# Frankie2030/DataMining_RecBLR

Hardware: AMD Instinct MI355X
Metric: sequences/sec fwd+bwd at B=2048 L=200 d=128; 1/2/4/8-GPU scaling (higher is better)
Workload: dtype f32 I/O, f16x3 split GEMM products

## Files before the change

datamining_recblr_amd/_lib.py:

```python
from __future__ import annotations

import ctypes
import os
import re
import threading

_HERE = os.path.dirname(os.path.abspath(__file__))
LIB_PATH = os.environ.get("RECBLR_LIB") or os.path.join(_HERE, "lib", "libdmrecblr.so")
HEADER_PATH = os.path.join(os.path.dirname(_HERE), "include", "recblr_hip.h")


class RecBLRNativeError(RuntimeError):
    """The HIP extension is missing, failed to load, or a kernel call failed."""


_BY_VALUE = {"int": ctypes.c_int, "int64_t": ctypes.c_int64, "uint64_t": ctypes.c_uint64,
             "float": ctypes.c_float, "double": ctypes.c_double}
_NOT_DECLARATIONS = re.compile(
    r'/\*.*?\*/|//[^\n]*|^[ \t]*#[^\n]*|\btypedef\b(?:[^;{]|\{[^}]*\})*;|extern\s+"C"\s*\{|^\s*\}\s*$',
    re.S | re.M)


def parse_header(text: str) -> dict:
    out = {}
    for decl in _NOT_DECLARATIONS.sub(" ", text).split(";"):
        decl = " ".join(decl.split())
        if not decl:
            continue
        m = re.fullmatch(r"([\w\s*]+?)\s*\b(\w+)\s*\(([^()]*)\)", decl)
        if m is None:
            raise RecBLRNativeError(f"header: not a plain function declaration: {decl!r}")
        ret, name, params = m.groups()
        if re.fullmatch(r"const\s+char\s*\*", ret):
            restype = ctypes.c_char_p
        elif ret in _BY_VALUE:
            restype = _BY_VALUE[ret]
        else:
            raise RecBLRNativeError(f"header: {name}: unsupported return type {ret!r}")
        argtypes = []
        for param in ([] if params.strip() == "void" else params.split(",")):
            words = param.split()
            by_value = " ".join(words[:-1] if len(words) > 1 else words)
            if "*" in param:
                argtypes.append(ctypes.c_void_p)
            elif by_value in _BY_VALUE:
                argtypes.append(_BY_VALUE[by_value])
            else:
                raise RecBLRNativeError(f"header: {name}: unsupported parameter {param.strip()!r}")
        out[name] = (restype, argtypes)
    return out


def _read(path: str) -> str:
    with open(path) as f:
        return f.read()


def _define(text: str, name: str) -> int:
    m = re.search(rf"^[ \t]*#[ \t]*define[ \t]+{name}[ \t]+\(?(-?\d+)\)?[ \t]*$", text, re.M)
    if m is None:
        raise RecBLRNativeError(f"header: no integer #define {name}")
    return int(m.group(1))


_header = _read(HEADER_PATH)
RB_EINVAL = _define(_header, "RB_EINVAL")
RB_TILE = _define(_header, "RB_TILE")
ABI_VERSION = _define(_header, "RB_ABI_VERSION")

SIGNATURES = parse_header(_header)
DENSE_SIGNATURES = parse_header(_read(os.path.join(os.path.dirname(HEADER_PATH),
                                                   "recblr_dense.h")))
PAIR_SIGNATURES = parse_header(_read(os.path.join(os.path.dirname(HEADER_PATH),
                                                  "recblr_pairs.h")))
CANDIDATE_SIGNATURES = parse_header(_read(os.path.join(os.path.dirname(HEADER_PATH),
                                                       "recblr_candidates.h")))
EXP_SIGNATURES = parse_header(_read(os.path.join(_HERE, "experimental", "recblr_exp.h")))
PROBE_SIGNATURES = parse_header(_read(os.path.join(_HERE, "probes", "recblr_probe.h")))
SESSION_SIGNATURES = parse_header(_read(os.path.join(_HERE, "session", "recblr_session.h")))

_lock = threading.Lock()
_loaded = {}


def _load(path, signatures, missing, version=None, mismatch=None, cache=True,
          hint="") -> ctypes.CDLL:
    with _lock:
        if cache and path in _loaded:
            return _loaded[path]
        if not os.path.exists(path):
            raise RecBLRNativeError(f"{missing}: {path} is missing. Run "
                                    f"`python -m datamining_recblr_amd.build`{hint}.")
        try:
            lib = ctypes.CDLL(path)
        except OSError as exc:
            raise RecBLRNativeError(f"failed to load {path}: {exc}") from exc
        for name, (res, args) in signatures.items():
            fn = getattr(lib, name)
            fn.restype = res
            fn.argtypes = args
        if version is not None and getattr(lib, version)() != ABI_VERSION:
            raise RecBLRNativeError(mismatch.format(getattr(lib, version)(), ABI_VERSION))
        if cache:
            _loaded[path] = lib
        return lib


def load(path: str | None = None) -> ctypes.CDLL:
    return _load(path or LIB_PATH,
                 {**SIGNATURES, **DENSE_SIGNATURES, **PAIR_SIGNATURES, **CANDIDATE_SIGNATURES},
                 "HIP extension not built",
                 "rb_version",
                 "ABI mismatch: library {} vs binding {}; rebuild", cache=path is None,
                 hint=" (hipcc --offload-arch=gfx950)")


def load_probe() -> ctypes.CDLL:
    return _load(os.path.join(os.path.dirname(LIB_PATH), "libdmrecblr_probe.so"),
                 PROBE_SIGNATURES, "probe library not built")


def load_exp() -> ctypes.CDLL:
    return _load(os.path.join(os.path.dirname(LIB_PATH), "libdmrecblr_exp.so"), EXP_SIGNATURES,
                 "experimental library not built", "rb_exp_version",
                 "experimental library ABI {} vs {}; rebuild")


def load_session() -> ctypes.CDLL:
    return _load(os.path.join(os.path.dirname(LIB_PATH), "libdmrecblr_session.so"),
                 SESSION_SIGNATURES, "session library not built", "rb_session_version",
                 "session library ABI {} vs {}; rebuild")


_fns = {}
_failure_hooks = []


def on_failure(hook) -> None:
    _failure_hooks.append(hook)


def _check(rc: int, name: str, lib: ctypes.CDLL, last_error: str, hooks: bool = True) -> None:
    if rc == 0:
        return
    kind = str(rc)
    if hooks:
        for hook in _failure_hooks:
            hook()
        kind = "invalid argument" if rc == RB_EINVAL else f"hipError {rc}"
    msg = getattr(lib, last_error)()
    raise RecBLRNativeError(f"{name} failed ({kind}): {msg.decode() if msg else ''}")


def call(name: str, *args) -> None:
    fn = _fns.get(name)
    if fn is None:
        fn = _fns[name] = getattr(load(), name)
    rc = fn(*args)
    if rc != 0:
        _check(rc, name, load(), "rb_last_error_string")


def call_probe(name: str, *args) -> None:
    lib = load_probe()
    _check(getattr(lib, name)(*args), name, lib, "rb_probe_last_error_string", hooks=False)


def call_exp(name: str, *args) -> None:
    lib = load_exp()
    _check(getattr(lib, name)(*args), name, lib, "rb_exp_last_error_string")


def call_session(name: str, *args) -> None:
    lib = load_session()
    rc = getattr(lib, name)(*args)
    if rc != 0:
        _check(rc, name, lib, "rb_session_last_error_string")
```

datamining_recblr_amd/build.py:

```python
from __future__ import annotations

import glob
import os
import shutil
import subprocess
import sys

_HERE = os.path.dirname(os.path.abspath(__file__))
ROOT = os.path.dirname(_HERE)
SOURCES = sorted(glob.glob(os.path.join(_HERE, "csrc", "*.hip")))
HEADERS = sorted(glob.glob(os.path.join(_HERE, "csrc", "*.h"))) + [
    os.path.join(ROOT, "include", "recblr_hip.h"),
    os.path.join(ROOT, "include", "recblr_dense.h"),
    os.path.join(ROOT, "include", "recblr_pairs.h"),
    os.path.join(ROOT, "include", "recblr_candidates.h")]
OUT = os.path.join(_HERE, "lib", "libdmrecblr.so")
PROBE_SOURCES = sorted(glob.glob(os.path.join(_HERE, "probes", "*.hip")))
PROBE_HEADERS = HEADERS + sorted(glob.glob(os.path.join(_HERE, "probes", "*.h")))
PROBE_OUT = os.path.join(_HERE, "lib", "libdmrecblr_probe.so")
EXP_SOURCES = sorted(glob.glob(os.path.join(_HERE, "experimental", "*.hip")))
EXP_HEADERS = HEADERS + sorted(glob.glob(os.path.join(_HERE, "experimental", "*.h")))
EXP_OUT = os.path.join(_HERE, "lib", "libdmrecblr_exp.so")
SESSION_SOURCES = sorted(glob.glob(os.path.join(_HERE, "session", "*.hip")))
SESSION_HEADERS = HEADERS + sorted(glob.glob(os.path.join(_HERE, "session", "*.h")))
SESSION_OUT = os.path.join(_HERE, "lib", "libdmrecblr_session.so")
ARCH = os.environ.get("PYTORCH_ROCM_ARCH", "gfx950")

FLAGS = ["-O3", "-std=c++20", "-shared", "-fPIC", f"--offload-arch={ARCH}",
         "-ffp-contract=off", "-Wall", "-Wno-unused-function"]


def hipcc() -> str:
    for cand in (os.environ.get("HIPCC"), "/opt/rocm/bin/hipcc", shutil.which("hipcc")):
        if cand and os.path.exists(cand):
            return cand
    raise RuntimeError("hipcc not found (expected /opt/rocm/bin/hipcc)")


def _stale(out, deps) -> bool:
    if not os.path.exists(out):
        return True
    t = os.path.getmtime(out)
    return any(os.path.getmtime(s) > t for s in deps)


def _compile(out, sources, extra, verbose, jobs):
    os.makedirs(os.path.dirname(out), exist_ok=True)
    tmp = out + ".tmp"
    cmd = [hipcc(), *FLAGS, *extra, "-I", os.path.join(ROOT, "include"), "-o", tmp, *sources]
    if jobs > 1:
        cmd.insert(1, f"-parallel-jobs={jobs}")
    if verbose:
        print(" ".join(cmd), flush=True)
    subprocess.run(cmd, check=True)
    os.replace(tmp, out)


def build(force: bool = False, verbose: bool = False, jobs: int = 4) -> str:
    if force or _stale(OUT, SOURCES + HEADERS):
        _compile(OUT, SOURCES, [], verbose, jobs)
    if PROBE_SOURCES and (force or _stale(PROBE_OUT, PROBE_SOURCES + PROBE_HEADERS)):
        _compile(PROBE_OUT, PROBE_SOURCES, ["-fvisibility=hidden"], verbose, jobs)
    if EXP_SOURCES and (force or _stale(EXP_OUT, EXP_SOURCES + EXP_HEADERS)):
        _compile(EXP_OUT, EXP_SOURCES, ["-fvisibility=hidden"], verbose, jobs)
    if SESSION_SOURCES and (force or _stale(SESSION_OUT, SESSION_SOURCES + SESSION_HEADERS)):
        _compile(SESSION_OUT, SESSION_SOURCES, ["-fvisibility=hidden"], verbose, jobs)
    return OUT


if __name__ == "__main__":
    print(build(force="--force" in sys.argv, verbose=True))
```

datamining_recblr_amd/csrc/capi.hip:

```cpp
#include "common.h"

#include <atomic>

namespace rb {

namespace {
thread_local std::string g_last_error;
}

int fail(const char* msg) {
  g_last_error = msg;
  return RB_EINVAL;
}

static int fail(const char* fn, const char* msg) {
  g_last_error = std::string(fn) + ": " + msg;
  return RB_EINVAL;
}

int num_cus() {
  static std::atomic<int> cache[64];
  int dev = 0;
  if (hipGetDevice(&dev) != hipSuccess || dev < 0 || dev >= 64) dev = 0;
  int n = cache[dev].load(std::memory_order_relaxed);
// ... 713 lines not shown
  return launch_candidate_scores(h, ldh, table, cand, B, C, d, V, scores, as_stream(stream));
}

int rb_candidate_topk(const float* h, int64_t ldh, const float* table, const int64_t* cand,
                      int64_t B, int64_t C, int64_t d, int64_t V, int64_t first_item, int64_t k,
                      const int64_t* exclude, int64_t E, int64_t* ids, float* scores,
                      void* stream) {
  const char* fn = "rb_candidate_topk";
  if (B < 0) return fail(fn, "B must be >= 0");
  if (B == 0) return 0;
  if (int rc = check_candidates(fn, h, ldh, table, cand, C, d, V)) return rc;
  if (!ids || !scores) return fail(fn, "null pointer");
  if (C > 4096) return fail(fn, "C must be in [1, 4096]");
  if (E < 0 || E > 4096) return fail(fn, "E must be in [0, 4096]");
  if (E > 0 && !exclude) return fail(fn, "null pointer");
  if (k < 1 || k >= (int64_t(1) << 31)) return fail(fn, "k must be in [1, 2^31)");
  if (first_item < 0 || first_item > V) return fail(fn, "first_item must be in [0, V]");
  if (B >= (int64_t(1) << 31)) return fail(fn, "grid too large");
  return launch_candidate_topk(h, ldh, table, cand, B, C, d, V, first_item, k, exclude, E, ids,
                               scores, as_stream(stream));
}

int rb_candidate_ranks(const float* h, int64_t ldh, const float* table, const int64_t* target,
                       const int64_t* cand, int64_t B, int64_t C, int64_t d, int64_t V,
                       int64_t first_item, int64_t* n_greater, int64_t* n_equal, void* stream) {
  const char* fn = "rb_candidate_ranks";
  if (B < 0) return fail(fn, "B must be >= 0");
  if (B == 0) return 0;
  if (int rc = check_candidates(fn, h, ldh, table, cand, C, d, V)) return rc;
  if (!target || !n_greater || !n_equal) return fail(fn, "null pointer");
  if (first_item < 0 || first_item > V) return fail(fn, "first_item must be in [0, V]");
  if (B >= (int64_t(1) << 31) || C >= (int64_t(1) << 40) ||
      B * candidate_rank_chunks(C) >= (int64_t(1) << 31))
    return fail(fn, "grid too large");
  return launch_candidate_ranks(h, ldh, table, target, cand, B, C, d, V, first_item, n_greater,
                                n_equal, as_stream(stream));
}

int rb_group_absmax(const float* x, int64_t n, int64_t c, int64_t ld, float* out, void* stream) {
  if (!x || !out) return fail("rb_group_absmax: null pointer");
  if (n <= 0 || c <= 0 || ld < c) return fail("rb_group_absmax: bad shape");
  return launch_group_absmax(x, n, c, ld, out, reinterpret_cast<hipStream_t>(stream));
}

int rb_item_scores(const float* seq, const float* items, int64_t B, int64_t V, int64_t d,
                   float* scores, void* stream) {
  if (int rc = check_items("rb_item_scores", seq, items, B, V, d)) return rc;
  if (!scores) return fail("rb_item_scores: null pointer");
  return launch_item_scores(seq, items, B, V, d, scores, reinterpret_cast<hipStream_t>(stream));
}

int rb_pad_prefix_fwd(const float* conv_b, const float* gate_w, const float* gate_b,
                      const float* lam, const int64_t* pad, int64_t pad_len, int64_t n_rows,
                      int64_t H, float* h0, float* workspace, void* stream) {
  if (!conv_b || !gate_w || !gate_b || !lam || !h0 || !workspace)
    return fail("rb_pad_prefix_fwd: null pointer");
  if (H <= 0 || H > 4096 || n_rows <= 0 || pad_len < 0)
    return fail("rb_pad_prefix_fwd: need 0 < H <= 4096, n_rows > 0, pad_len >= 0");
  return launch_pad_prefix_fwd(conv_b, gate_w, gate_b, lam, pad, pad_len, n_rows, H, h0,
                               workspace, reinterpret_cast<hipStream_t>(stream));
}

int rb_pad_prefix_bwd(const float* conv_b, const float* gate_w, const float* gate_b,
                      const float* lam, const int64_t* pad, int64_t pad_len, int64_t n_rows,
                      int64_t H, const float* dh0, float* dconv_b, float* dgate_w,
                      float* dgate_b, float* dlam, float* workspace, int accumulate,
                      void* stream) {
  if (!conv_b || !gate_w || !gate_b || !lam || !dh0 || !dconv_b || !dgate_w || !dgate_b || !dlam ||
      !workspace)
    return fail("rb_pad_prefix_bwd: null pointer");
  if (H <= 0 || H > 4096 || n_rows <= 0 || pad_len < 0)
    return fail("rb_pad_prefix_bwd: need 0 < H <= 4096, n_rows > 0, pad_len >= 0");
  return launch_pad_prefix_bwd(conv_b, gate_w, gate_b, lam, pad, pad_len, n_rows, H, dh0,
                               dconv_b, dgate_w, dgate_b, dlam, workspace, accumulate,
                               reinterpret_cast<hipStream_t>(stream));
}

int rb_colsum(const float* in, int64_t M, int64_t P, int64_t C, int64_t rs, int64_t ms,
              float* out, void* stream) {
  if (!in || !out) return fail("rb_colsum: null pointer");
  if (M <= 0 || P <= 0 || C <= 0 || rs < C || (M > 1 && ms < P * rs))
    return fail("rb_colsum: bad shape or strides");
  if (M * ((C + 63) / 64) > 0x7fffffffLL) return fail("rb_colsum: grid too large");
  return launch_colsum(in, M, P, C, rs, ms, out, reinterpret_cast<hipStream_t>(stream));
}

int rb_colsum_chunked(const float* in, int64_t M, int64_t P, int64_t C, int64_t rs,
                      int64_t chunk_rows, float* part, uint32_t* counters, int64_t n_counters,
                      float* out, void* stream) {
  if (!in || !out || !part || !counters) return fail("rb_colsum_chunked: null pointer");
  if (M <= 0 || P <= 0 || C <= 0 || rs < C ||
      (chunk_rows != 64 && chunk_rows != 128 && chunk_rows != 256) || P % chunk_rows)
    return fail("rb_colsum_chunked: bad shape, stride or chunk size");
  const int64_t cblocks = (C + 63) / 64;
  if (n_counters < M * cblocks) return fail("rb_colsum_chunked: too few counters");
  if (M * cblocks * (P / chunk_rows) > 0x7fffffffLL || M * P * rs >= ((int64_t)1 << 40))
    return fail("rb_colsum_chunked: grid too large");
  return launch_colsum_chunked(in, M, P, C, rs, (int)chunk_rows, part,
                               reinterpret_cast<unsigned*>(counters), out,
                               reinterpret_cast<hipStream_t>(stream));
}

int rb_pack_plan(const int64_t* item_seq, int64_t seq_rs, const int64_t* seq_offsets,
                 const int64_t* order, int64_t B, int64_t L, int64_t* ids, int64_t* row_pos,
                 int64_t* inv, int64_t* last, void* stream) {
  if (!item_seq || !seq_offsets || !order || !ids || !row_pos || !inv || !last)
    return fail("rb_pack_plan: null pointer");
  if (B < 1 || L < 1 || seq_rs < L) return fail("rb_pack_plan: bad shape or row stride");
  if ((B + 3) / 4 > 0x7fffffffLL) return fail("rb_pack_plan: grid too large");
  return launch_pack_plan(item_seq, seq_rs, seq_offsets, order, B, ids, row_pos, inv, last,
                          reinterpret_cast<hipStream_t>(stream));
}

int64_t rb_gemm_h_weight_bytes(int64_t C, int64_t R) {
  return ws_image_offset(C, R) + (R % 32 == 0 ? C * R * 4 : 0);
}
int rb_gemm_nt_h_mode(int mode) { return gemm_nt_h_mode(mode); }

int rb_gemm_nt_h_ln(const float* A, int64_t lda, int64_t M, int64_t R, const void* Wf, int64_t C,
                    const float* bias, const float* resid, const float* gamma, const float* beta,
                    float eps, uint64_t seed, float p, float* y, float* s_out, float* mean,
                    float* rstd, int64_t ldo, float* rmax, void* stream) {
  if (!A || !Wf || !resid || !gamma || !beta || !y || !s_out || !mean || !rstd)
    return fail("rb_gemm_nt_h_ln: null pointer");
  if (M <= 0 || R <= 0 || C != 128) return fail("rb_gemm_nt_h_ln: C must be 128, M and R positive");
  if (R != 128 && R != 256 && R != 512) return fail("rb_gemm_nt_h_ln: R must be 128, 256 or 512");
  if (lda < R || lda % 4 || ldo < C || ldo % 4) return fail("rb_gemm_nt_h_ln: bad row strides");
  if (!aligned16(A) || !aligned16(Wf) || !aligned16(resid) || !aligned16(y) || !aligned16(s_out) ||
      !aligned16(gamma) || !aligned16(beta) || (bias && !aligned16(bias)))
    return fail("rb_gemm_nt_h_ln: A, Wf, resid, y, s_out, gamma, beta and bias must be 16-byte aligned");
  if (!(p >= 0.0f && p < 1.0f)) return fail("rb_gemm_nt_h_ln: dropout p must be in [0, 1)");
  if (!(eps > 0.0f)) return fail("rb_gemm_nt_h_ln: eps must be positive");
  if ((M + 31) / 32 > 0x3fffffffLL) return fail("rb_gemm_nt_h_ln: grid too large");
  if (gemm_nt_h_mode(-1) != 1) return fail("rb_gemm_nt_h_ln: needs the weight-stationary kernel (rb_gemm_nt_h_mode 1)");
  return launch_gemm_nt_ws_ln(A, lda, M, (int)R, Wf, (int)C, bias, resid, make_drop(nullptr, seed, p),
                              gamma, beta, eps, y, s_out, mean, rstd, ldo, rmax,
                              reinterpret_cast<hipStream_t>(stream));
}

int rb_gemm_h_split_weights(const rb_split_job* jobs, int64_t n, void* stream) {
  if (!jobs || n < 1 || n > RB_MAX_SPLIT_JOBS)
    return fail("rb_gemm_h_split_weights: need 1..RB_MAX_SPLIT_JOBS jobs");
  for (int64_t j = 0; j < n; ++j) {
    const rb_split_job& b = jobs[j];
    if (!b.W || !b.Wf) return fail("rb_gemm_h_split_weights: null pointer");
    if (b.C <= 0 || b.R <= 0 || b.C % 32 || b.R % 16 || b.C > (1 << 20) || b.R > (1 << 20))
      return fail("rb_gemm_h_split_weights: C must be a multiple of 32 and R of 16");
    if (b.ldw < (b.transpose ? b.C : b.R)) return fail("rb_gemm_h_split_weights: bad row stride");
    if (!aligned16(b.Wf)) return fail("rb_gemm_h_split_weights: Wf must be 16-byte aligned");
  }
  return launch_split_weights_h(jobs, (int)n, reinterpret_cast<hipStream_t>(stream));
}

int rb_gemm_nt_h(const float* A, int64_t lda, int64_t M, int64_t R, const void* Wf, int64_t C,
                 const float* bias, float* out, int64_t ldo, int accumulate, float* rmax,
                 void* stream) {
  if (!A || !Wf || !out) return fail("rb_gemm_nt_h: null pointer");
  if (M <= 0 || R <= 0 || C <= 0) return fail("rb_gemm_nt_h: empty shape");
  if (accumulate) return fail("rb_gemm_nt_h: accumulate is not supported (add the residual in its consumer)");
  if (R % 32 || C % 32 || R > (1 << 16) || C > 1024)
    return fail("rb_gemm_nt_h: R and C must be multiples of 32 (C <= 1024)");
  if (lda < R || lda % 4 || ldo < C || ldo % 2) return fail("rb_gemm_nt_h: bad row strides");
  if (!aligned16(A) || !aligned16(Wf) || (reinterpret_cast<uintptr_t>(out) & 7))
    return fail("rb_gemm_nt_h: A and Wf must be 16-byte aligned, out 8-byte aligned");
  if ((M + 31) / 32 > 0x7fffffffLL) return fail("rb_gemm_nt_h: grid too large");
  return launch_gemm_nt_h(A, lda, M, (int)R, Wf, (int)C, bias, out, ldo, accumulate, rmax,
                          reinterpret_cast<hipStream_t>(stream));
}

int rb_gemm_nt_h_act(const float* A, int64_t lda, int64_t M, int64_t R, const void* Wf, int64_t C,
                     const float* bias, float* out, int64_t ldo, float* rmax, float* act,
                     uint64_t seed, float p, void* stream) {
  if (!A || !Wf || !out || !act) return fail("rb_gemm_nt_h_act: null pointer");
  if (M <= 0 || R <= 0 || C <= 0) return fail("rb_gemm_nt_h_act: empty shape");
  if (R % 32 || C % 32 || R > 1024 || C > 1024)
    return fail("rb_gemm_nt_h_act: R and C must be multiples of 32 (R, C <= 1024)");
  if (lda < R || lda % 4 || ldo < C || ldo % 4) return fail("rb_gemm_nt_h_act: bad row strides");
  if (!aligned16(A) || !aligned16(Wf) || !aligned16(out) || !aligned16(act) ||
      (bias && !aligned16(bias)))
    return fail("rb_gemm_nt_h_act: A, Wf, out, act and bias must be 16-byte aligned");
  if (!(p >= 0.0f && p < 1.0f)) return fail("rb_gemm_nt_h_act: dropout p must be in [0, 1)");
  if ((M + 31) / 32 > 0x7fffffffLL) return fail("rb_gemm_nt_h_act: grid too large");
  return launch_gemm_nt_h_act(A, lda, M, (int)R, Wf, (int)C, bias, out, ldo, rmax, act,
                              make_drop(nullptr, seed, p), reinterpret_cast<hipStream_t>(stream));
}

int rb_adam_step(const rb_adam_job* jobs, int64_t n, double lr, double beta1, double beta2,
                 double eps, double weight_decay, double bc1, double bc2, void* stream) {
  if (!jobs || n <= 0 || n > RB_MAX_ADAM_JOBS) return fail("rb_adam_step: 1..RB_MAX_ADAM_JOBS jobs");
  int64_t blocks = 0;
  for (int64_t j = 0; j < n; ++j) {
    const rb_adam_job& b = jobs[j];
    if (!b.param || !b.grad || !b.exp_avg || !b.exp_avg_sq || b.n <= 0)
      return fail("rb_adam_step: null pointer or empty tensor");
    if (!aligned16(b.param) || !aligned16(b.grad) || !aligned16(b.exp_avg) ||
        !aligned16(b.exp_avg_sq))
      return fail("rb_adam_step: tensors must be 16-byte aligned");
    blocks += (b.n + 1023) / 1024;
  }
  if (blocks > 0x7fffffffLL) return fail("rb_adam_step: too many elements");
  if (!(bc1 > 0.0 && bc2 > 0.0)) return fail("rb_adam_step: bias corrections must be > 0");
  return launch_adam(jobs, (int)n, lr, beta1, beta2, eps, weight_decay, bc1, bc2,
                     reinterpret_cast<hipStream_t>(stream));
}

int64_t rb_gemm_nt_h_dact_parts(void) { return nt_h_dact_parts(); }

int rb_gemm_nt_h_dact(const float* A, int64_t lda, int64_t M, int64_t R, const void* Wf, int64_t C,
                      float* out, int64_t ldo, float* rmax, const float* pre, uint64_t seed,
                      float p, float* dpart, int64_t n_parts, void* stream) {
  if (!A || !Wf || !out || !pre || !dpart) return fail("rb_gemm_nt_h_dact: null pointer");
  if (M <= 0 || R <= 0 || C <= 0) return fail("rb_gemm_nt_h_dact: empty shape");
  if (R % 32 || C % 32 || R > 1024 || C > 512)
    return fail("rb_gemm_nt_h_dact: R and C must be multiples of 32 (R <= 1024, C <= 512)");
  if (lda < R || lda % 4 || ldo < C || ldo % 4) return fail("rb_gemm_nt_h_dact: bad row strides");
  if (!aligned16(A) || !aligned16(Wf) || !aligned16(out) || !aligned16(pre) || !aligned16(dpart))
    return fail("rb_gemm_nt_h_dact: A, Wf, out, pre and dpart must be 16-byte aligned");
  if (!(p >= 0.0f && p < 1.0f)) return fail("rb_gemm_nt_h_dact: dropout p must be in [0, 1)");
  if ((M + 31) / 32 > 0x7fffffffLL) return fail("rb_gemm_nt_h_dact: grid too large");
  return launch_gemm_nt_h_dact(A, lda, M, (int)R, Wf, (int)C, out, ldo, rmax, pre,
                               make_drop(nullptr, seed, p), dpart, n_parts,
                               reinterpret_cast<hipStream_t>(stream));
}

int rb_gemm_tn_h(const float* dY, int64_t ldy, const float* X, int64_t ldx, int64_t M, int64_t N,
                 int64_t K, const float* ymax, const float* xmax, float* parts, int64_t splits,
                 void* stream) {
  if (!dY || !X || !ymax || !xmax || !parts) return fail("rb_gemm_tn_h: null pointer");
  if (M <= 0 || N <= 0 || K <= 0) return fail("rb_gemm_tn_h: empty shape");
  if (N % 128 || K % 128 || N > 65536 || K > 65536)
    return fail("rb_gemm_tn_h: N and K must be multiples of 128 (<= 65536)");
  if (splits < 1 || splits > 65536) return fail("rb_gemm_tn_h: splits must be in [1, 65536]");
  if (ldy < N || ldx < K || ldy % 4 || ldx % 4) return fail("rb_gemm_tn_h: bad row strides");
  if (!aligned16(dY) || !aligned16(X)) return fail("rb_gemm_tn_h: dY and X must be 16-byte aligned");
  if ((N / 128) * (K / 128) * splits > 0x7fffffffLL) return fail("rb_gemm_tn_h: grid too large");
  const int64_t mk = ((M + splits - 1) / splits + 31) / 32 * 32;
  if (mk * (ldy > ldx ? ldy : ldx) * 4 >= 0x7fffffffLL)
    return fail("rb_gemm_tn_h: a row chunk spans 2 GiB or more (use more splits)");
  return launch_gemm_tn_h(dY, ldy, X, ldx, M, (int)N, (int)K, ymax, xmax, parts, (int)splits,
                          reinterpret_cast<hipStream_t>(stream));
}

int rb_gemm_bf16_weight_image(const float* W, int64_t ldw, int64_t C, int64_t R, int transpose,
                              void* img, void* stream) {
  if (!W || !img) return fail("rb_gemm_bf16_weight_image: null pointer");
  if (C <= 0 || R <= 0 || C % 16 || R % 32 || C > 65536 || R > 65536)
    return fail("rb_gemm_bf16_weight_image: C % 16 == 0 and R % 32 == 0 required (<= 65536)");
  if (ldw < (transpose ? C : R)) return fail("rb_gemm_bf16_weight_image: bad row stride");
  if (!aligned16(img)) return fail("rb_gemm_bf16_weight_image: img must be 16-byte aligned");
  return launch_bf16_weight_image(W, ldw, (int)C, (int)R, transpose ? 1 : 0, img,
                                  reinterpret_cast<hipStream_t>(stream));
}

int rb_gemm_nt_bf16(const void* A, int64_t lda, int64_t M, int64_t R, const void* img, int64_t C,
                    const float* bias, void* out, int64_t ldo, void* stream) {
  if (!A || !img || !out) return fail("rb_gemm_nt_bf16: null pointer");
  if (M <= 0 || R <= 0 || C <= 0) return fail("rb_gemm_nt_bf16: empty shape");
  if (R % 64 || C % 256 || R > 16384 || C > 65536)
    return fail("rb_gemm_nt_bf16: R % 64 == 0 (<= 16384) and C % 256 == 0 required");
  if (lda < R || lda % 8 || lda > (1 << 20) || ldo < C || ldo % 8)
    return fail("rb_gemm_nt_bf16: bad row strides (lda % 8 == 0, ldo % 8 == 0)");
  if (!aligned16(A) || !aligned16(img) || !aligned16(out) || (bias && !aligned16(bias)))
    return fail("rb_gemm_nt_bf16: A, img, out and bias must be 16-byte aligned");
  if ((M + 255) / 256 > 0x7fffffffLL / (C / 256) / 2) return fail("rb_gemm_nt_bf16: too many tiles");
  return launch_gemm_nt_bf16(A, lda, M, (int)R, img, (int)C, bias, out, ldo,
                             reinterpret_cast<hipStream_t>(stream));
}

int rb_gemm_tn_hs(const float* dY, int64_t ldy, const float* X, int64_t ldx, int64_t M, int64_t N,
                  int64_t K, float* dw, int accumulate, void* stream) {
  if (!dY || !X || !dw) return fail("rb_gemm_tn_hs: null pointer");
  if (M <= 0 || N <= 0 || K <= 0) return fail("rb_gemm_tn_hs: empty shape");
  if (N % 32 || K % 32 || N > 65536 || K > 65536)
    return fail("rb_gemm_tn_hs: N and K must be multiples of 32");
  if (M > (1 << 24)) return fail("rb_gemm_tn_hs: M too large for the few-rows kernel");
  if (ldy < N || ldx < K) return fail("rb_gemm_tn_hs: bad row strides");
  return launch_gemm_tn_hs(dY, ldy, X, ldx, M, (int)N, (int)K, dw, accumulate,
                           reinterpret_cast<hipStream_t>(stream));
}

}
```

datamining_recblr_amd/csrc/common.h:

```cpp
#pragma once

#include <hip/hip_runtime.h>

#include <algorithm>
#include <cstdint>
#include <string>
#include <type_traits>

#include "../../include/recblr_hip.h"
#include "../../include/recblr_dense.h"
#include "../../include/recblr_pairs.h"
#include "../../include/recblr_candidates.h"

namespace rb {

constexpr int kWave = 64;

int fail(const char* msg);
int launch_status(const char* what);
int num_cus();

inline bool aligned16(const void* p) { return (reinterpret_cast<uintptr_t>(p) & 15) == 0; }

template <class F>
auto dispatch_bool(bool b, F&& f) {
  return b ? f(std::true_type{}) : f(std::false_type{});
}
template <int... Vs, class F>
bool dispatch_int(int v, F&& f) {
  return ((v == Vs ? (f(std::integral_constant<int, Vs>{}), true) : false) || ...);
}

__device__ __forceinline__ float sigm(float x) { return 1.0f / (1.0f + expf(-x)); }
__device__ __forceinline__ float softplus_f(float x) { return x > 20.0f ? x : log1pf(expf(x)); }
__device__ __forceinline__ float dsoftplus_f(float x) { return x > 20.0f ? 1.0f : sigm(x); }
__device__ __forceinline__ float silu_f(float x) { return x / (1.0f + expf(-x)); }
__device__ __forceinline__ float dsilu_f(float x) {
  const float s = sigm(x);
  return s * (1.0f + x * (1.0f - s));
}

constexpr float kLog2e = 1.4426950408889634f;
__device__ __forceinline__ float fexp(float x) { return __builtin_amdgcn_exp2f(x * kLog2e); }
__device__ __forceinline__ float frcp(float x) { return __builtin_amdgcn_rcpf(x); }
__device__ __forceinline__ float fsqrt(float x) { return __builtin_amdgcn_sqrtf(x); }
__device__ __forceinline__ float fsigm(float x) { return frcp(1.0f + fexp(-x)); }
__device__ __forceinline__ float fsilu(float x) { return x * fsigm(x); }
__device__ __forceinline__ float fdsilu(float x) {
  const float s = fsigm(x);
  return s * (1.0f + x * (1.0f - s));
}

typedef float rb_f32x4 __attribute__((ext_vector_type(4)));
typedef float rb_f32x2v __attribute__((ext_vector_type(2)));
typedef uint32_t rb_u32x4 __attribute__((ext_vector_type(4)));
typedef uint32_t rb_u32x2 __attribute__((ext_vector_type(2)));

template <bool NT, typename T>
__device__ __forceinline__ T ld_pol(const T* p) {
  if constexpr (NT) return __builtin_nontemporal_load(p);
  else return *p;
}
template <bool NT, typename T>
__device__ __forceinline__ void st_pol(T v, T* p) {
  if constexpr (NT) __builtin_nontemporal_store(v, p);
  else *p = v;
}
constexpr bool kNT = true;

template <bool NT, int V>
__device__ __forceinline__ void ld_f32(float (&o)[V], const float* p) {
  if constexpr (V == 4) {
    const rb_f32x4 t = ld_pol<NT>(reinterpret_cast<const rb_f32x4*>(p));
    o[0] = t[0]; o[1] = t[1]; o[2] = t[2]; o[3] = t[3];
  } else if constexpr (V == 2) {
    const rb_f32x2v t = ld_pol<NT>(reinterpret_cast<const rb_f32x2v*>(p));
    o[0] = t[0]; o[1] = t[1];
  } else {
#pragma unroll
    for (int v = 0; v < V; ++v) o[v] = ld_pol<NT>(p + v);
  }
}

template <bool NT, int V>
__device__ __forceinline__ void st_f32(float* p, const float (&o)[V]) {
  if constexpr (V == 4) {
    st_pol<NT>(rb_f32x4{o[0], o[1], o[2], o[3]}, reinterpret_cast<rb_f32x4*>(p));
  } else if constexpr (V == 2) {
    st_pol<NT>(rb_f32x2v{o[0], o[1]}, reinterpret_cast<rb_f32x2v*>(p));
  } else {
#pragma unroll
    for (int v = 0; v < V; ++v) st_pol<NT>(o[v], p + v);
  }
}

template <int V>
__device__ __forceinline__ void ldv(float (&o)[V], const float* p) { ld_f32<kNT>(o, p); }
template <int V>
__device__ __forceinline__ void stv(float* p, const float (&o)[V]) { st_f32<kNT>(p, o); }
template <int V>
__device__ __forceinline__ void ldc(float (&o)[V], const float* p) { ld_f32<false>(o, p); }
template <int V>
__device__ __forceinline__ void stc(float* p, const float (&o)[V]) { st_f32<false>(p, o); }

typedef __bf16 bf16_t;
typedef __bf16 rb_bf16x2 __attribute__((ext_vector_type(2)));
typedef float rb_f32x2 __attribute__((ext_vector_type(2)));

__device__ __forceinline__ void unpack2(uint32_t u, float& a, float& b) {
  a = __uint_as_float(u << 16);
  b = __uint_as_float(u & 0xffff0000u);
}
__device__ __forceinline__ uint32_t pack2(float a, float b) {
  return __builtin_bit_cast(uint32_t, __builtin_convertvector(rb_f32x2{a, b}, rb_bf16x2));
}

template <bool NT, int V>
__device__ __forceinline__ void ld_b16(float (&o)[V], const bf16_t* p) {
  if constexpr (V == 8) {
    const rb_u32x4 t = ld_pol<NT>(reinterpret_cast<const rb_u32x4*>(p));
    unpack2(t[0], o[0], o[1]); unpack2(t[1], o[2], o[3]);
    unpack2(t[2], o[4], o[5]); unpack2(t[3], o[6], o[7]);
  } else if constexpr (V == 4) {
    const rb_u32x2 t = ld_pol<NT>(reinterpret_cast<const rb_u32x2*>(p));
    unpack2(t[0], o[0], o[1]); unpack2(t[1], o[2], o[3]);
  } else if constexpr (V == 2) {
    unpack2(ld_pol<NT>(reinterpret_cast<const uint32_t*>(p)), o[0], o[1]);
  } else {
#pragma unroll
    for (int v = 0; v < V; ++v) o[v] = (float)p[v];
  }
}

template <bool NT, int V>
__device__ __forceinline__ void st_b16(bf16_t* p, const float (&o)[V]) {
  if constexpr (V == 8) {
    st_pol<NT>(rb_u32x4{pack2(o[0], o[1]), pack2(o[2], o[3]), pack2(o[4], o[5]), pack2(o[6], o[7])},
               reinterpret_cast<rb_u32x4*>(p));
  } else if constexpr (V == 4) {
    st_pol<NT>(rb_u32x2{pack2(o[0], o[1]), pack2(o[2], o[3])}, reinterpret_cast<rb_u32x2*>(p));
  } else if constexpr (V == 2) {
    st_pol<NT>(pack2(o[0], o[1]), reinterpret_cast<uint32_t*>(p));
  } else {
#pragma unroll
    for (int v = 0; v < V; ++v) p[v] = (bf16_t)o[v];
  }
}

template <int V>
__device__ __forceinline__ void ldv(float (&o)[V], const bf16_t* p) { ld_b16<kNT>(o, p); }
template <int V>
__device__ __forceinline__ void stv(bf16_t* p, const float (&o)[V]) { st_b16<kNT>(p, o); }
template <int V>
__device__ __forceinline__ void ldc(float (&o)[V], const bf16_t* p) { ld_b16<false>(o, p); }
template <int V>
__device__ __forceinline__ void stc(bf16_t* p, const float (&o)[V]) { st_b16<false>(p, o); }

template <typename T, int V>
struct RawVec {
  float w[V];
};
template <int V>
struct RawVec<bf16_t, V> {
  static_assert(V % 2 == 0, "packed bf16 needs an even width");
  uint32_t w[V / 2];
// ... 32 lines not shown
}
template <int V>
__device__ __forceinline__ void unpack_raw(float (&o)[V], const RawVec<bf16_t, V>& r) {
  if constexpr (V == 1) {
    o[0] = r.w[0];
  } else {
#pragma unroll
    for (int k = 0; k < V / 2; ++k) unpack2(r.w[k], o[2 * k], o[2 * k + 1]);
  }
}

template <int VH, typename T, int V>
__device__ __forceinline__ void unpack_part(float (&o)[VH], const RawVec<T, V>& r, int h0) {
  if constexpr (VH == V) {
    unpack_raw(o, r);
  } else if constexpr (sizeof(T) == 4) {
#pragma unroll
    for (int v = 0; v < VH; ++v) o[v] = r.w[h0 + v];
  } else {
#pragma unroll
    for (int k = 0; k < VH / 2; ++k) unpack2(r.w[h0 / 2 + k], o[2 * k], o[2 * k + 1]);
  }
}
template <int VH, typename T, int V>
__device__ __forceinline__ void pack_part(RawVec<T, V>& r, const float (&o)[VH], int h0) {
  if constexpr (sizeof(T) == 4) {
#pragma unroll
    for (int v = 0; v < VH; ++v) r.w[h0 + v] = o[v];
  } else {
    static_assert(VH % 2 == 0, "packed bf16 pairs");
#pragma unroll
    for (int k = 0; k < VH / 2; ++k) r.w[h0 / 2 + k] = pack2(o[2 * k], o[2 * k + 1]);
  }
}
template <int VH, typename T, int V>
__device__ __forceinline__ void opaque_part(RawVec<T, V>& r, int h0) {
  constexpr int per = sizeof(T) == 2 && V > 1 ? 2 : 1;
#pragma unroll
  for (int k = 0; k < VH / per; ++k) asm volatile("" : "+v"(r.w[h0 / per + k]));
}
template <int V>
__device__ __forceinline__ void stv_raw(float* p, const RawVec<float, V>& r) { st_f32<kNT>(p, r.w); }
template <int V>
__device__ __forceinline__ void stv_raw(bf16_t* p, const RawVec<bf16_t, V>& r) {
  if constexpr (V == 8) {
    st_pol<kNT>(rb_u32x4{r.w[0], r.w[1], r.w[2], r.w[3]}, reinterpret_cast<rb_u32x4*>(p));
  } else if constexpr (V == 4) {
    st_pol<kNT>(rb_u32x2{r.w[0], r.w[1]}, reinterpret_cast<rb_u32x2*>(p));
  } else {
    static_assert(V == 2, "packed bf16 image");
    st_pol<kNT>(r.w[0], reinterpret_cast<uint32_t*>(p));
  }
}

__device__ __forceinline__ uint4 philox4x32_10(uint4 c, uint32_t k0, uint32_t k1) {
#pragma unroll
  for (int i = 0; i < 10; ++i) {
    const uint64_t p0 = (uint64_t)0xD2511F53u * c.x, p1 = (uint64_t)0xCD9E8D57u * c.z;
    const uint32_t lo0 = (uint32_t)p0, hi0 = (uint32_t)(p0 >> 32);
    const uint32_t lo1 = (uint32_t)p1, hi1 = (uint32_t)(p1 >> 32);
    c = make_uint4(hi1 ^ c.y ^ k0, lo1, hi0 ^ c.w ^ k1, lo0);
    k0 += 0x9E3779B9u;
    k1 += 0xBB67AE85u;
  }
  return c;
}

struct DropSpec {
  const uint8_t* mask;
  uint32_t key0, key1, keep_thresh;
  float scale;
  int mode;

  __device__ __forceinline__ void get4(int64_t e, float (&m)[4]) const {
    if (mode == 0) {
      m[0] = m[1] = m[2] = m[3] = 1.0f;
    } else if (mode == 1) {
      const uchar4 t = *reinterpret_cast<const uchar4*>(mask + e);
      m[0] = t.x * scale; m[1] = t.y * scale; m[2] = t.z * scale; m[3] = t.w * scale;
    } else {
      const uint64_t g = (uint64_t)e >> 2;
      const uint4 r = philox4x32_10(make_uint4((uint32_t)g, (uint32_t)(g >> 32), 0u, 0u), key0,
                                    key1);
      m[0] = r.x < keep_thresh ? scale : 0.0f;
      m[1] = r.y < keep_thresh ? scale : 0.0f;
      m[2] = r.z < keep_thresh ? scale : 0.0f;
      m[3] = r.w < keep_thresh ? scale : 0.0f;
    }
  }
};

DropSpec make_drop(const uint8_t* mask, uint64_t seed, float p);


int launch_pack_plan(const int64_t* seq, int64_t seq_rs, const int64_t* offs,
                     const int64_t* order, int64_t B, int64_t* ids, int64_t* pos, int64_t* inv,
                     int64_t* last, hipStream_t st);
int launch_next_item_targets(const int64_t* ids, const int64_t* offs, const int64_t* order,
                             const int64_t* pos_items, int64_t B, int64_t ntok, int64_t m_pad,
                             int64_t* tgt, hipStream_t st);
template <typename T>
int launch_scan_fwd(const T* gates, const T* tokens, T* states, int64_t rows, int64_t steps,
                    hipStream_t st);
template <typename T>
int launch_scan_bwd(const T* gates, const T* states, const T* grad, T* d_gates, T* d_tokens,
                    int64_t rows, int64_t steps, hipStream_t st);
template <typename T>
int launch_conv_fwd(const T* x, int64_t x_rs, const float* w, const float* bias, T* xc,
                    int64_t xc_rs, int64_t B, int64_t L, int64_t H, int64_t K,
                    const int64_t* offs, hipStream_t st);
template <typename T>
int launch_conv_fwd_rows(const T* x, int64_t x_rs, const float* w, const float* bias, T* xc,
                         int64_t xc_rs, int64_t ntok, int64_t H, int64_t K, const int64_t* pos,
                         hipStream_t st);
template <typename T>
int launch_conv_bwd(const T* x, int64_t x_rs, const float* w, const float* bias, const T* g1,
                    const T* g2, T* dx, int64_t dx_rs, float* dw_part, float* db_part, int64_t B,
                    int64_t L, int64_t H, int64_t K, const int64_t* offs, hipStream_t st);
template <typename T>
int launch_gate_fwd(const T* rg, int64_t rg_rs, const T* xc, int64_t xc_rs, const T* z,
                    int64_t z_rs, const float* lam, const float* gb, const float* h0,
                    int64_t h0_bs, T* y, int64_t y_rs, float* carries, int64_t B, int64_t L,
                    int64_t H, const int64_t* offs, hipStream_t st, T* y_last = nullptr,
                    const int64_t* order = nullptr);
template <typename T>
int launch_gate_bwd(const T* rg, int64_t rg_rs, const T* xc, int64_t xc_rs, const T* z,
                    int64_t z_rs, const float* lam, const float* gb, const float* carries,
                    const T* dy, T* drg, int64_t drg_rs, T* dxc, int64_t dxc_rs, T* dz,
                    int64_t dz_rs, float* part, float* dh0_part, int64_t B, int64_t L, int64_t H,
                    const int64_t* offs, hipStream_t st, const T* dy_last = nullptr,
                    const int64_t* order = nullptr);
int launch_add_ln_fwd(const float* a, const int64_t* idx, int64_t nidx, const DropSpec& drop,
                      const float* r, const float* gamma, const float* beta, float eps, float* y,
                      float* s_out, float* mean, float* rstd, int64_t rows, int64_t d,
                      hipStream_t st);
int launch_add_ln_bwd(const float* dy, const float* dy2, const float* s, const float* gamma,
                      const float* mean, const float* rstd, const DropSpec& drop, float* ds,
                      float* da, float* dgp, float* dbp, float* dbiasp, int64_t nparts,
                      int64_t rows, int64_t d, hipStream_t st);
int64_t ln_num_parts(int64_t rows, int64_t d);
int launch_silu_dropout_fwd(const float* a, const float* bias, const DropSpec& drop, float* u,
                            int64_t rows, int64_t cols, hipStream_t st);
int launch_silu_dropout_bwd(const float* a, const float* bias, const DropSpec& drop,
                            const float* du, float* da, float* dbias_part, int64_t nparts,
                            int64_t rows, int64_t cols, hipStream_t st);
int launch_dropout_mask(const DropSpec& drop, uint8_t* out, int64_t n, hipStream_t st);
int launch_split_weights_h(const rb_split_job* jobs, int n, hipStream_t st);
int launch_bf16_weight_image(const float* W, int64_t ldw, int C, int R, int transpose, void* img,
                             hipStream_t st);
int launch_gemm_nt_bf16(const void* A, int64_t lda, int64_t M, int R, const void* img, int C,
                        const float* bias, void* out, int64_t ldo, hipStream_t st);
int launch_gemm_tn_h(const float* Y, int64_t ldy, const float* X, int64_t ldx, int64_t M, int N,
                     int K, const float* ymax, const float* xmax, float* parts, int S,
                     hipStream_t st);
constexpr int kWeightScale = 14;
template <class S>
struct WeightSlot {
  S slot;
  int col, k0;
};
template <class S = int64_t, class I>
__host__ __device__ inline WeightSlot<S> weight_slot32(int nkb, I cb, int kb, int p, int lane) {
  return {((S)(cb * nkb + kb) * 2 + p) * 64 + lane, (int)cb * 32 + (lane & 31),
          kb * 16 + 8 * (lane >> 5)};
}
template <class S = int64_t, class I>
__host__ __device__ inline WeightSlot<S> weight_slot16(int nkb, I cb, int ks, int p, int lane) {
  return {((S)(cb * nkb + ks) * 2 + p) * 64 + lane, (int)cb * 16 + (lane & 15),
          ks * 32 + 8 * (lane >> 4)};
}
__host__ __device__ inline int64_t ws_image_offset(int64_t C, int64_t K) {
  return C * K * 4 + ((C * 4 + 15) / 16) * 16;
}
struct WeightImage {
  const void* wf;
  const int* ew;
  const void* wi;
};
inline WeightImage weight_image(const void* Wf, int64_t C, int64_t R) {
  const char* base = static_cast<const char*>(Wf);
  return {Wf, reinterpret_cast<const int*>(base + C * R * 4), base + ws_image_offset(C, R)};
}
int nt_dact_zero_rest(float* dpart, int64_t used, int64_t n_parts, int C, hipStream_t st);
bool nt_ws_ok(int64_t M, int K, int C, const float* A, int64_t lda, const float* out, int64_t ldo);
int launch_gemm_nt_ws(const float* A, int64_t lda, int64_t M, int K, const void* Wf, int C,
                      const float* bias, float* out, int64_t ldo, float* rmax, hipStream_t st);
int gemm_nt_h_mode(int mode);
bool nt_ws_act_ok(int64_t M, int K, int C, const float* A, int64_t lda, const float* out,
                  const float* other, int64_t ldo);
int launch_gemm_nt_ws_act(const float* A, int64_t lda, int64_t M, int K, const void* Wf, int C,
                          const float* bias, float* out, int64_t ldo, float* rmax, float* act,
                          DropSpec drop, hipStream_t st);
int launch_gemm_nt_ws_dact(const float* A, int64_t lda, int64_t M, int K, const void* Wf, int C,
                           float* out, int64_t ldo, float* rmax, const float* pre, DropSpec drop,
                           float* dpart, int64_t n_parts, hipStream_t st);
bool nt_ws_ln_ok(int64_t M, int K, int C, const float* A, int64_t lda, const float* y,
                 const float* s_out, const float* resid, int64_t ldo);
int launch_gemm_nt_ws_ln(const float* A, int64_t lda, int64_t M, int K, const void* Wf, int C,
                         const float* bias, const float* resid, DropSpec drop, const float* gamma,
                         const float* beta, float eps, float* y, float* s_out, float* mean,
                         float* rstd, int64_t ldo, float* rmax, hipStream_t st);
int launch_gemm_nt_h(const float* A, int64_t lda, int64_t M, int R, const void* Wf, int C,
                     const float* bias, float* out, int64_t ldo, int accumulate, float* rmax,
                     hipStream_t st);
int launch_gemm_nt_h_act(const float* A, int64_t lda, int64_t M, int R, const void* Wf, int C,
                         const float* bias, float* out, int64_t ldo, float* rmax, float* act,
                         DropSpec drop, hipStream_t st);
int64_t nt_h_dact_parts();
int launch_gemm_nt_h_dact(const float* A, int64_t lda, int64_t M, int R, const void* Wf, int C,
                          float* out, int64_t ldo, float* rmax, const float* pre, DropSpec drop,
                          float* dpart, int64_t n_parts, hipStream_t st);
int launch_adam(const rb_adam_job* jobs, int n, double lr, double beta1, double beta2, double eps,
                double weight_decay, double bc1, double bc2, hipStream_t st);
int launch_gemm_nt_hs(const float* A, int64_t lda, int64_t M, int R, const void* Wf, int C,
                      const float* bias, float* out, int64_t ldo, float* rmax, hipStream_t st);
int launch_gemm_tn_hs(const float* Y, int64_t ldy, const float* X, int64_t ldx, int64_t M, int N,
                      int K, float* dw, int accumulate, hipStream_t st);
int64_t emb_workspace_bytes(int64_t M, int64_t V, int64_t d);
int launch_embedding_plan(const int64_t* idx, int64_t M, int64_t d, int64_t V, void* workspace,
                          int64_t ws_bytes, hipStream_t st);
int launch_embedding_apply(const float* grad, int64_t M, int64_t d, int64_t V,
                           int64_t padding_idx, float* dw, void* workspace, int64_t ws_bytes,
                           hipStream_t st);
int launch_embedding_bwd(const int64_t* idx, const float* grad, int64_t M, int64_t d, int64_t V,
                         int64_t padding_idx, float* dw, void* workspace, int64_t ws_bytes,
                         hipStream_t st);
int launch_embedding_apply_scaled(const float* src, int64_t src_ld, int64_t src_rows,
                                  const float* coef, int64_t M, int64_t d, int64_t V,
                                  int64_t padding_idx, float* dw, void* workspace,
                                  int64_t ws_bytes, hipStream_t st);
int launch_sample_negatives(const int64_t* item_seq, int64_t seq_rs, const int64_t* lengths,
                            const int64_t* pos_items, const int64_t* offsets, const int64_t* inv,
                            int64_t B, int64_t L, int64_t n_neg, int64_t first, int64_t V,
                            uint64_t seed, int64_t ntok, int64_t m_pad, int64_t* neg,
                            hipStream_t st);
int64_t pair_loss_workspace_bytes(int64_t M);
int launch_pair_loss_fwd(const float* h, int64_t ldh, const float* tab, const int64_t* pos,
                         const int64_t* neg, int64_t M, int64_t d, int64_t V, int64_t n_neg,
                         float gamma, float* diff, float* loss, int64_t* n_live, void* workspace,
                         hipStream_t st);
int launch_pair_loss_bwd(const float* tab, const int64_t* pos, const int64_t* neg,
                         const float* diff, const float* dloss, const int64_t* n_live, int64_t M,
                         int64_t d, int64_t V, int64_t n_neg, float gamma, float* dh, float* coef,
                         hipStream_t st);
int launch_candidate_scores(const float* h, int64_t ldh, const float* tab, const int64_t* cand,
                            int64_t B, int64_t C, int64_t d, int64_t V, float* scores,
                            hipStream_t st);
int launch_candidate_topk(const float* h, int64_t ldh, const float* tab, const int64_t* cand,
                          int64_t B, int64_t C, int64_t d, int64_t V, int64_t first, int64_t k,
                          const int64_t* exclude, int64_t E, int64_t* ids, float* scores,
                          hipStream_t st);
int64_t candidate_rank_chunks(int64_t C);
int launch_candidate_ranks(const float* h, int64_t ldh, const float* tab, const int64_t* target,
                           const int64_t* cand, int64_t B, int64_t C, int64_t d, int64_t V,
                           int64_t first, int64_t* n_gt, int64_t* n_eq, hipStream_t st);
int64_t item_ce_workspace_bytes(int64_t B, int64_t V, int64_t D);
int64_t item_rank_workspace_bytes(int64_t B, int64_t V);
int launch_item_ce_fwd(const float* E, const float* W, const int64_t* tgt, int64_t B, int64_t V,
                       int64_t D, float* lse, float* loss, void* ws, int64_t ws_bytes,
                       hipStream_t st);
int launch_item_ce_bwd(const float* E, const float* W, const int64_t* tgt, const float* lse,
                       const float* dloss, int64_t B, int64_t V, int64_t D, float* dE, float* dW,
                       void* ws, int64_t ws_bytes, hipStream_t st);
int launch_item_rank(const float* E, const float* W, const int64_t* tgt, int64_t B, int64_t V,
                     int64_t D, int64_t first, int64_t* n_gt, int64_t* n_eq, void* ws,
                     int64_t ws_bytes, hipStream_t st);
int64_t item_topk_workspace_bytes(int64_t B, int64_t V, int64_t k);
int launch_item_topk(const float* E, const float* W, int64_t B, int64_t V, int64_t D, int64_t k,
                     int64_t first, const int64_t* ex, int64_t NE, int64_t* ids, float* scores,
                     void* ws, int64_t ws_bytes, hipStream_t st);
int launch_item_ce_probs(const float* E, const float* W, const int64_t* tgt, const float* lse,
                         const float* dloss, int64_t B, int64_t V, int64_t D, int64_t v_off,
                         int64_t n_total, float* out, int64_t ld, hipStream_t st);
int launch_item_scores(const float* E, const float* W, int64_t B, int64_t V, int64_t D,
                       float* out, hipStream_t st);
int launch_item_split_h(const float* X, int64_t N, int64_t D, void* img, int* ex, float* gmax,
                        hipStream_t st);
int launch_item_ce_fwd_h(const void* Ei, const int* Ee, const void* Wi, const int* We,
                         const int64_t* tgt, int64_t B, int64_t V, int64_t D, float* lse,
                         float* loss, void* ws, int64_t ws_bytes, bool rows_mode, float inv_n,
                         int accumulate, hipStream_t st);
int launch_item_ce_probs_h(const void* Ei, const int* Ee, const void* Wi, const int* We,
                           const int64_t* tgt, const float* lse, const float* dloss, int64_t B,
                           int64_t V, int64_t D, int64_t v_off, float* out, int64_t ld,
                           float* gmax, float* out2, int64_t ld2, float* bmax, float rows_inv_n,
                           hipStream_t st);
int launch_group_absmax(const float* x, int64_t n, int64_t c, int64_t ld, float* out,
                        hipStream_t st);
int launch_pad_prefix_fwd(const float* conv_b, const float* gw, const float* gb,
                          const float* lam, const int64_t* pad, int64_t pad_len, int64_t n_rows,
                          int64_t H, float* h0, float* ws, hipStream_t st);
int launch_pad_prefix_bwd(const float* conv_b, const float* gw, const float* gb,
                          const float* lam, const int64_t* pad, int64_t pad_len, int64_t n_rows,
                          int64_t H, const float* dh0, float* dconv_b, float* dgw, float* dgb,
                          float* dlam, float* ws, int accumulate, hipStream_t st);
int launch_colsum(const float* in, int64_t M, int64_t P, int64_t C, int64_t rs, int64_t ms,
                  float* out, hipStream_t st);
int launch_colsum_chunked(const float* in, int64_t M, int64_t P, int64_t C, int64_t rs, int CH,
                          float* part, unsigned* cnt, float* out, hipStream_t st);

}
```

datamining_recblr_amd/csrc/gemm_half.hip:

```cpp
#include "common.h"
#include "f16x3.h"
#include "nt_plan.h"

#include <type_traits>

namespace rb {
namespace {

constexpr int kTA = 4;
constexpr int kHead = 11;
constexpr int kTRedo = 14;
constexpr int kSent = -4096;

struct SplitJobsH {
  const float* W[RB_MAX_SPLIT_JOBS];
  f16x8* Wf[RB_MAX_SPLIT_JOBS];
  int64_t ldw[RB_MAX_SPLIT_JOBS];
  int C[RB_MAX_SPLIT_JOBS], R[RB_MAX_SPLIT_JOBS], tr[RB_MAX_SPLIT_JOBS];
  int bstart[RB_MAX_SPLIT_JOBS + 1];
  int n;
};

__global__ void __launch_bounds__(256) k_split_weights_h(const SplitJobsH jobs) {
  __shared__ float smax[256];
// ... 552 lines not shown
      float m = 0.0f;
      for (int kb = 0; kb < KB16; ++kb) {
        const f32x4 p = *reinterpret_cast<const f32x4*>(arow + kb * 16);
        const f32x4 q = *reinterpret_cast<const f32x4*>(arow + kb * 16 + 4);
        m = fmaxf(m, max8abs(p, q));
      }
      m = fmaxf(m, __shfl_xor(m, 32));
      const int e = exp_of(m);
      const float sc = __builtin_amdgcn_ldexpf(1.0f, kTRedo - e);
      int erow[16];
#pragma unroll
      for (int j = 0; j < 16; ++j) erow[j] = __shfl(e, crow(j)) - kTRedo - kWeightScale;
      for (int n = 0; n < N_NB; ++n) {
        f32x16 c;
#pragma unroll
        for (int j = 0; j < 16; ++j) c[j] = 0.0f;
        for (int kb = 0; kb < KB16; ++kb) {
          const f32x4 p = *reinterpret_cast<const f32x4*>(arow + kb * 16);
          const f32x4 q = *reinterpret_cast<const f32x4*>(arow + kb * 16 + 4);
          f16x8 a0, a1;
          split8(p, q, sc, a0, a1);
          const f16x8* bp = Wf + ((int64_t)((ct * N_NB + n) * KB16 + kb) * 2) * 64 + lane;
          const f16x8 b0 = bp[0], b1 = bp[64];
          c = mfma3_h(a0, a1, b0, b1, c);
        }
        const int col = ct * N_BN + n * 32 + ccol;
        const int ecol = s_ew[col];
        const float bv = BIAS ? s_bias[col] : 0.0f;
        float csum = 0.0f;
#pragma unroll
        for (int j = 0; j < 16; ++j) {
          const int64_t r = (int64_t)mt * N_BM + wave * 32 + crow(j);
          if (r < M) {
            float v = __builtin_amdgcn_ldexpf(c[j], erow[j] + ecol) + bv;
            if constexpr (DACT) {
              float mk[4];
              const int64_t ei = e_base + r * C + col;
              drop.get4(ei & ~(int64_t)3, mk);
              const int q = (int)(ei & 3);
              v = (v * (q == 0 ? mk[0] : q == 1 ? mk[1] : q == 2 ? mk[2] : mk[3])) *
                  fdsilu(pre[r * ldo + col] + 0.0f);
              csum += v;
            }
            out[r * ldo + col] = v;
            if constexpr (ACT) {
              float mk[4];
              const int64_t ei = e_base + r * C + col;
              drop.get4(ei & ~(int64_t)3, mk);
              const int q = (int)(ei & 3);
              act[r * ldo + col] = fsilu(v) * (q == 0 ? mk[0] : q == 1 ? mk[1] : q == 2 ? mk[2] : mk[3]);
            }
          }
        }
        if constexpr (DACT) {
          csum += __shfl_xor(csum, 32);
          if (lane < 32) s_col[col] += csum;
        }
      }
    }
  }
  if constexpr (DACT) {
    __syncthreads();
    const float* s_all = reinterpret_cast<const float*>(smem + CF::LDS);
    for (int c = tid; c < C; c += N_THREADS) {
      float t = s_all[c];
#pragma unroll
      for (int w = 1; w < N_WAVES; ++w) t += s_all[w * N_DACT_MAXC + c];
      dpart[(int64_t)bid * C + c] = t;
    }
  }
}

template <bool BIAS, bool WIDE, int NB, bool ACT = false, bool DACT = false>
__global__ void __launch_bounds__(N_THREADS, 1) k_gemm_nt_h(const float* __restrict__ A, int64_t lda,
                                                          int64_t M, int R,
                                                          const f16x8* __restrict__ Wf,
                                                          const int* __restrict__ ew, int C,
                                                          const float* __restrict__ bias,
                                                          float* __restrict__ out, int64_t ldo,
                                                          float* __restrict__ rmax, int m_tiles,
                                                          float* __restrict__ act, DropSpec drop,
                                                          int64_t e_base,
                                                          const float* __restrict__ pre,
                                                          float* __restrict__ dpart) {
  extern __shared__ __attribute__((aligned(16))) char smem[];
  nt_h_body<BIAS, WIDE, NB, ACT, DACT>(smem, (int)blockIdx.x, (int)gridDim.x, A, lda, M, R, Wf, ew,
                                       C, bias, out, ldo, rmax, m_tiles, act, drop, e_base, pre,
                                       dpart);
}

struct NtPhase {
  const float* A;
  int64_t M;
  float* out;
  float* rmax;
  float* act;
  const float* pre;
  float* dpart;
  int64_t e_base;
  int m_tiles;
  int grid;
};

template <bool BIAS, int NB, bool ACT = false, bool DACT = false>
__global__ void __launch_bounds__(N_THREADS, 1)
k_gemm_nt_h2(int64_t lda, int R, const f16x8* __restrict__ Wf, const int* __restrict__ ew, int C,
             const float* __restrict__ bias, int64_t ldo, DropSpec drop, NtPhase main_ph,
             NtPhase tail_ph) {
  extern __shared__ __attribute__((aligned(16))) char smem[];
  const int bid = (int)blockIdx.x;
  if (bid < main_ph.grid)
    nt_h_body<BIAS, true, NB, ACT, DACT>(smem, bid, main_ph.grid, main_ph.A, lda, main_ph.M, R, Wf,
                                         ew, C, bias, main_ph.out, ldo, main_ph.rmax,
                                         main_ph.m_tiles, main_ph.act, drop, main_ph.e_base,
                                         main_ph.pre, main_ph.dpart);
  __syncthreads();
  if (bid < tail_ph.grid)
    nt_h_body<BIAS, true, 2, ACT, DACT>(smem, bid, tail_ph.grid, tail_ph.A, lda, tail_ph.M, R, Wf,
                                        ew, C, bias, tail_ph.out, ldo, tail_ph.rmax,
                                        tail_ph.m_tiles, tail_ph.act, drop, tail_ph.e_base,
                                        tail_ph.pre, tail_ph.dpart);
}

constexpr int T_BT = 128;
constexpr int T_PITCH = 80;
constexpr int kTT = 14;

template <int NBN, int NBK>
struct TnCfg {
  static constexpr int THREADS = 256 * NBN * NBK;
  static constexpr int YC = T_BT * NBN, XC = T_BT * NBK;
  static constexpr int YPLANE = YC * T_PITCH, XPLANE = XC * T_PITCH;
  static constexpr int STAGE = 2 * YPLANE + 2 * XPLANE;
  static constexpr int LDS = 2 * STAGE;
  static constexpr int LOADERS = (YC + XC) / 4 * 4;
};

__device__ __forceinline__ uint32_t tn_off(int col, int chunk) {
  return col * T_PITCH + ((chunk ^ ((col >> 4) & 3)) << 4);
}

template <int NBN, int NBK>
__device__ __attribute__((noinline)) void tn_percol(char* smem, const float* __restrict__ Y, int64_t ldy, const float* __restrict__ X,
                                        int64_t ldx, int64_t M, int N, int K,
                                        const float* __restrict__ ymax,
                                        const float* __restrict__ xmax, float* __restrict__ parts,
                                        int S, int64_t mk, int nt_k);

template <int NBN, int NBK, bool PERCOL>
__device__ __forceinline__ void tn_body(char* smem, const float* __restrict__ Y, int64_t ldy, const float* __restrict__ X,
                                        int64_t ldx, int64_t M, int N, int K,
                                        const float* __restrict__ ymax,
                                        const float* __restrict__ xmax, float* __restrict__ parts,
                                        int S, int64_t mk, int nt_k) {
  using CF = TnCfg<NBN, NBK>;
  const int tid = threadIdx.x;
  const int lane = tid & 63;
  const int wave = __builtin_amdgcn_readfirstlane(tid >> 6);
  const int wm = wave / (2 * NBK), wk = wave % (2 * NBK);
  const int G = gridDim.x;
  const int idx = (blockIdx.x & 7) * (G >> 3) + (blockIdx.x >> 3);
  const int nt = (N / CF::YC) * nt_k;
  const int tile = idx % nt, s = idx / nt;
  if (s >= S) return;
  const int n0 = (tile / nt_k) * CF::YC, k0 = (tile % nt_k) * CF::XC;
  const int64_t r_begin = (int64_t)s * mk;
  const int64_t r_end = r_begin + mk < M ? r_begin + mk : M;
  const int64_t nrows = r_end > r_begin ? r_end - r_begin : 0;
  const int T = (int)((nrows + 31) / 32);

  float my = 0.0f, mx = 0.0f;
  for (int64_t g = r_begin / 32 + tid; g * 32 < r_end; g += CF::THREADS) {
    my = fmaxf(my, ymax[g]);
    mx = fmaxf(mx, xmax[g]);
  }
  float* red = reinterpret_cast<float*>(smem);
#pragma unroll
  for (int o = 32; o >= 1; o >>= 1) {
    my = fmaxf(my, __shfl_xor(my, o));
    mx = fmaxf(mx, __shfl_xor(mx, o));
  }
  constexpr int NW = CF::THREADS / 64;
  if (lane == 0) { red[wave] = my; red[NW + wave] = mx; }
  __syncthreads();
  my = 0.0f;
  mx = 0.0f;
#pragma unroll
  for (int w = 0; w < NW; ++w) {
    my = fmaxf(my, red[w]);
    mx = fmaxf(mx, red[NW + w]);
  }
  const int ey = exp_of(my), ex = exp_of(mx);
  __syncthreads();

  const bool loader = tid < CF::LOADERS;
  const int op = tid < CF::YC ? 0 : 1;
  const int lt = op == 0 ? tid : tid - CF::YC;
  const int ncg = (op == 0 ? CF::YC : CF::XC) / 4;
  const int cc = loader ? lt % ncg : 0;
  const int rg = loader ? lt / ncg : 0;
  const int64_t ld = op == 0 ? ldy : ldx;
  float scv[4];
#pragma unroll
  for (int c = 0; c < 4; ++c) {
    int e = op == 0 ? ey : ex;
    if constexpr (PERCOL) {
      const int col = 4 * cc + c;
      e = *reinterpret_cast<const int*>(smem + (op == 0 ? col * T_PITCH
                                                        : 2 * CF::YPLANE + col * T_PITCH) + 64);
    }
    scv[c] = __builtin_amdgcn_ldexpf(1.0f, kTT - e);
  }
  float cm[4] = {0.0f, 0.0f, 0.0f, 0.0f};
  const uint32_t smem_base = (uint32_t)(uintptr_t)(lds_ptr_t)smem;

  f32x4 raw0[8], raw1[8];
  const float* cbase = (op == 0 ? Y + n0 : X + k0) + r_begin * ld;
  const uint64_t cb = reinterpret_cast<uint64_t>(cbase);
  const uint64_t cbu =
      (uint64_t)(uint32_t)__builtin_amdgcn_readfirstlane((uint32_t)cb) |
      ((uint64_t)(uint32_t)__builtin_amdgcn_readfirstlane((uint32_t)(cb >> 32)) << 32);
  const uint32_t ld4 = __builtin_amdgcn_readfirstlane((uint32_t)(ld * 4));
  const auto rsrc = __builtin_amdgcn_make_buffer_rsrc(
      reinterpret_cast<void*>(cbu), 0, (int)(nrows * ld4), 0x00020000);
  const uint32_t voff = (uint32_t)(rg * 8) * ld4 + (uint32_t)(16 * cc);
  auto load = [&](int t, f32x4 (&r)[8]) {
    __builtin_amdgcn_sched_barrier(0);
#pragma unroll
    for (int q = 0; q < 8; ++q)
      r[q] = __builtin_bit_cast(
          f32x4, __builtin_amdgcn_raw_buffer_load_b128(rsrc, voff + (uint32_t)(t * 32 + q) * ld4, 0, 0));
    __builtin_amdgcn_sched_barrier(0);
  };
  auto convert_pair = [&](const f32x4 (&r)[8], int buf, int p) {
    const uint32_t img = smem_base + buf * CF::STAGE + (op == 0 ? 0 : 2 * CF::YPLANE);
    const uint32_t plane = op == 0 ? CF::YPLANE : CF::XPLANE;
    const f32x2 sc{scv[2 * p], scv[2 * p + 1]};
    f16x8 h0[2], h1[2];
#pragma unroll
    for (int q = 0; q < 8; ++q) {
      const f32x2 v{r[q][2 * p], r[q][2 * p + 1]};
      f16x2 p0, p1;
      split2h(v * sc, p0, p1);
      h0[0][q] = p0[0]; h0[1][q] = p0[1];
      h1[0][q] = p1[0]; h1[1][q] = p1[1];
    }
    if constexpr (!PERCOL) {
#pragma unroll
      for (int c = 0; c < 2; ++c)
#pragma unroll
        for (int q = 0; q < 8; q += 4) {
          cm[2 * p + c] = max3abs(cm[2 * p + c], r[q][2 * p + c], r[q + 1][2 * p + c]);
          cm[2 * p + c] = max3abs(cm[2 * p + c], r[q + 2][2 * p + c], r[q + 3][2 * p + c]);
        }
    }
#pragma unroll
    for (int c = 0; c < 2; ++c) {
      const uint32_t off = tn_off(4 * cc + 2 * p + c, rg);
      lds_write16(img + off, h0[c]);
      lds_write16(img + plane + off, h1[c]);
    }
  };

  f32x16 acc[2][2];
#pragma unroll
  for (int a = 0; a < 2; ++a)
#pragma unroll
    for (int b = 0; b < 2; ++b)
#pragma unroll
      for (int e = 0; e < 16; ++e) acc[a][b][e] = 0.0f;

  const int h = lane >> 5;
  auto mma = [&](int buf, auto conv_c, const f32x4 (&r)[8], int t, int nbuf, auto late_c) {
    (void)t;
    constexpr bool CONV = decltype(conv_c)::value;
    constexpr bool LATE = decltype(late_c)::value;
    const uint32_t iy = smem_base + buf * CF::STAGE;
    const uint32_t ix = iy + 2 * CF::YPLANE;
#pragma unroll
    for (int st = 0; st < 2; ++st) {
      if constexpr (CONV && !LATE) convert_pair(r, nbuf, st);
      f16x8 b[2][2];
#pragma unroll
      for (int j = 0; j < 2; ++j) {
        const uint32_t ob = tn_off(64 * wk + 32 * j + (lane & 31), 2 * st + h);
        b[j][0] = lds_read16<f16x8>(ix + ob);
        b[j][1] = lds_read16<f16x8>(ix + CF::XPLANE + ob);
      }
#pragma unroll
      for (int i = 0; i < 2; ++i) {
        const uint32_t oa = tn_off(64 * wm + 32 * i + (lane & 31), 2 * st + h);
        f16x8 a0 = lds_read16<f16x8>(iy + oa);
        f16x8 a1 = lds_read16<f16x8>(iy + CF::YPLANE + oa);
        if (i == 0)
          asm volatile("s_waitcnt lgkmcnt(0)"
                       : "+v"(a0), "+v"(a1), "+v"(b[0][0]), "+v"(b[0][1]), "+v"(b[1][0]),
                         "+v"(b[1][1]));
        else
          asm volatile("s_waitcnt lgkmcnt(0)" : "+v"(a0), "+v"(a1));
#pragma unroll
        for (int j = 0; j < 2; ++j) {
          acc[i][j] = mfma3_h(a0, a1, b[j][0], b[j][1], acc[i][j]);
        }
      }
      if constexpr (CONV && LATE) convert_pair(r, nbuf, st);
    }
  };
  using conv_t = std::true_type;
  using noconv_t = std::false_type;

  const int Tp = (T + 1) & ~1;
  auto loader_loop = [&](auto late_c) {
    load(0, raw0);
    load(1, raw1);
    convert_pair(raw0, 0, 0);
    convert_pair(raw0, 0, 1);
    load(2, raw0);
    __syncthreads();
    for (int t = 0; t < Tp; t += 2) {
      mma(0, conv_t{}, raw1, t + 1, 1, late_c);
      load(t + 3, raw1);
      __syncthreads();
      mma(1, conv_t{}, raw0, t + 2, 0, late_c);
      load(t + 4, raw0);
      __syncthreads();
    }
  };
  const int wv = __builtin_amdgcn_readfirstlane(tid >> 6);
  if (wv < CF::LOADERS / 64) {
    if (CF::THREADS == 512 && wv >= 4) loader_loop(std::true_type{});
    else loader_loop(std::false_type{});
  } else {
    __syncthreads();
    for (int t = 0; t < Tp; t += 2) {
      mma(0, noconv_t{}, raw1, 0, 0, std::false_type{});
      __syncthreads();
      mma(1, noconv_t{}, raw0, 0, 0, std::false_type{});
      __syncthreads();
    }
  }

  constexpr int NCOL = CF::YC + CF::XC;
  constexpr int pass = PERCOL ? 1 : 0;
  if constexpr (!PERCOL) {
    __syncthreads();
    float* s_cm = reinterpret_cast<float*>(smem + CF::STAGE);
    int* s_redo = reinterpret_cast<int*>(smem + CF::STAGE) + 4 * NCOL;
    if (tid == 0) *s_redo = 0;
    if (loader) {
#pragma unroll
      for (int c = 0; c < 4; ++c) s_cm[rg * NCOL + (op == 0 ? 0 : CF::YC) + 4 * cc + c] = cm[c];
    }
    __syncthreads();
    for (int col = tid; col < NCOL; col += CF::THREADS) {
      const float m = fmaxf(fmaxf(s_cm[col], s_cm[NCOL + col]),
                            fmaxf(s_cm[2 * NCOL + col], s_cm[3 * NCOL + col]));
      const int ec = col < CF::YC ? ey : ex;
      if (m > 0.0f && m < __builtin_amdgcn_ldexpf(1.0f, ec - 16)) *s_redo = 1;
      const int e = exp_of(m);
      const int slot = col < CF::YC ? col * T_PITCH : 2 * CF::YPLANE + (col - CF::YC) * T_PITCH;
      *reinterpret_cast<int*>(smem + slot + 64) = e;
    }
    __syncthreads();
    if (*s_redo != 0) {
      tn_percol<NBN, NBK>(smem, Y, ldy, X, ldx, M, N, K, ymax, xmax, parts, S, mk, nt_k);
      return;
    }
  }

  float* out = parts + (int64_t)s * N * K;
  if constexpr (pass == 0) {
    const int sh = ey + ex - 2 * kTT;
#pragma unroll
    for (int i = 0; i < 2; ++i)
#pragma unroll
      for (int j = 0; j < 2; ++j) {
        const int col = k0 + 64 * wk + 32 * j + (lane & 31);
#pragma unroll
        for (int e = 0; e < 16; ++e) {
          const int row = n0 + 64 * wm + 32 * i + 8 * (e >> 2) + 4 * h + (e & 3);
          __builtin_nontemporal_store(__builtin_amdgcn_ldexpf(acc[i][j][e], sh), out + (int64_t)row * K + col);
        }
      }
  } else {
#pragma unroll
    for (int i = 0; i < 2; ++i)
#pragma unroll
      for (int e = 0; e < 16; ++e) {
        const int nl = 64 * wm + 32 * i + 8 * (e >> 2) + 4 * h + (e & 3);
        const int en = *reinterpret_cast<const int*>(smem + nl * T_PITCH + 64) - 2 * kTT;
#pragma unroll
        for (int j = 0; j < 2; ++j) {
          const int kl = 64 * wk + 32 * j + (lane & 31);
          const int ek = *reinterpret_cast<const int*>(smem + 2 * CF::YPLANE + kl * T_PITCH + 64);
          __builtin_nontemporal_store(__builtin_amdgcn_ldexpf(acc[i][j][e], en + ek), out + (int64_t)(n0 + nl) * K + k0 + kl);
        }
      }
  }
}

template <int NBN, int NBK>
__device__ __attribute__((noinline)) void tn_percol(char* smem, const float* __restrict__ Y, int64_t ldy, const float* __restrict__ X,
                                        int64_t ldx, int64_t M, int N, int K,
                                        const float* __restrict__ ymax,
                                        const float* __restrict__ xmax, float* __restrict__ parts,
                                        int S, int64_t mk, int nt_k) {
  tn_body<NBN, NBK, true>(smem, Y, ldy, X, ldx, M, N, K, ymax, xmax, parts, S, mk, nt_k);
}

template <int NBN, int NBK>
__global__ void __launch_bounds__(256 * NBN * NBK, 2 / (NBN * NBK))
k_gemm_tn_h(const float* __restrict__ Y, int64_t ldy, const float* __restrict__ X, int64_t ldx,
            int64_t M, int N, int K, const float* __restrict__ ymax,
            const float* __restrict__ xmax, float* __restrict__ parts, int S, int64_t mk,
            int nt_k) {
  extern __shared__ __attribute__((aligned(16))) char smem[];
  tn_body<NBN, NBK, false>(smem, Y, ldy, X, ldx, M, N, K, ymax, xmax, parts, S, mk, nt_k);
}


template <bool BIAS, bool WIDE, int NB, bool ACT = false, bool DACT = false>
void run_nt_h(const float* A, int64_t lda, int64_t M, int R, const f16x8* wf, const int* ew, int C,
              const float* bias, float* out, int64_t ldo, float* rmax, int m_tiles, unsigned grid,
              hipStream_t st, float* act = nullptr, DropSpec drop = DropSpec{}, int64_t e_base = 0,
              const float* pre = nullptr, float* dpart = nullptr) {
  constexpr int lds = NtCfg<NB>::LDS + (DACT ? N_WAVES * N_DACT_MAXC * 4 : 0);
  static_assert(lds <= 160 * 1024, "LDS");
  static bool done = false;
  if (!done) {
    (void)hipFuncSetAttribute((const void*)k_gemm_nt_h<BIAS, WIDE, NB, ACT, DACT>,
                        hipFuncAttributeMaxDynamicSharedMemorySize, lds);
    done = true;
  }
  k_gemm_nt_h<BIAS, WIDE, NB, ACT, DACT><<<grid, N_THREADS, lds, st>>>(
      A, lda, M, R, wf, ew, C, bias, out, ldo, rmax, m_tiles, act, drop, e_base, pre, dpart);
}


struct NtArgs {
  const float* A;
  int64_t lda, M;
  int R;
  const void* Wf;
  int C;
  const float* bias;
  float* out;
  int64_t ldo;
  float* rmax;
  float* act;
  const float* pre;
  float* dpart;
  DropSpec drop;
  hipStream_t st;
};

NtPhase nt_phase(const NtArgs& a, int64_t r0, int64_t M, int m_tiles, int grid,
                 int64_t dpart_row) {
  NtPhase p{};
  p.A = a.A + r0 * a.lda;
  p.M = M;
  p.out = a.out + r0 * a.ldo;
  p.rmax = a.rmax ? a.rmax + r0 / 32 : nullptr;
  p.act = a.act ? a.act + r0 * a.ldo : nullptr;
  p.pre = a.pre ? a.pre + r0 * a.ldo : nullptr;
  p.dpart = a.dpart ? a.dpart + dpart_row * a.C : nullptr;
  p.e_base = r0 * a.C;
  p.m_tiles = m_tiles;
  p.grid = grid;
  return p;
}

template <bool BIAS, int NB, bool ACT = false, bool DACT = false>
void run_nt_h2(int64_t lda, int R, const f16x8* wf, const int* ew, int C, const float* bias,
               int64_t ldo, DropSpec drop, const NtPhase& mp, const NtPhase& tp, hipStream_t st) {
  constexpr int base = NtCfg<NB>::LDS > NtCfg<2>::LDS ? NtCfg<NB>::LDS : NtCfg<2>::LDS;
  constexpr int lds = base + (DACT ? N_WAVES * N_DACT_MAXC * 4 : 0);
  static_assert(lds <= 160 * 1024, "LDS");
  static bool done = false;
  if (!done) {
    (void)hipFuncSetAttribute((const void*)k_gemm_nt_h2<BIAS, NB, ACT, DACT>,
                              hipFuncAttributeMaxDynamicSharedMemorySize, lds);
    done = true;
  }
  const unsigned grid = (unsigned)std::max(mp.grid, tp.grid);
  k_gemm_nt_h2<BIAS, NB, ACT, DACT><<<grid, N_THREADS, lds, st>>>(lda, R, wf, ew, C, bias, ldo,
                                                                  drop, mp, tp);
}

template <bool BIAS, bool WIDE, int NB, bool ACT = false, bool DACT = false>
int run_nt_plan(const char* what, const NtPlan& p, const NtArgs& a) {
  const WeightImage w = weight_image(a.Wf, a.C, a.R);
  const f16x8* wf = (const f16x8*)w.wf;
  const NtPhase mp = nt_phase(a, 0, p.M_main, p.m_tiles, p.grid, 0);
  const NtPhase tp = nt_phase(a, p.M_main, a.M - p.M_main, p.m_tiles_t, p.grid_t, p.dpart_tail);
  auto launch = [&](auto wide_c, auto nb_c, const NtPhase& ph) {
    run_nt_h<BIAS, decltype(wide_c)::value, decltype(nb_c)::value, ACT, DACT>(
        ph.A, a.lda, ph.M, a.R, wf, w.ew, a.C, a.bias, ph.out, a.ldo, ph.rmax, ph.m_tiles,
        (unsigned)ph.grid, a.st, ph.act, a.drop, ph.e_base, ph.pre, ph.dpart);
    return launch_status(what);
  };
  switch (p.path) {
    case NtPath::error:
      return fail(p.err);
    case NtPath::both:
      run_nt_h2<BIAS, NB, ACT, DACT>(a.lda, a.R, wf, w.ew, a.C, a.bias, a.ldo, a.drop, mp, tp, a.st);
      return launch_status(what);
    case NtPath::tail:
      return launch(std::true_type{}, std::integral_constant<int, 2>{}, tp);
    case NtPath::few:
    case NtPath::few_main: {
      const int rc = launch_gemm_nt_hs(tp.A, a.lda, tp.M, a.R, a.Wf, a.C, a.bias, tp.out, a.ldo,
                                       tp.rmax, a.st);
      if (rc || p.path == NtPath::few) return rc;
      break;
    }
    case NtPath::main:
      break;
  }
  return launch(std::bool_constant<WIDE>{}, std::integral_constant<int, NB>{}, mp);
}

}

int launch_split_weights_h(const rb_split_job* jobs, int n, hipStream_t st) {
  SplitJobsH sj{};
  sj.n = n;
  int blocks = 0;
  for (int j = 0; j < n; ++j) {
    sj.W[j] = jobs[j].W;
    sj.Wf[j] = (f16x8*)jobs[j].Wf;
    sj.ldw[j] = jobs[j].ldw;
    sj.C[j] = (int)jobs[j].C;
    sj.R[j] = (int)jobs[j].R;
    sj.tr[j] = (int)jobs[j].transpose;
    sj.bstart[j] = blocks;
    blocks += (int)(jobs[j].C / 32);
  }
  sj.bstart[n] = blocks;
  k_split_weights_h<<<(unsigned)blocks, 256, 0, st>>>(sj);
  return launch_status("rb_gemm_h_split_weights");
}

static int g_nt_mode = 1;
constexpr int64_t NT_WS_MIN_ROWS = 16384;
int gemm_nt_h_mode(int mode) {
  const int prev = g_nt_mode;
  if (mode == 0 || mode == 1) g_nt_mode = mode;
  return prev;
}

static_assert(NT_WAVES == N_WAVES && NT_BM == N_BM && NT_MAXC == N_MAXC &&
              NT_DACT_MAXC == N_DACT_MAXC, "nt_plan.h sizes the kernels' tiles");

int launch_gemm_nt_h(const float* A, int64_t lda, int64_t M, int R, const void* Wf, int C,
                     const float* bias, float* out, int64_t ldo, int accumulate, float* rmax,
                     hipStream_t st) {
  (void)accumulate;
  if (g_nt_mode == 1 && M >= NT_WS_MIN_ROWS && nt_ws_ok(M, R, C, A, lda, out, ldo))
    return launch_gemm_nt_ws(A, lda, M, R, Wf, C, bias, out, ldo, rmax, st);
  const bool wide = aligned16(out) && ldo % 4 == 0;
  const NtPlan p = nt_plan(NtKind::plain, M, R, C, wide, bias != nullptr, num_cus());
  const NtArgs a{A, lda, M, R, Wf, C, bias, out, ldo, rmax, nullptr, nullptr, nullptr, DropSpec{}, st};
  return dispatch_bool(p.bias, [&](auto bias_c) {
    constexpr bool BIAS = decltype(bias_c)::value;
    if (p.nb == 8) return run_nt_plan<BIAS, true, 8>("rb_gemm_nt_h", p, a);
    if (p.wide) return run_nt_plan<BIAS, true, 4>("rb_gemm_nt_h", p, a);
    return run_nt_plan<BIAS, false, 4>("rb_gemm_nt_h", p, a);
  });
}

int launch_gemm_nt_h_act(const float* A, int64_t lda, int64_t M, int R, const void* Wf, int C,
                         const float* bias, float* out, int64_t ldo, float* rmax, float* act,
                         DropSpec drop, hipStream_t st) {
  if (g_nt_mode == 1 && M >= NT_WS_MIN_ROWS && nt_ws_act_ok(M, R, C, A, lda, out, act, ldo))
    return launch_gemm_nt_ws_act(A, lda, M, R, Wf, C, bias, out, ldo, rmax, act, drop, st);
  const bool wide = aligned16(out) && aligned16(act) && ldo % 4 == 0;
  const NtPlan p = nt_plan(NtKind::act, M, R, C, wide, bias != nullptr, num_cus());
  const NtArgs a{A, lda, M, R, Wf, C, bias, out, ldo, rmax, act, nullptr, nullptr, drop, st};
  return dispatch_bool(p.bias, [&](auto bias_c) {
    return run_nt_plan<decltype(bias_c)::value, true, 8, true>("rb_gemm_nt_h_act", p, a);
  });
}

int64_t nt_h_dact_parts() { return nt_h_dact_parts(num_cus()); }

int nt_dact_zero_rest(float* dpart, int64_t used, int64_t n_parts, int C, hipStream_t st) {
  if (used < n_parts &&
      hipMemsetAsync(dpart + used * C, 0, (size_t)(n_parts - used) * C * 4, st) != hipSuccess)
    return fail("rb_gemm_nt_h_dact: hipMemsetAsync failed");
  return 0;
}

int launch_gemm_nt_h_dact(const float* A, int64_t lda, int64_t M, int R, const void* Wf, int C,
                          float* out, int64_t ldo, float* rmax, const float* pre, DropSpec drop,
                          float* dpart, int64_t n_parts, hipStream_t st) {
  if (g_nt_mode == 1 && M >= NT_WS_MIN_ROWS && nt_ws_act_ok(M, R, C, A, lda, out, pre, ldo))
    return launch_gemm_nt_ws_dact(A, lda, M, R, Wf, C, out, ldo, rmax, pre, drop, dpart, n_parts, st);
  const bool wide = aligned16(out) && aligned16(pre) && ldo % 4 == 0;
  const NtPlan p = nt_plan(NtKind::dact, M, R, C, wide, false, num_cus(), n_parts);
  const NtArgs a{A, lda, M, R, Wf, C, nullptr, out, ldo, rmax, nullptr, pre, dpart, drop, st};
  const int rc = run_nt_plan<false, true, 4, false, true>("rb_gemm_nt_h_dact", p, a);
  return rc ? rc : nt_dact_zero_rest(dpart, p.used, n_parts, C, st);
}

inline int tn_tile_shape(int N, int K) {
  return N % 256 == 0 ? 2 : (K % 256 == 0 ? 1 : 0);
}

int launch_gemm_tn_h(const float* Y, int64_t ldy, const float* X, int64_t ldx, int64_t M, int N,
                     int K, const float* ymax, const float* xmax, float* parts, int S,
                     hipStream_t st) {
  const int64_t mk = ((M + S - 1) / S + 31) / 32 * 32;
  auto run = [&](auto nbn_c, auto nbk_c) {
    constexpr int NBN = decltype(nbn_c)::value, NBK = decltype(nbk_c)::value;
    using CF = TnCfg<NBN, NBK>;
    static bool done = false;
    if (!done) {
      (void)hipFuncSetAttribute((const void*)k_gemm_tn_h<NBN, NBK>,
                                hipFuncAttributeMaxDynamicSharedMemorySize, CF::LDS);
      done = true;
    }
    const int nt_k = K / CF::XC;
    const int nt = (N / CF::YC) * nt_k;
    k_gemm_tn_h<NBN, NBK><<<(unsigned)((nt * S + 7) / 8 * 8), CF::THREADS, CF::LDS, st>>>(
        Y, ldy, X, ldx, M, N, K, ymax, xmax, parts, S, mk, nt_k);
  };
  switch (tn_tile_shape(N, K)) {
    case 2: run(std::integral_constant<int, 2>{}, std::integral_constant<int, 1>{}); break;
    case 1: run(std::integral_constant<int, 1>{}, std::integral_constant<int, 2>{}); break;
    default: run(std::integral_constant<int, 1>{}, std::integral_constant<int, 1>{}); break;
  }
  return launch_status("rb_gemm_tn_h");
}

}
```

datamining_recblr_amd/csrc/gemm_ws.hip:

```cpp
#include "common.h"
#include "f16x3.h"

#include <type_traits>
#include <utility>

namespace rb {
namespace ws {

constexpr int kTR = 14;
constexpr int WAVES = 8, THREADS = 64 * WAVES, RB = 32;

template <int K, int NCB_, int D_>
struct Cfg {
  static constexpr int KS = K / 32;
  static constexpr int NCB = NCB_;
  static constexpr int D = D_;
  static constexpr int WC = 16 * NCB;
  static constexpr int NT = WC * WAVES;
  static constexpr int NLD = K / 64;
  static constexpr int IMG = RB * K * 4;
  static constexpr int NST = 2 * NCB;
  static constexpr int INFO = 2 * IMG;
  static constexpr int COLS = INFO + 2 * RB * 8;
  static constexpr int STATS = COLS + NT * 8;
  static constexpr bool STG = K <= 256;
  static constexpr int STAGE = STATS + 2 * 2 * RB * WAVES * 4;
  static constexpr int LDS = STAGE + (STG ? D * WAVES * NLD * 1024 : 0);
  static_assert(KS * NCB <= 16 && NCB >= 1, "B slice <= 128 VGPRs");
  static_assert(LDS <= 160 * 1024, "LDS");
};

__device__ __forceinline__ f32x4 gload16(const char* base, uint32_t off) {
  return *reinterpret_cast<const f32x4*>(base + off);
}
__device__ __forceinline__ void dma16(__amdgpu_buffer_rsrc_t rs, uint32_t lds, uint32_t voff) {
  __builtin_amdgcn_raw_ptr_buffer_load_lds(rs, (__attribute__((address_space(3))) void*)(uintptr_t)lds, 16,
                                           voff, 0, 0, 0);
}

struct LnSpec {
  const float* gamma = nullptr;
  const float* beta = nullptr;
  float eps = 0.0f;
  float* mean = nullptr;
  float* rstd = nullptr;
};

template <int K, int NCB, int D, bool BIAS, bool DEFER, int ABL, int EPI = 0>
__global__ void __launch_bounds__(THREADS, 1)
k_gemm_nt_ws(const float* __restrict__ A, int64_t lda, int64_t M, const f16x8* __restrict__ Wi,
             const int* __restrict__ ew, int C, const float* __restrict__ bias,
             float* __restrict__ out, int64_t ldo, float* __restrict__ rmax,
             float* __restrict__ act, DropSpec drop, const float* __restrict__ pre,
             float* __restrict__ dpart, LnSpec ln) {
  using CF = Cfg<K, NCB, D>;
  constexpr int KS = CF::KS, WC = CF::WC, NT = CF::NT, NLD = CF::NLD, NST = CF::NST;
  constexpr bool TWO = EPI == 1 || EPI == 3;
  constexpr bool PRE = EPI == 2 || EPI == 3;
  constexpr int NSTT = TWO ? 2 * NST : NST;
  constexpr int NPRE = PRE ? 2 * NCB : 0;
  constexpr int NSO = NSTT + 1 + (EPI == 3 ? 2 : 0);
  static_assert(EPI != 3 || (NCB == 1 && DEFER), "LN epilogue: whole 128-column rows, deferred stores");
  constexpr bool EARLY1 = D == 1 && (ABL & 32) == 0;
  extern __shared__ __attribute__((aligned(16))) char smem[];
  const int tid = threadIdx.x, lane = tid & 63;
  const int wave = __builtin_amdgcn_readfirstlane(tid >> 6);
  const int bid = blockIdx.x, G = gridDim.x;
  const int nct = C / NT;
  const int ct = (bid >> 3) % nct;
  const int64_t nrb = (M + RB - 1) / RB;
  const int64_t rb0 = (int64_t)(bid / (8 * nct)) * 8 + (bid & 7);
  const int64_t rbs = (int64_t)(G / (8 * nct)) * 8;
  const int nb = rb0 < nrb ? (int)((nrb - 1 - rb0) / rbs + 1) : 0;
  const int64_t prow = (int64_t)(bid / (8 * nct)) * 8 + (bid & 7);
  if (nb == 0) {
    if constexpr (EPI == 2)
      for (int c = tid; c < NT; c += THREADS) dpart[prow * C + ct * NT + c] = 0.0f;
    return;
  }

  const uint32_t sbase = (uint32_t)(uintptr_t)(__attribute__((address_space(3))) void*)smem;
  const uint32_t s_info = sbase + CF::INFO;
  const uint32_t s_cols = sbase + CF::COLS;
  for (int c = tid; c < NT; c += THREADS) {
    const int e = ew[ct * NT + c] - kTR - kWeightScale;
    const float bv = BIAS ? bias[ct * NT + c] : 0.0f;
    asm volatile("ds_write_b32 %0, %1" ::"v"(s_cols + c * 4), "v"(e) : "memory");
    asm volatile("ds_write_b32 %0, %1" ::"v"(s_cols + (NT + c) * 4), "v"(bv) : "memory");
  }

  const int col0 = ct * NT + wave * WC;
  f16x8 bw[NCB][KS][2];
#pragma unroll
  for (int cb = 0; cb < NCB; ++cb)
#pragma unroll
    for (int s = 0; s < KS; ++s)
#pragma unroll
      for (int p = 0; p < 2; ++p)
        bw[cb][s][p] = Wi[weight_slot16(KS, col0 / 16 + cb, s, p, lane).slot];

  const int my_row = 4 * wave + (lane >> 4);
  uint32_t woff[NLD];
#pragma unroll
  for (int j = 0; j < NLD; ++j) {
    const int c = 16 * j + (lane & 15);
    const int r16 = my_row & 15, rb16 = my_row >> 4;
    const int s = c >> 3, g = (c >> 1) & 3, half = c & 1;
    const int pos = (r16 ^ ((4 * s + g) & 15)) + 16 * g;
    woff[j] = (uint32_t)(((rb16 * KS + s) * 2) * 1024 + pos * 16 + half * 8);
  }
  f32x4 ra[CF::STG ? 1 : D][NLD];
  auto blk_r0 = [&](int b) __attribute__((always_inline)) -> int64_t { return (rb0 + (int64_t)b * rbs) * RB; };
  auto rsrc_of = [&](const float* p, int64_t r0, int64_t ld) __attribute__((always_inline)) {
    const uint64_t u = reinterpret_cast<uint64_t>(p + r0 * ld);
    const uint64_t ub = (uint64_t)(uint32_t)__builtin_amdgcn_readfirstlane((uint32_t)u) |
                        ((uint64_t)(uint32_t)__builtin_amdgcn_readfirstlane((uint32_t)(u >> 32)) << 32);
    const int64_t n = M - r0 < RB ? (M - r0 > 0 ? M - r0 : 0) : RB;
    return __builtin_amdgcn_make_buffer_rsrc(reinterpret_cast<void*>(ub), 0, (int)(n * ld * 4), 0x00020000);
  };
  const uint32_t a_voff = (uint32_t)(my_row * lda * 4) + (uint32_t)(lane & 15) * 16;
  const uint32_t s_stage = sbase + CF::STAGE;
  auto stage_of = [&](int set) __attribute__((always_inline)) -> uint32_t { return s_stage + (uint32_t)((set * WAVES + wave) * NLD) * 1024; };
  auto issue = [&](int b, f32x4 (&dst)[NLD], int set) __attribute__((always_inline)) {
    if constexpr ((ABL & 8) != 0) return;
    const auto rs = rsrc_of(A, blk_r0(b), lda);
    if constexpr (CF::STG) {
      const uint32_t st = __builtin_amdgcn_readfirstlane(stage_of(set));
#pragma unroll
      for (int j = 0; j < NLD; ++j)
        dma16(rs, st + j * 1024, a_voff + j * 256);
    } else {
#pragma unroll
      for (int j = 0; j < NLD; ++j)
        dst[j] = __builtin_bit_cast(f32x4, __builtin_amdgcn_raw_buffer_load_b128(rs, a_voff + j * 256, 0, 0));
    }
    asm volatile("" ::: "memory");
  };

  auto split = [&](f32x4 (&src)[NLD], int ib, int set) __attribute__((always_inline)) {
    if constexpr (CF::STG) {
#pragma unroll
      for (int j = 0; j < NLD; ++j) src[j] = lds_read16<f32x4>(stage_of(set) + j * 1024 + lane * 16);
      if constexpr (NLD == 2) asm volatile("s_waitcnt lgkmcnt(0)" : "+v"(src[0]), "+v"(src[1]));
      else asm volatile("s_waitcnt lgkmcnt(0)" : "+v"(src[0]), "+v"(src[1]), "+v"(src[2]), "+v"(src[3]));
    }
    if constexpr ((ABL & 2) != 0) {
#pragma unroll
      for (int j = 0; j < NLD; ++j) asm volatile("" ::"v"(src[j]));
      return;
    }
    float mx = max4abs(src[0]);
#pragma unroll
    for (int j = 1; j < NLD; ++j) mx = fmaxf(mx, max4abs(src[j]));
    mx = fmaxf(mx, dpp_xor1(mx));
    mx = fmaxf(mx, dpp_xor2(mx));
    mx = fmaxf(mx, __builtin_bit_cast(float, __builtin_amdgcn_mov_dpp(__builtin_bit_cast(int, mx), 0x124, 0xF, 0xF, false)));
    mx = fmaxf(mx, __builtin_bit_cast(float, __builtin_amdgcn_mov_dpp(__builtin_bit_cast(int, mx), 0x128, 0xF, 0xF, false)));
    const int e = exp_of(mx);
    const float sc = __builtin_amdgcn_ldexpf(1.0f, kTR - e);
    const uint32_t img = sbase + ib * CF::IMG;
#pragma unroll
    for (int j = 0; j < NLD; ++j) {
      const f32x4 v = src[j] * sc;
      f16x2 h0a, h1a, h0b, h1b;
      split2h(f32x2{v[0], v[1]}, h0a, h1a);
      split2h(f32x2{v[2], v[3]}, h0b, h1b);
      lds_write8<0>(img + woff[j], f16x4{h0a[0], h0a[1], h0b[0], h0b[1]});
      lds_write8<1024>(img + woff[j], f16x4{h1a[0], h1a[1], h1b[0], h1b[1]});
    }
    if ((lane & 15) == 0) {
      asm volatile("ds_write_b32 %0, %1" ::"v"(s_info + (ib * RB + my_row) * 4), "v"(e) : "memory");
      asm volatile("ds_write_b32 %0, %1" ::"v"(s_info + (2 * RB + ib * RB + my_row) * 4), "v"(mx) : "memory");
    }
  };

  uint32_t rpos[4];
#pragma unroll
  for (int t = 0; t < 4; ++t) rpos[t] = (uint32_t)((((lane & 15) ^ ((4 * t + (lane >> 4)) & 15)) + (lane & 48)) * 16);

  f32x4 acc[2][NCB];
  auto multiply = [&](int ib, auto&& hook) __attribute__((always_inline)) {
#pragma unroll
    for (int r = 0; r < 2; ++r)
#pragma unroll
      for (int cb = 0; cb < NCB; ++cb) acc[r][cb] = f32x4{0.0f, 0.0f, 0.0f, 0.0f};
    if constexpr ((ABL & 1) != 0) return;
    const uint32_t img = sbase + ib * CF::IMG;
    f16x8 fa[2][2];
    auto rd = [&](auto uc, int t) __attribute__((always_inline)) {
      constexpr int u = decltype(uc)::value, s = u >> 1, r = u & 1;
      const uint32_t a = img + rpos[s & 3];
      fa[t][0] = lds_read16o<((r * KS + s) * 2 + 0) * 1024, f16x8>(a);
      fa[t][1] = lds_read16o<((r * KS + s) * 2 + 1) * 1024, f16x8>(a);
    };
    rd(std::integral_constant<int, 0>{}, 0);
    auto unit = [&](auto uc) __attribute__((always_inline)) {
      constexpr int u = decltype(uc)::value, t = u & 1, s = u >> 1, r = u & 1;
      if constexpr ((ABL & 16) != 0) {
        asm volatile("s_waitcnt lgkmcnt(0)" : "+v"(fa[0][0]), "+v"(fa[0][1]));
        fa[1][0] = fa[0][0]; fa[1][1] = fa[0][1];
      } else if constexpr (u + 1 < 2 * KS) {
        rd(std::integral_constant<int, u + 1>{}, t ^ 1);
        asm volatile("s_waitcnt lgkmcnt(2)" : "+v"(fa[t][0]), "+v"(fa[t][1]));
      } else {
        asm volatile("s_waitcnt lgkmcnt(0)" : "+v"(fa[t][0]), "+v"(fa[t][1]));
      }
#pragma unroll
      for (int cb = 0; cb < NCB; ++cb) {
        acc[r][cb] = mfma3_16(bw[cb][s][0], bw[cb][s][1], fa[t][0], fa[t][1], acc[r][cb]);
      }
      hook(uc);
    };
    [&]<int... U>(std::integer_sequence<int, U...>) __attribute__((always_inline)) {
      (unit(std::integral_constant<int, U>{}), ...);
    }(std::make_integer_sequence<int, 2 * KS>{});
  };

  const uint32_t ldo4 = (uint32_t)ldo * 4;
  f32x4 pend[NST];
  uint32_t soff[NST];
#pragma unroll
  for (int r = 0; r < 2; ++r) {
    if constexpr (NCB == 1) {
      soff[r] = (uint32_t)((16 * r + (lane & 15)) * ldo4) + (uint32_t)(col0 + 4 * (lane >> 4)) * 4;
    } else {
#pragma unroll
      for (int q = 0; q < NCB / 2; ++q) {
        const uint32_t off = (uint32_t)((16 * r + (lane & 7)) * ldo4) +
                             (uint32_t)(col0 + 32 * q + 16 * ((lane >> 3) & 1) + 4 * (lane >> 4)) * 4;
        soff[(q * 2 + r) * 2] = off;
        soff[(q * 2 + r) * 2 + 1] = off + 8 * ldo4;
      }
    }
  }
  __amdgpu_buffer_rsrc_t pending_rs = rsrc_of(out, M, ldo);
  f32x4 pend2[TWO ? NST : 1];
  __amdgpu_buffer_rsrc_t pending_act = rsrc_of(TWO ? act : out, M, ldo);
  auto flush = [&](int i) __attribute__((always_inline)) {
    if constexpr ((ABL & 4) == 0) {
      if (i < NST)
        __builtin_amdgcn_raw_buffer_store_b128(__builtin_bit_cast(u32x4, pend[i]), pending_rs, soff[i], 0, 2);
      else if constexpr (TWO)
        __builtin_amdgcn_raw_buffer_store_b128(__builtin_bit_cast(u32x4, pend2[i - NST]), pending_act,
                                               soff[i - NST], 0, 2);
    }
  };
  f32x4 prv[PRE ? 2 : 1][PRE ? NCB : 1];
  f32x4 csum[EPI == 2 ? NCB : 1];
  if constexpr (EPI == 2)
#pragma unroll
    for (int cb = 0; cb < NCB; ++cb) csum[cb] = f32x4{0.0f, 0.0f, 0.0f, 0.0f};
  auto load_pre = [&](int b) __attribute__((always_inline)) {
    if constexpr (PRE) {
      const auto rs = rsrc_of(pre, blk_r0(b), ldo);
#pragma unroll
      for (int r = 0; r < 2; ++r)
#pragma unroll
        for (int cb = 0; cb < NCB; ++cb)
          prv[r][cb] = __builtin_bit_cast(f32x4, __builtin_amdgcn_raw_buffer_load_b128(
              rs, (uint32_t)((16 * r + (lane & 15)) * ldo4) + (uint32_t)(col0 + 16 * cb + 4 * (lane >> 4)) * 4,
              0, 0));
      asm volatile("" ::: "memory");
    }
  };
  const uint32_t s_stats = sbase + CF::STATS;
  constexpr uint32_t kQ = 2 * RB * WAVES * 4;
  f32x4 gm{}, bt{};
  float lmu[2] = {0.0f, 0.0f}, lrs[2] = {0.0f, 0.0f};
  if constexpr (EPI == 3) {
    gm = *reinterpret_cast<const f32x4*>(ln.gamma + col0 + 4 * (lane >> 4));
    bt = *reinterpret_cast<const f32x4*>(ln.beta + col0 + 4 * (lane >> 4));
  }
  auto ln_part = [&](f32x4 sv, int ib, int r) __attribute__((always_inline)) {
    float m = ((sv[0] + sv[1]) + (sv[2] + sv[3])) * 0.25f;
    float q = 0.0f;
#pragma unroll
    for (int i = 0; i < 4; ++i) {
      const float d = sv[i] - m;
      q += d * d;
    }
#pragma unroll
    for (int o = 16, n2 = 2; o <= 32; o <<= 1, n2 <<= 1) {
      const float mo = __shfl_xor(m, o), qo = __shfl_xor(q, o);
      const float d = mo - m;
      m = (m + mo) * 0.5f;
      q = (q + qo) + (d * d) * (float)n2;
    }
    if (lane < 16) {
      const uint32_t a = s_stats + ((ib * RB + 16 * r + lane) * WAVES + wave) * 4;
      asm volatile("ds_write_b32 %0, %1" ::"v"(a), "v"(m) : "memory");
      asm volatile("ds_write_b32 %0, %1 offset:%2" ::"v"(a), "v"(q), "n"(kQ) : "memory");
    }
  };
  auto normalize = [&](int ibp) __attribute__((always_inline)) {
    f32x4 pm[2][2], pq[2][2];
#pragma unroll
    for (int r = 0; r < 2; ++r) {
      const uint32_t a = s_stats + ((ibp * RB + 16 * r + (lane & 15)) * WAVES) * 4;
      pm[r][0] = lds_read16<f32x4>(a);
      pm[r][1] = lds_read16o<16, f32x4>(a);
      pq[r][0] = lds_read16o<kQ, f32x4>(a);
      pq[r][1] = lds_read16o<kQ + 16, f32x4>(a);
    }
    asm volatile("s_waitcnt lgkmcnt(0)" : "+v"(pm[0][0]), "+v"(pm[0][1]), "+v"(pm[1][0]), "+v"(pm[1][1]),
                 "+v"(pq[0][0]), "+v"(pq[0][1]), "+v"(pq[1][0]), "+v"(pq[1][1]));
#pragma unroll
    for (int r = 0; r < 2; ++r) {
      const f32x4 m0 = pm[r][0], m1 = pm[r][1], q0 = pq[r][0], q1 = pq[r][1];
      const float mu = (((m0[0] + m0[1]) + (m0[2] + m0[3])) + ((m1[0] + m1[1]) + (m1[2] + m1[3]))) * 0.125f;
      float dev = 0.0f;
#pragma unroll
      for (int i = 0; i < 4; ++i) {
        const float d0 = m0[i] - mu, d1 = m1[i] - mu;
        dev += d0 * d0;
        dev += d1 * d1;
      }
      const float m2 = (((q0[0] + q0[1]) + (q0[2] + q0[3])) + ((q1[0] + q1[1]) + (q1[2] + q1[3]))) + dev * 16.0f;
      const float rs = 1.0f / sqrtf(m2 * (1.0f / (float)(8 * WC)) + ln.eps);
#pragma unroll
      for (int i = 0; i < 4; ++i) pend2[r][i] = (pend[r][i] - mu) * rs * gm[i] + bt[i];
      lmu[r] = mu;
      lrs[r] = rs;
    }
  };
  auto ln_store = [&](int bprev) __attribute__((always_inline)) {
    const int64_t r0 = bprev >= 0 ? blk_r0(bprev) : M;
    const bool mine = wave == 0 && r0 < M;
    const int64_t n = mine ? (M - r0 < RB ? M - r0 : RB) : 0;
    const uint32_t off = lane < RB ? (uint32_t)lane * 4 : 0x40000000u;
    const float* bases[2] = {ln.mean, ln.rstd};
    const float vals[2] = {lane < 16 ? lmu[0] : lmu[1], lane < 16 ? lrs[0] : lrs[1]};
#pragma unroll
    for (int k = 0; k < 2; ++k) {
      const uint64_t u = reinterpret_cast<uint64_t>(bases[k] + (mine ? r0 : 0));
      const uint64_t ub = (uint64_t)(uint32_t)__builtin_amdgcn_readfirstlane((uint32_t)u) |
                          ((uint64_t)(uint32_t)__builtin_amdgcn_readfirstlane((uint32_t)(u >> 32)) << 32);
      const auto rr = __builtin_amdgcn_make_buffer_rsrc(reinterpret_cast<void*>(ub), 0, (int)(n * 4), 0x00020000);
      __builtin_amdgcn_raw_buffer_store_b32(__float_as_uint(vals[k]), rr, off, 0, 0);
    }
  };
  auto finish = [&](int b, int ib) __attribute__((always_inline)) {
    const int64_t r0 = blk_r0(b);
    int er[2];
    er[0] = lds_read_i32(s_info + (ib * RB + (lane & 15)) * 4);
    er[1] = lds_read_i32(s_info + (ib * RB + 16 + (lane & 15)) * 4);
    constexpr int NG = NCB == 1 ? 1 : 2;
#pragma unroll
    for (int q = 0; q < NCB / NG; ++q) {
      i32x4 ec[NG];
      f32x4 bc[NG];
#pragma unroll
      for (int g = 0; g < NG; ++g) {
        const int cb = NG * q + g;
        ec[g] = lds_read16<i32x4>(s_cols + (wave * WC + cb * 16 + 4 * (lane >> 4)) * 4);
        if (BIAS) bc[g] = lds_read16<f32x4>(s_cols + (NT + wave * WC + cb * 16 + 4 * (lane >> 4)) * 4);
        else bc[g] = f32x4{0.0f, 0.0f, 0.0f, 0.0f};
      }
      if constexpr (NG == 1)
        asm volatile("s_waitcnt lgkmcnt(0)" : "+v"(er[0]), "+v"(er[1]), "+v"(ec[0]), "+v"(bc[0]));
      else
        asm volatile("s_waitcnt lgkmcnt(0)" : "+v"(er[0]), "+v"(er[1]), "+v"(ec[0]), "+v"(bc[0]),
                     "+v"(ec[1]), "+v"(bc[1]));
#pragma unroll
      for (int r = 0; r < 2; ++r) {
        f32x4 v[NG];
        f32x4 av[NG];
        const int64_t row = r0 + 16 * r + (lane & 15);
#pragma unroll
        for (int g = 0; g < NG; ++g) {
#pragma unroll
          for (int i = 0; i < 4; ++i) {
            v[g][i] = __builtin_amdgcn_ldexpf(acc[r][NG * q + g][i], er[r] + ec[g][i]);
            if (BIAS) v[g][i] += bc[g][i];
          }
          if constexpr (EPI != 0) {
            float mk[4];
            drop.get4(row * C + col0 + 16 * (NG * q + g) + 4 * (lane >> 4), mk);
            if constexpr (EPI == 1) {
#pragma unroll
              for (int i = 0; i < 4; ++i) av[g][i] = fsilu(v[g][i]) * mk[i];
            } else if constexpr (EPI == 2) {
              const f32x4 pv = prv[r][NG * q + g];
#pragma unroll
              for (int i = 0; i < 4; ++i) v[g][i] = (v[g][i] * mk[i]) * fdsilu(pv[i] + 0.0f);
              csum[NG * q + g] += v[g];
            } else {
              const f32x4 pv = prv[r][NG * q + g];
#pragma unroll
              for (int i = 0; i < 4; ++i) v[g][i] = v[g][i] * mk[i] + pv[i];
            }
          }
        }
        if constexpr (NG == 1) {
          pend[r] = v[0];
          if constexpr (EPI == 1) pend2[r] = av[0];
          if constexpr (EPI == 3) ln_part(v[0], ib, r);
        } else {
          f32x4 x1, x2;
#pragma unroll
          for (int i = 0; i < 4; ++i) {
            const float f0 = v[0][i], f1 = v[1][i];
            const int a0 = __float_as_int(f0), a1 = __float_as_int(f1);
            x1[i] = __int_as_float(__builtin_amdgcn_update_dpp(a0, a1, 0x128, 0xF, 0xC, false));
            x2[i] = __int_as_float(__builtin_amdgcn_update_dpp(a1, a0, 0x128, 0xF, 0x3, false));
          }
          pend[(q * 2 + r) * 2] = x1;
          pend[(q * 2 + r) * 2 + 1] = x2;
          if constexpr (EPI == 1) {
#pragma unroll
            for (int i = 0; i < 4; ++i) {
              const float f0 = av[0][i], f1 = av[1][i];
              const int a0 = __float_as_int(f0), a1 = __float_as_int(f1);
              x1[i] = __int_as_float(__builtin_amdgcn_update_dpp(a0, a1, 0x128, 0xF, 0xC, false));
              x2[i] = __int_as_float(__builtin_amdgcn_update_dpp(a1, a0, 0x128, 0xF, 0x3, false));
            }
            pend2[(q * 2 + r) * 2] = x1;
            pend2[(q * 2 + r) * 2 + 1] = x2;
          }
        }
      }
    }
    pending_rs = rsrc_of(out, r0, ldo);
    if constexpr (TWO) pending_act = rsrc_of(act, r0, ldo);
  };
  auto rmax_store = [&](int b, int ib) __attribute__((always_inline)) {
    const int64_t r0 = blk_r0(b);
    float x = 0.0f;
    if (lane < RB)
      asm volatile("ds_read_b32 %0, %1\n\ts_waitcnt lgkmcnt(0)" : "=v"(x) : "v"(s_info + (2 * RB + ib * RB + lane) * 4));
#pragma unroll
    for (int o = 32; o >= 1; o >>= 1) x = fmaxf(x, __shfl_xor(x, o));
    const bool mine = rmax != nullptr && ct == 0 && wave == 0 && r0 < M;
    const uint64_t u = reinterpret_cast<uint64_t>(rmax) + (mine ? (uint64_t)(r0 / RB) * 4 : 0);
    const uint64_t ub = (uint64_t)(uint32_t)__builtin_amdgcn_readfirstlane((uint32_t)u) |
                        ((uint64_t)(uint32_t)__builtin_amdgcn_readfirstlane((uint32_t)(u >> 32)) << 32);
    const auto rr = __builtin_amdgcn_make_buffer_rsrc(reinterpret_cast<void*>(ub), 0, mine ? 4 : 0, 0x00020000);
    __builtin_amdgcn_raw_buffer_store_b32(__float_as_uint(x), rr, 0, 0, 0);
  };

  [&]<int... P>(std::integer_sequence<int, P...>) __attribute__((always_inline)) {
    (issue(P, ra[CF::STG ? 0 : P], P), ...);
  }(std::make_integer_sequence<int, D>{});
  if constexpr (CF::STG) wait_vm<(D - 1) * NLD>();
  split(ra[0], 0, 0);
  if constexpr (EARLY1) {
    if (wave >= 4) issue(1, ra[0], 0);
  }
  asm volatile("s_waitcnt lgkmcnt(0)" ::: "memory");
  __builtin_amdgcn_s_barrier();

  auto loop = [&](auto late_c) __attribute__((always_inline)) {
    constexpr bool LATE = decltype(late_c)::value;
    constexpr int YS = (LATE ? D : D - 1) * NSO + D * NPRE + (D - 1) * NLD;
    constexpr int Y0 = (D - 1) * NLD + NPRE + (LATE ? NSO : 0);
    auto body = [&](int b, auto par) __attribute__((always_inline)) {
      constexpr int P = decltype(par)::value;
      const int ib = b & 1;
      auto do_split = [&]() __attribute__((always_inline)) {
        if constexpr (CF::STG) {
          if (b >= D - 1) wait_vm<(YS > 63 ? 63 : YS)>();
          else wait_vm<(Y0 > 63 ? 63 : Y0)>();
        }
        split(ra[CF::STG ? 0 : (P + 1) % D], ib ^ 1, (P + 1) % D);
      };
      if constexpr (EARLY1 && !LATE) {
        do_split();
        issue(b + 2, ra[0], 0);
        load_pre(b);
      } else {
        issue(b + D, ra[CF::STG ? 0 : P], P);
        load_pre(b);
        if constexpr (!LATE) do_split();
      }
      if constexpr (DEFER) {
        constexpr int U = 2 * KS, STEP = U / NSTT;
        static_assert(STEP >= 1, "more stores than MFMA units");
        if constexpr (EPI == 3) normalize(ib ^ 1);
        multiply(ib, [&](auto uc) __attribute__((always_inline)) {
          constexpr int u = decltype(uc)::value;
          if constexpr (u % STEP == 0 && u / STEP < NSTT) flush(u / STEP);
        });
        rmax_store(b, ib);
        if constexpr (EPI == 3) ln_store(b - 1);
        finish(b, ib);
      } else {
        multiply(ib, [](auto) __attribute__((always_inline)) {});
        finish(b, ib);
#pragma unroll
        for (int i = 0; i < NSTT; ++i) flush(i);
        rmax_store(b, ib);
      }
      if constexpr (LATE) do_split();
      asm volatile("s_waitcnt lgkmcnt(0)" ::: "memory");
      __builtin_amdgcn_s_barrier();
    };
    for (int b = 0; b < nb; b += D) {
      [&]<int... P>(std::integer_sequence<int, P...>) __attribute__((always_inline)) {
        (body(b + P, std::integral_constant<int, P>{}), ...);
      }(std::make_integer_sequence<int, D>{});
    }
  };
  if ((D == 1 && !EARLY1) || wave < 4) loop(std::true_type{});
  else loop(std::false_type{});
  if constexpr (DEFER) {
    const int blast = (nb + D - 1) / D * D - 1;
    if constexpr (EPI == 3) normalize(blast & 1);
#pragma unroll
    for (int i = 0; i < NSTT; ++i) flush(i);
    if constexpr (EPI == 3) ln_store(blast);
  }
  if constexpr (EPI == 2) {
#pragma unroll
    for (int cb = 0; cb < NCB; ++cb) {
#pragma unroll
      for (int i = 0; i < 4; ++i) {
        float x = csum[cb][i];
        x += dpp_xor1(x);
        x += dpp_xor2(x);
        x += __builtin_bit_cast(float, __builtin_amdgcn_mov_dpp(__builtin_bit_cast(int, x), 0x124, 0xF, 0xF, false));
        x += __builtin_bit_cast(float, __builtin_amdgcn_mov_dpp(__builtin_bit_cast(int, x), 0x128, 0xF, 0xF, false));
        csum[cb][i] = x;
      }
      if ((lane & 15) == 0)
        *reinterpret_cast<f32x4*>(dpart + prow * C + col0 + 16 * cb + 4 * (lane >> 4)) = csum[cb];
    }
  }
}

template <int K, int NCB, int D, bool BIAS, bool DEFER, int ABL, int EPI = 0>
void run(const float* A, int64_t lda, int64_t M, const void* Wi, const int* ew, int C,
         const float* bias, float* out, int64_t ldo, float* rmax, int grid, hipStream_t st,
         float* act = nullptr, DropSpec drop = DropSpec{}, const float* pre = nullptr,
         float* dpart = nullptr, LnSpec ln = LnSpec{}) {
  using CF = Cfg<K, NCB, D>;
  static bool done = false;
  if (!done) {
    (void)hipFuncSetAttribute((const void*)k_gemm_nt_ws<K, NCB, D, BIAS, DEFER, ABL, EPI>,
                              hipFuncAttributeMaxDynamicSharedMemorySize, CF::LDS);
    done = true;
  }
  k_gemm_nt_ws<K, NCB, D, BIAS, DEFER, ABL, EPI><<<grid, THREADS, CF::LDS, st>>>(
      A, lda, M, (const f16x8*)Wi, ew, C, bias, out, ldo, rmax, act, drop, pre, dpart, ln);
}

template <int K>
constexpr int depth() { return K == 512 ? 1 : K == 256 ? 2 : 3; }

inline int ncb_for(int K, int C) {
  int ncb = 16 / (K / 32);
  while (ncb > 1 && C % (128 * ncb)) ncb >>= 1;
  return C % (128 * ncb) ? 0 : ncb;
}

inline int grid_for(int64_t M, int C, int ncb) {
  const int nct = C / (128 * ncb);
  const int unit = 8 * nct;
  int grid = num_cus() / unit * unit;
  const int64_t items = (M + RB - 1) / RB * nct;
  if (items < grid) grid = (int)((items + unit - 1) / unit * unit);
  return grid;
}

}

bool nt_ws_ok(int64_t M, int K, int C, const float* A, int64_t lda, const float* out, int64_t ldo) {
  return (K == 128 || K == 256 || K == 512) && ws::ncb_for(K, C) > 0 && aligned16(A) &&
         lda % 4 == 0 && aligned16(out) && ldo % 4 == 0 && M > 0 &&
         (M + ws::RB - 1) / ws::RB <= 0x3fffffffLL;
}

int launch_gemm_nt_ws(const float* A, int64_t lda, int64_t M, int K, const void* Wf, int C,
                      const float* bias, float* out, int64_t ldo, float* rmax, hipStream_t st) {
  if (!nt_ws_ok(M, K, C, A, lda, out, ldo)) return fail("rb_gemm_nt_h: no weight-stationary launch for this shape");
  const WeightImage w = weight_image(Wf, C, K);
  const int ncb = ws::ncb_for(K, C);
  const int grid = ws::grid_for(M, C, ncb);
  dispatch_int<128, 256, 512>(K, [&](auto kc) {
    dispatch_int<1, 2, 4>(ncb, [&](auto nc) {
      dispatch_bool(bias != nullptr, [&](auto bias_c) {
        constexpr int KK = decltype(kc)::value, NC = decltype(nc)::value;
        if constexpr (NC <= 16 / (KK / 32))
          ws::run<KK, NC, ws::depth<KK>(), decltype(bias_c)::value, true, 0>(
              A, lda, M, w.wi, w.ew, C, bias, out, ldo, rmax, grid, st);
      });
    });
  });
  return launch_status("rb_gemm_nt_h");
}

bool nt_ws_act_ok(int64_t M, int K, int C, const float* A, int64_t lda, const float* out,
                  const float* other, int64_t ldo) {
  return K == 128 && C % 256 == 0 && nt_ws_ok(M, K, C, A, lda, out, ldo) && aligned16(other);
}

int launch_gemm_nt_ws_act(const float* A, int64_t lda, int64_t M, int K, const void* Wf, int C,
                          const float* bias, float* out, int64_t ldo, float* rmax, float* act,
                          DropSpec drop, hipStream_t st) {
  if (!nt_ws_act_ok(M, K, C, A, lda, out, act, ldo)) return fail("rb_gemm_nt_h_act: shape");
  const WeightImage w = weight_image(Wf, C, K);
  const int grid = ws::grid_for(M, C, 2);
  dispatch_bool(bias != nullptr, [&](auto bias_c) {
    ws::run<128, 2, ws::depth<128>(), decltype(bias_c)::value, true, 0, 1>(
        A, lda, M, w.wi, w.ew, C, bias, out, ldo, rmax, grid, st, act, drop);
  });
  return launch_status("rb_gemm_nt_h_act");
}

int launch_gemm_nt_ws_dact(const float* A, int64_t lda, int64_t M, int K, const void* Wf, int C,
                           float* out, int64_t ldo, float* rmax, const float* pre, DropSpec drop,
                           float* dpart, int64_t n_parts, hipStream_t st) {
  if (!nt_ws_act_ok(M, K, C, A, lda, out, pre, ldo)) return fail("rb_gemm_nt_h_dact: shape");
  const WeightImage w = weight_image(Wf, C, K);
  const int grid = ws::grid_for(M, C, 2);
  const int64_t used = grid / (C / 256);
  if (used > n_parts) return fail("rb_gemm_nt_h_dact: dpart has too few rows");
  ws::run<128, 2, ws::depth<128>(), false, true, 0, 2>(A, lda, M, w.wi, w.ew, C, nullptr, out, ldo, rmax, grid,
                                                      st, nullptr, drop, pre, dpart);
  const int rc = launch_status("rb_gemm_nt_h_dact");
  return rc ? rc : nt_dact_zero_rest(dpart, used, n_parts, C, st);
}

bool nt_ws_ln_ok(int64_t M, int K, int C, const float* A, int64_t lda, const float* y,
                 const float* s_out, const float* resid, int64_t ldo) {
  return C == 128 && nt_ws_ok(M, K, C, A, lda, y, ldo) && ws::ncb_for(K, C) == 1 &&
         aligned16(s_out) && aligned16(resid);
}

int launch_gemm_nt_ws_ln(const float* A, int64_t lda, int64_t M, int K, const void* Wf, int C,
                         const float* bias, const float* resid, DropSpec drop, const float* gamma,
                         const float* beta, float eps, float* y, float* s_out, float* mean,
                         float* rstd, int64_t ldo, float* rmax, hipStream_t st) {
  if (!nt_ws_ln_ok(M, K, C, A, lda, y, s_out, resid, ldo) || !gamma || !beta || !mean || !rstd ||
      !aligned16(gamma) || !aligned16(beta))
    return fail("rb_gemm_nt_h_ln: shape, alignment or null pointer");
  const WeightImage w = weight_image(Wf, C, K);
  const int grid = ws::grid_for(M, C, 1);
  ws::LnSpec ln;
  ln.gamma = gamma;
  ln.beta = beta;
  ln.eps = eps;
  ln.mean = mean;
  ln.rstd = rstd;
  dispatch_int<128, 256, 512>(K, [&](auto kc) {
    dispatch_bool(bias != nullptr, [&](auto bias_c) {
      constexpr int KK = decltype(kc)::value;
      ws::run<KK, 1, ws::depth<KK>(), decltype(bias_c)::value, true, 0, 3>(
          A, lda, M, w.wi, w.ew, C, bias, s_out, ldo, rmax, grid, st, y, drop, resid, nullptr, ln);
    });
  });
  return launch_status("rb_gemm_nt_h_ln");
}

}
```

datamining_recblr_amd/kernels.py:

```python
from __future__ import annotations

import contextlib
import ctypes

import torch

from . import _lib
from ._lib import RB_TILE, RecBLRNativeError

__all__ = [
    "scan_fwd", "scan_bwd", "conv_silu_fwd", "conv_silu_bwd", "gate_scan_fwd",
    "gate_scan_bwd", "num_tiles", "RecBLRNativeError", "kernel_timing", "KernelTimer",
    "item_ce_fwd", "item_ce_bwd", "item_ce_probs", "item_rank", "item_scores",
    "item_topk", "SplitRows", "item_split_h", "item_ce_fwd_h", "item_ce_probs_h",
    "embedding_bwd", "embedding_plan",
    "item_ce_fwd_h_rows", "item_ce_probs_h_rows", "item_ce_probs_h_both_rows",
    "next_item_targets", "next_item_targets_reference",
    "sample_negatives", "sample_negatives_reference", "philox4x32_10", "pair_loss_fwd",
    "pair_loss_bwd", "embedding_bwd_scaled", "pair_loss_supported",
    "candidate_scores", "candidate_topk", "candidate_ranks", "candidates_supported",
    "CANDIDATE_MAX", "CANDIDATE_EXCLUDE_MAX",
]


# ... 1128 lines not shown
            loss.data_ptr(), n_live.data_ptr(), ws.data_ptr(), ws_bytes, _stream(h))
    return loss, n_live, diff


def pair_loss_bwd(table: torch.Tensor, pos: torch.Tensor, neg: torch.Tensor, diff: torch.Tensor,
                  dloss: torch.Tensor, n_live: torch.Tensor, gamma: float):
    M, n = neg.shape
    V, d = table.shape
    dh = torch.empty((M, d), device=table.device, dtype=torch.float32)
    coef = torch.empty(((1 + n) * M,), device=table.device, dtype=torch.float32)
    _launch("rb_pair_loss_bwd", 4 * (2 + n) * M * d, table.data_ptr(), pos.data_ptr(),
            neg.data_ptr(), diff.data_ptr(), dloss.data_ptr(), n_live.data_ptr(), M, d, V, n,
            float(gamma), dh.data_ptr(), coef.data_ptr(), _stream(table))
    return dh, coef


def embedding_bwd_scaled(coef: torch.Tensor, src: torch.Tensor, num_rows: int, plan: torch.Tensor,
                         padding_idx=None):
    _check(coef, "coef")
    _check(src, "src")
    M = coef.numel()
    rows, d = src.shape
    if src.stride(1) != 1 or (d % 4 == 0 and (src.stride(0) % 4 or src.data_ptr() % 16)):
        src = src.contiguous()
    dw = torch.empty((num_rows, d), device=src.device, dtype=torch.float32)
    pad = -1 if padding_idx is None else int(padding_idx)
    _launch("rb_embedding_bwd_scaled", 4 * M * d + 4 * num_rows * d, src.data_ptr(), src.stride(0),
            rows, coef.contiguous().data_ptr(), M, d, num_rows, pad, dw.data_ptr(),
            plan.data_ptr(), plan.numel(), _stream(src), _fn="rb_embedding_bwd_apply_scaled")
    return dw


CANDIDATE_MAX = 4096
CANDIDATE_EXCLUDE_MAX = 4096
CANDIDATE_MAX_D = 512


def candidates_supported(h: torch.Tensor, table: torch.Tensor) -> bool:
    return (h.is_cuda and table.is_cuda and h.dtype == torch.float32
            and table.dtype == torch.float32 and h.dim() == 2 and table.dim() == 2
            and h.shape[1] == table.shape[1] and h.shape[1] % 4 == 0
            and 4 <= h.shape[1] <= CANDIDATE_MAX_D)


def _candidate_operands(h, table, cand):
    _check(h, "h")
    _check(table, "table")
    _check(cand, "candidates", torch.int64)
    if h.dim() != 2 or table.dim() != 2 or table.shape[1] != h.shape[1]:
        raise ValueError("candidates: h [B, d] and table [V, d] required")
    if cand.dim() != 2 or cand.shape[0] != h.shape[0]:
        raise ValueError(f"candidates must be [B, C], got {tuple(cand.shape)}")
    if h.stride(1) != 1 or h.stride(0) % 4 or h.data_ptr() % 16:
        h = h.contiguous()
    return h, table.contiguous(), cand.contiguous()


def candidate_scores(h: torch.Tensor, table: torch.Tensor, cand: torch.Tensor) -> torch.Tensor:
    h, table, cand = _candidate_operands(h, table, cand)
    (B, d), C, V = h.shape, cand.shape[1], table.shape[0]
    out = torch.empty((B, C), device=h.device, dtype=torch.float32)
    if B and C:
        _launch("rb_candidate_scores", 4 * (C + 1) * d * B, h.data_ptr(), h.stride(0),
                table.data_ptr(), cand.data_ptr(), B, C, d, V, out.data_ptr(), _stream(h))
    return out


def candidate_topk(h: torch.Tensor, table: torch.Tensor, cand: torch.Tensor, k: int,
                   first_item: int = 0, exclude: torch.Tensor | None = None):
    h, table, cand = _candidate_operands(h, table, cand)
    (B, d), C, V = h.shape, cand.shape[1], table.shape[0]
    k = int(k)
    if k < 1:
        raise ValueError(f"k = {k} must be positive")
    if not 1 <= C <= CANDIDATE_MAX:
        raise ValueError(f"C = {C} candidates per row: expected 1 .. {CANDIDATE_MAX}")
    E = 0
    if exclude is not None:
        _check(exclude, "exclude", torch.int64)
        if exclude.dim() != 2 or exclude.shape[0] != B:
            raise ValueError(f"exclude must be [B, E], got {tuple(exclude.shape)}")
        exclude = exclude.contiguous()
        E = exclude.shape[1]
        if E > CANDIDATE_EXCLUDE_MAX:
            raise ValueError(f"E = {E} excluded ids per row: at most {CANDIDATE_EXCLUDE_MAX}")
    ids = torch.empty((B, k), device=h.device, dtype=torch.int64)
    scores = torch.empty((B, k), device=h.device, dtype=torch.float32)
    if B:
        _launch("rb_candidate_topk", 4 * (C + 1) * d * B, h.data_ptr(), h.stride(0),
                table.data_ptr(), cand.data_ptr(), B, C, d, V, int(first_item), k,
                exclude.data_ptr() if E > 0 else None, E, ids.data_ptr(), scores.data_ptr(),
                _stream(h))
    return ids, scores


def candidate_ranks(h: torch.Tensor, table: torch.Tensor, target: torch.Tensor,
                    cand: torch.Tensor, first_item: int = 1):
    h, table, cand = _candidate_operands(h, table, cand)
    _check(target, "target", torch.int64)
    (B, d), C, V = h.shape, cand.shape[1], table.shape[0]
    if target.shape != (B,):
        raise ValueError(f"target must be [B], got {tuple(target.shape)}")
    if C < 1:
        raise ValueError("candidates must hold at least one id per row")
    gt = torch.empty((B,), device=h.device, dtype=torch.int64)
    eq = torch.empty((B,), device=h.device, dtype=torch.int64)
    if B:
        _launch("rb_candidate_ranks", 4 * (C + 2) * d * B, h.data_ptr(), h.stride(0),
                table.data_ptr(), target.contiguous().data_ptr(), cand.data_ptr(), B, C, d, V,
                int(first_item), gt.data_ptr(), eq.data_ptr(), _stream(h))
    return gt, eq


class _SplitJob(ctypes.Structure):
    _fields_ = [("W", ctypes.c_void_p), ("ldw", ctypes.c_int64), ("C", ctypes.c_int64),
                ("R", ctypes.c_int64), ("transpose", ctypes.c_int64), ("Wf", ctypes.c_void_p)]


MAX_SPLIT_JOBS = 32



def gemm_h_weight(w: torch.Tensor, transpose: bool = False) -> torch.Tensor:
    _check(w, "weight")
    if w.dim() != 2 or w.stride(1) != 1:
        raise ValueError("weight must be a 2-D row-major tensor")
    R, C = (w.shape[0], w.shape[1]) if transpose else (w.shape[1], w.shape[0])
    nbytes = _lib.load().rb_gemm_h_weight_bytes(C, R)
    wf = torch.empty(nbytes // 2, device=w.device, dtype=torch.float16)
    gemm_h_split_weights([(w, transpose, wf)])
    return wf


def gemm_h_split_weights(jobs) -> None:
    jobs = list(jobs)
    lib = _lib.load()
    for k in range(0, len(jobs), MAX_SPLIT_JOBS):
        chunk = jobs[k:k + MAX_SPLIT_JOBS]
        arr = (_SplitJob * len(chunk))()
        for d, (w, transpose, wf) in zip(arr, chunk):
            _check(w, "weight")
            if w.dim() != 2 or w.stride(1) != 1:
                raise ValueError("weight must be a 2-D row-major tensor")
            R, C = (w.shape[0], w.shape[1]) if transpose else (w.shape[1], w.shape[0])
            if wf.numel() * 2 != lib.rb_gemm_h_weight_bytes(C, R) or wf.device != w.device:
                raise ValueError("f16 weight image buffer does not match the weight")
            d.W, d.ldw, d.C, d.R = w.data_ptr(), w.stride(0), C, R
            d.transpose, d.Wf = int(transpose), wf.data_ptr()
        _lib.call("rb_gemm_h_split_weights", ctypes.addressof(arr), len(chunk),
                  _stream(chunk[0][0]))


def gemm_nt_h(a: torch.Tensor, wf: torch.Tensor, C: int, bias: torch.Tensor | None = None,
              out: torch.Tensor | None = None, rmax: torch.Tensor | None = None) -> torch.Tensor:
    _check(a, "a")
    if a.dim() != 2 or a.stride(1) != 1:
        raise ValueError("a must be a 2-D tensor with unit inner stride")
    M, R = a.shape
    if out is None:
        out = torch.empty((M, C), device=a.device, dtype=torch.float32)
    elif out.shape != (M, C) or out.stride(1) != 1:
        raise ValueError("out must be [M, C] with unit inner stride")
    if bias is not None:
        _check(bias, "bias")
    if rmax is not None:
        _check(rmax, "rmax")
        if rmax.numel() < (M + 31) // 32:
            raise ValueError("rmax needs ceil(M/32) entries")
    _lib.call("rb_gemm_nt_h", a.data_ptr(), a.stride(0), M, R, wf.data_ptr(), C,
              0 if bias is None else bias.data_ptr(), out.data_ptr(), out.stride(0), 0,
              0 if rmax is None else rmax.data_ptr(), _stream(a))
    return out


def gemm_nt_h_mode(mode: int = -1) -> int:
    return int(_lib.load().rb_gemm_nt_h_mode(int(mode)))


@contextlib.contextmanager
def nt_h_mode(mode: int):
    prev = gemm_nt_h_mode(mode)
    try:
        yield
    finally:
        gemm_nt_h_mode(prev)


def gemm_nt_h_ln_ok(a: torch.Tensor, C: int) -> bool:
    return (a.dim() == 2 and C == 128 and a.shape[1] in (128, 256, 512) and a.stride(1) == 1
            and a.stride(0) % 4 == 0 and a.data_ptr() % 16 == 0 and gemm_nt_h_mode() == 1)


def gemm_nt_h_ln(a: torch.Tensor, wf: torch.Tensor, C: int, bias: torch.Tensor | None,
                 resid: torch.Tensor, gamma: torch.Tensor, beta: torch.Tensor, eps: float,
                 seed: int, p: float, rmax: torch.Tensor | None = None):
    _check(a, "a")
    _check(resid, "resid")
    _check_p(p)
    if not gemm_nt_h_ln_ok(a, C):
        raise ValueError(f"gemm_nt_h_ln: no fused launch for {tuple(a.shape)} -> {C}")
    M, R = a.shape
    if resid.shape != (M, C) or not resid.is_contiguous():
        raise ValueError("resid must be a contiguous [M, C] tensor")
    for t, n in ((gamma, "gamma"), (beta, "beta")):
        _check(t, n)
        if t.numel() != C or t.data_ptr() % 16:
            raise ValueError(f"{n} must hold C floats, 16-byte aligned")
    if bias is not None:
        _check(bias, "bias")
    if rmax is not None:
        _check(rmax, "rmax")
        if rmax.numel() < (M + 31) // 32:
            raise ValueError("rmax needs ceil(M/32) entries")
    y = torch.empty((M, C), device=a.device, dtype=torch.float32)
    s = torch.empty_like(y)
    mean = torch.empty(M, device=a.device, dtype=torch.float32)
    rstd = torch.empty_like(mean)
    _lib.call("rb_gemm_nt_h_ln", a.data_ptr(), a.stride(0), M, R, wf.data_ptr(), C,
              0 if bias is None else bias.data_ptr(), resid.data_ptr(), gamma.data_ptr(),
              beta.data_ptr(), float(eps), int(seed), float(p), y.data_ptr(), s.data_ptr(),
              mean.data_ptr(), rstd.data_ptr(), y.stride(0),
              0 if rmax is None else rmax.data_ptr(), _stream(a))
    return y, s, mean, rstd


def gemm_nt_h_act_ok(a: torch.Tensor, C: int) -> bool:
    M, R = a.shape
    return C % 256 == 0 and C <= 1024 and R % 32 == 0 and R <= 1024 and not (
        M <= 4096 and (R > 256 or C < 256))


def gemm_nt_h_act(a: torch.Tensor, wf: torch.Tensor, C: int, bias: torch.Tensor | None,
                  seed: int, p: float, rmax: torch.Tensor | None = None):
    _check(a, "a")
    _check_p(p)
    if a.dim() != 2 or a.stride(1) != 1:
        raise ValueError("a must be a 2-D tensor with unit inner stride")
    if not gemm_nt_h_act_ok(a, C):
        raise ValueError(f"gemm_nt_h_act: no fused launch for {tuple(a.shape)} -> {C}")
    M, R = a.shape
    out = torch.empty((M, C), device=a.device, dtype=torch.float32)
    act = torch.empty_like(out)
    if bias is not None:
        _check(bias, "bias")
    if rmax is not None:
        _check(rmax, "rmax")
        if rmax.numel() < (M + 31) // 32:
            raise ValueError("rmax needs ceil(M/32) entries")
    _lib.call("rb_gemm_nt_h_act", a.data_ptr(), a.stride(0), M, R, wf.data_ptr(), C,
              0 if bias is None else bias.data_ptr(), out.data_ptr(), out.stride(0),
              0 if rmax is None else rmax.data_ptr(), act.data_ptr(), int(seed), float(p),
              _stream(a))
    return out, act


_dact_parts = None


def gemm_nt_h_dact(a: torch.Tensor, wf: torch.Tensor, C: int, pre: torch.Tensor, seed: int,
                   p: float, rmax: torch.Tensor | None = None, want_dbias: bool = True):
    global _dact_parts
    _check(a, "a")
    _check(pre, "pre")
    _check_p(p)
    if a.dim() != 2 or a.stride(1) != 1:
        raise ValueError("a must be a 2-D tensor with unit inner stride")
    M, R = a.shape
    if not gemm_nt_h_act_ok(a, C) or C > 512:
        raise ValueError(f"gemm_nt_h_dact: no fused launch for {tuple(a.shape)} -> {C}")
    if pre.shape != (M, C) or not pre.is_contiguous():
        raise ValueError("pre must be a contiguous [M, C] tensor")
    if rmax is not None:
        _check(rmax, "rmax")
        if rmax.numel() < (M + 31) // 32:
            raise ValueError("rmax needs ceil(M/32) entries")
    if _dact_parts is None:
        _dact_parts = int(_lib.load().rb_gemm_nt_h_dact_parts())
    out = torch.empty((M, C), device=a.device, dtype=torch.float32)
    part = torch.empty((_dact_parts, C), device=a.device, dtype=torch.float32)
    _lib.call("rb_gemm_nt_h_dact", a.data_ptr(), a.stride(0), M, R, wf.data_ptr(), C,
              out.data_ptr(), out.stride(0), 0 if rmax is None else rmax.data_ptr(),
              pre.data_ptr(), int(seed), float(p), part.data_ptr(), _dact_parts, _stream(a))
    return out, (colsum(part) if want_dbias else None)


def gemm_tn_h(dy: torch.Tensor, x: torch.Tensor, ymax: torch.Tensor, xmax: torch.Tensor,
              splits: int) -> torch.Tensor:
    for t, n in ((dy, "dy"), (x, "x"), (ymax, "ymax"), (xmax, "xmax")):
        _check(t, n)
    if dy.dim() != 2 or x.dim() != 2 or dy.stride(1) != 1 or x.stride(1) != 1:
        raise ValueError("dy and x must be 2-D with unit inner stride")
    M, N = dy.shape
    K = x.shape[1]
    if x.shape[0] != M:
        raise ValueError("dy and x must have the same rows")
    if ymax.numel() < (M + 31) // 32 or xmax.numel() < (M + 31) // 32:
        raise ValueError("ymax / xmax need ceil(M/32) entries")
    parts = torch.empty((splits, N, K), device=dy.device, dtype=torch.float32)
    _lib.call("rb_gemm_tn_h", dy.data_ptr(), dy.stride(0), x.data_ptr(), x.stride(0), M, N, K,
              ymax.data_ptr(), xmax.data_ptr(), parts.data_ptr(), splits, _stream(dy))
    return parts


def bf16_weight_image(w: torch.Tensor, transpose: bool = False) -> torch.Tensor:
    _check(w, "w")
    if w.dim() != 2 or w.stride(1) != 1:
        raise ValueError("w must be a 2-D tensor with unit inner stride")
    C, R = (w.shape[1], w.shape[0]) if transpose else (w.shape[0], w.shape[1])
    img = torch.empty(C * R, device=w.device, dtype=torch.bfloat16)
    _lib.call("rb_gemm_bf16_weight_image", w.data_ptr(), w.stride(0), C, R, int(transpose),
              img.data_ptr(), _stream(w))
    return img


def gemm_nt_bf16(a: torch.Tensor, img: torch.Tensor, C: int,
                 bias: torch.Tensor | None = None) -> torch.Tensor:
    _check(a, "a", torch.bfloat16)
    _check(img, "img", torch.bfloat16)
    if a.dim() != 2 or a.stride(1) != 1:
        raise ValueError("a must be a 2-D tensor with unit inner stride")
    M, R = a.shape
    if img.numel() != C * R:
        raise ValueError("img does not match a [M, R] operand with C outputs")
    if bias is not None:
        _check(bias, "bias")
    out = torch.empty((M, C), device=a.device, dtype=torch.bfloat16)
    _lib.call("rb_gemm_nt_bf16", a.data_ptr(), a.stride(0), M, R, img.data_ptr(), C,
              0 if bias is None else bias.data_ptr(), out.data_ptr(), out.stride(0), _stream(a))
    return out


def gemm_tn_hs(dy: torch.Tensor, x: torch.Tensor, out: torch.Tensor | None = None,
               accumulate: bool = False) -> torch.Tensor:
    for t, n in ((dy, "dy"), (x, "x")):
        _check(t, n)
    if dy.dim() != 2 or x.dim() != 2 or dy.stride(1) != 1 or x.stride(1) != 1:
        raise ValueError("dy and x must be 2-D with unit inner stride")
    M, N = dy.shape
    K = x.shape[1]
    if x.shape[0] != M:
        raise ValueError("dy and x must have the same rows")
    if out is None:
        out = torch.empty((N, K), device=dy.device, dtype=torch.float32)
        accumulate = False
    elif out.shape != (N, K) or not out.is_contiguous() or out.dtype != torch.float32:
        raise ValueError("out must be a contiguous fp32 [N, K] tensor")
    _lib.call("rb_gemm_tn_hs", dy.data_ptr(), dy.stride(0), x.data_ptr(), x.stride(0), M, N, K,
              out.data_ptr(), int(accumulate), _stream(dy))
    return out


def grl_pieces(lens_packed: torch.Tensor, offs: torch.Tensor, G: int) -> torch.Tensor:
    B = lens_packed.numel()
    k = torch.arange(B)
    r, j = k // G, k % G
    span_of = torch.where(r % 2 == 0, j, G - 1 - j)
    order = torch.sort(span_of, stable=True).indices
    counts = torch.bincount(span_of, minlength=G)
    span = torch.zeros(G + 1, dtype=torch.int64)
    torch.cumsum(counts, 0, out=span[1:])
    return torch.cat([offs[:-1][order], lens_packed[order], order, span]).to(torch.int32)


def grl_max_tiles(lens_packed: torch.Tensor, G: int) -> int:
    B = lens_packed.numel()
    k = torch.arange(B)
    r, j = k // G, k % G
    span_of = torch.where(r % 2 == 0, j, G - 1 - j)
    rows = torch.zeros(G, dtype=torch.int64).index_add_(0, span_of, lens_packed.to(torch.int64))
    return max(1, (int(rows.max()) + 63) // 64)


def grl_fwd(xz, conv_w, conv_b, wg_img, gate_b, lam, h0, seq: Packed, want_y=True,
            want_train=True, tile_carries=False):
    for t, n in ((xz, "xz"), (conv_w, "conv weight"), (conv_b, "conv bias"),
                 (gate_b, "gates bias"), (lam, "Lambda")):
        _check(t, n)
    ntok, H2 = xz.shape
    H = H2 // 2
    if seq.pieces is None or xz.stride(1) != 1 or ntok != seq.ntok:
        raise ValueError("grl_fwd needs packed sequences with their work lists")
    kc = conv_w.shape[-1]
    cw = conv_w.reshape(H, kc).contiguous()
    dev = xz.device
    y = torch.empty((ntok, H), device=dev) if want_y else None
    y_last = None if want_y else torch.empty((seq.B, H), device=dev)
    carries = xc = rg = rmax = tc = None
    nT = num_tiles(seq.L)
    if want_train and tile_carries:
        if seq.max_tiles <= 0:
            raise ValueError("tile_carries needs seq.max_tiles (grl_max_tiles)")
        tc = torch.empty((seq.G, seq.max_tiles, H), device=dev)
    elif want_train:
        carries = torch.empty((seq.B, nT, H), device=dev)
        xc = torch.empty((ntok, H), device=dev)
        rg = torch.empty((ntok, 2 * H), device=dev)
        rmax = torch.zeros((ntok + 31) // 32, device=dev)
    nbytes = (2 + (1 if want_y else 0) + (3 if xc is not None else 0)) * ntok * H * 4
    _launch("rb_grl_fwd", nbytes, xz.data_ptr(), xz.stride(0), cw.data_ptr(), kc,
            conv_b.contiguous().data_ptr(), wg_img.data_ptr(), gate_b.contiguous().data_ptr(),
            lam.contiguous().data_ptr(), 0 if h0 is None else h0.contiguous().data_ptr(),
            seq.pieces.data_ptr(), seq.B, seq.G, ntok, H,
            0 if y is None else y.data_ptr(), H, 0 if y_last is None else y_last.data_ptr(),
            0 if xc is None else xc.data_ptr(), 0 if rg is None else rg.data_ptr(),
            0 if carries is None else carries.data_ptr(), nT,
            0 if rmax is None else rmax.data_ptr(), _ptr(tc), seq.max_tiles if tc is not None else 0,
            _stream(xz), _exp=True)
    if tc is not None:
        carries = tc
    return (y if want_y else y_last), carries, xc, rg, rmax


def grl_bwd(xz, conv_w, conv_b, wg_img, wgt_img, gate_b, lam, h0, seq: Packed, tile_carries,
            dy, last_only=False, want_rmax=False):
    for t, n in ((xz, "xz"), (conv_w, "conv weight"), (conv_b, "conv bias"),
                 (gate_b, "gates bias"), (lam, "Lambda"), (dy, "dy")):
        _check(t, n)
    ntok, H2 = xz.shape
    H = H2 // 2
    if seq.pieces is None or xz.stride(1) != 1 or ntok != seq.ntok:
        raise ValueError("grl_bwd needs packed sequences with their work lists")
    if tile_carries.shape != (seq.G, seq.max_tiles, H) or not tile_carries.is_contiguous():
        raise ValueError("tile_carries shape mismatch")
    want = (seq.B, H) if last_only else (ntok, H)
    if tuple(dy.shape) != want or not dy.is_contiguous():
        raise ValueError(f"dy must be a contiguous fp32 {list(want)}")
    kc = conv_w.shape[-1]
    cw = conv_w.reshape(H, kc).contiguous()
    dev = xz.device
    dxz = torch.empty((ntok, H2), device=dev)
    drg = torch.empty((ntok, H2), device=dev)
    xc = torch.empty((ntok, H), device=dev)
    nr = (ntok + 31) // 32
    rmax = torch.zeros(2 * nr, device=dev) if want_rmax else None
    part = torch.empty((seq.G, 4, H), device=dev)
    cpart = torch.empty((seq.G * 8, H * kc + H), device=dev)
    nbytes = (2 + (0 if last_only else 1) + 5) * ntok * H * 4
    _launch("rb_grl_bwd", nbytes, xz.data_ptr(), xz.stride(0), cw.data_ptr(), kc,
            conv_b.contiguous().data_ptr(), wg_img.data_ptr(), wgt_img.data_ptr(),
            gate_b.contiguous().data_ptr(), lam.contiguous().data_ptr(), _ptr(h0),
            seq.pieces.data_ptr(), seq.B, seq.G, ntok, H, tile_carries.data_ptr(), seq.max_tiles,
            0 if last_only else dy.data_ptr(), dy.data_ptr() if last_only else 0,
            dxz.data_ptr(), H2, drg.data_ptr(), xc.data_ptr(),
            0 if rmax is None else rmax.data_ptr(), 0 if rmax is None else rmax[nr:].data_ptr(),
            part.data_ptr(), cpart.data_ptr(), _stream(xz), _exp=True)
    sums = colsum(part.view(seq.G, 4 * H)).view(4, H)
    csum = colsum(cpart)
    return (dxz, drg, xc, None if rmax is None else rmax[:nr], None if rmax is None else rmax[nr:],
            sums[0], sums[1:3].reshape(-1), sums[3], csum[:H * kc].view(H, kc), csum[H * kc:])
```

datamining_recblr_amd/linear.py:

```python
from __future__ import annotations

import os
import weakref

import torch

from . import _lib, gemm_tuning, kernels

__all__ = ["linear", "wgrad", "LinearFn", "mm_nt", "mm_nn", "split_gemm_enabled",
           "HipLinearForward", "has_hooks", "fire_hooks"]

_GEMM = os.environ.get("RECBLR_GEMM", "f16x3")
if _GEMM not in ("f16x3", "torch"):
    raise ValueError(f"RECBLR_GEMM must be f16x3 or torch, got {_GEMM!r}")
_split_on = os.environ.get("RECBLR_SPLIT_GEMM", "1") != "0" and _GEMM != "torch"
_half = _GEMM == "f16x3"
_tn_on = os.environ.get("RECBLR_TN", "1") != "0"
_cache_on = os.environ.get("RECBLR_SPLIT_CACHE", "1") != "0"
_small_tn = os.environ.get("RECBLR_SMALL_TN", "0") == "1"

_split_cache: dict = {}
_opt_steps = [0]
_cache_check = os.environ.get("RECBLR_SPLIT_CACHE_CHECK", "0") == "1"


class StaleSplitCacheError(RuntimeError):
    """A cached split weight image no longer matches its weight."""


def _count_step(*_args, **_kw):
    _opt_steps[0] += 1


try:
    from torch.optim.optimizer import register_optimizer_step_post_hook
except ImportError:
    register_optimizer_step_post_hook = None
if register_optimizer_step_post_hook is not None:
    register_optimizer_step_post_hook(_count_step)


def invalidate_split_cache() -> None:
    _split_cache.clear()
    _bf16_cache.clear()


def _stamp(w: torch.Tensor):
    return (w._version, _opt_steps[0])


def _make_image(w, transpose):
    return kernels.gemm_h_weight(w, transpose=transpose)


def _weight_split(w: torch.Tensor, transpose: bool) -> torch.Tensor:
    _apply_nt_ws()
    if not _cache_on:
        return _make_image(w, transpose)
    key = (id(w), transpose)
    e = _split_cache.get(key)
    if e is not None and e[0]() is w and e[1] == w.data_ptr() and e[2] == _stamp(w):
        if _cache_check and not torch.equal(e[3], _make_image(w, transpose)):
            raise StaleSplitCacheError(
                "cached split image of a weight is stale: the weight was rewritten without "
                "a torch.optim step or a version bump; call linear.invalidate_split_cache()")
        return e[3]
    if e is None or e[0]() is not w or e[1] != w.data_ptr():
        wf = _make_image(w, transpose)
        _split_cache[key] = [weakref.ref(w), w.data_ptr(), _stamp(w), wf]
        return wf
    jobs, fresh = [], []
    for k, ent in list(_split_cache.items()):
        ww = ent[0]()
        if ww is None or ww.data_ptr() != ent[1]:
            del _split_cache[k]
            continue
        if _stamp(ww) != ent[2] and ww.device == w.device:
            jobs.append((ww, k[1], ent[3]))
            fresh.append(ent)
    kernels.gemm_h_split_weights(jobs)
    for ent in fresh:
        ent[2] = _stamp(ent[0]())
    return e[3]


def split_gemm_enabled() -> bool:
    return _split_on


HALF_MIN_ROWS = 1


def _split_ok(a: torch.Tensor, C: int, R: int) -> bool:
    return (_split_on and _half and a.is_cuda and a.dim() == 2 and a.shape[0] >= HALF_MIN_ROWS
            and C % 32 == 0 and R % 32 == 0 and a.stride(1) == 1 and a.stride(0) % 4 == 0
            and a.data_ptr() % 16 == 0 and a.dtype == torch.float32 and C <= 1024)


def gemm_format() -> str:
    return _GEMM if _split_on else "torch"


_NT_WS = os.environ.get("RECBLR_NT_WS", "1")
if _NT_WS not in ("0", "1"):
    raise ValueError(f"RECBLR_NT_WS must be 0 or 1, got {_NT_WS!r}")
_nt_ws_applied = None


def _apply_nt_ws() -> None:
    global _nt_ws_applied
    if _nt_ws_applied != _NT_WS:
        _lib.load().rb_gemm_nt_h_mode(int(_NT_WS))
        _nt_ws_applied = _NT_WS


def set_nt_ws(on: bool) -> bool:
    global _NT_WS
    prev = _NT_WS == "1"
    _NT_WS = "1" if on else "0"
    _apply_nt_ws()
    return prev


def rmax_wanted() -> bool:
    return _half and _tn_on and _split_on


def rmax_buffer(a: torch.Tensor, C: int, R: int) -> torch.Tensor | None:
    if _half and _tn_on and _split_ok(a, C, R):
        return torch.empty((a.shape[0] + 31) // 32, device=a.device, dtype=torch.float32)
    return None


BF16_NT_MAX_R = 512
BF16_NT_MIN_ROWS = 65536
_BF16_MODES = ("auto", "1", "0")
_bf16_gemm = os.environ.get("RECBLR_BF16_GEMM", "auto")
if _bf16_gemm not in _BF16_MODES:
    raise ValueError(f"RECBLR_BF16_GEMM must be one of {_BF16_MODES}, got {_bf16_gemm!r}")
_bf16_cache: dict = {}


def set_bf16_gemm(mode) -> str:
    global _bf16_gemm
    m = {True: "1", False: "0"}.get(mode, mode) if isinstance(mode, bool) else str(mode)
    if m not in _BF16_MODES:
        raise ValueError(f"bf16 GEMM mode must be one of {_BF16_MODES}, got {mode!r}")
    prev, _bf16_gemm = _bf16_gemm, m
    return prev


def _bf16_image(w: torch.Tensor, transpose: bool) -> torch.Tensor:
    key = (id(w), transpose)
    e = _bf16_cache.get(key)
    if (_cache_on and e is not None and e[0]() is w and e[1] == w.data_ptr()
            and e[2] == _stamp(w)):
        return e[3]
    img = kernels.bf16_weight_image(w, transpose)
    if _cache_on:
        for k in [k for k, v in _bf16_cache.items() if v[0]() is None]:
            del _bf16_cache[k]
        _bf16_cache[key] = (weakref.ref(w), w.data_ptr(), _stamp(w), img)
    return img


def _bf16_ok(a: torch.Tensor, w: torch.Tensor, C: int, R: int) -> bool:
    return (_bf16_gemm != "0"
            and (_bf16_gemm == "1" or (R <= BF16_NT_MAX_R and a.shape[0] >= BF16_NT_MIN_ROWS))
            and a.dtype == torch.bfloat16 and w.dtype == torch.float32 and a.is_cuda
            and a.dim() == 2 and a.shape[0] > 0 and a.stride(1) == 1 and a.stride(0) % 8 == 0
            and a.data_ptr() % 16 == 0 and w.stride(1) == 1 and R % 64 == 0 and C % 256 == 0)


def mm_nt(a: torch.Tensor, w: torch.Tensor, bias: torch.Tensor | None = None,
          rmax: torch.Tensor | None = None) -> torch.Tensor:
    if a.dtype != w.dtype and _bf16_ok(a, w, w.shape[0], w.shape[1]):
        b = None if bias is None else bias.contiguous()
        return kernels.gemm_nt_bf16(a, _bf16_image(w, False), w.shape[0], bias=b)
    if a.dtype != w.dtype:
        wb = w.to(a.dtype)
        return torch.addmm(bias.to(a.dtype), a, wb.t()) if bias is not None else a @ wb.t()
    N, K = w.shape
    if _split_ok(a, N, K):
        return kernels.gemm_nt_h(a, _weight_split(w, False), N, bias=bias, rmax=rmax)
    return torch.addmm(bias, a, w.t()) if bias is not None else torch.mm(a, w.t())


_act_fused = os.environ.get("RECBLR_FFN_ACT", "1") != "0"
ACT_MIN_ROWS = 16384


def set_ffn_act_fused(on: bool) -> bool:
    global _act_fused
    prev, _act_fused = _act_fused, bool(on)
    return prev


def mm_nt_act_ok(a: torch.Tensor, w: torch.Tensor) -> bool:
    N, K = w.shape
    return (_act_fused and _half and a.dtype == w.dtype and a.shape[0] >= ACT_MIN_ROWS
            and _split_ok(a, N, K) and kernels.gemm_nt_h_act_ok(a, N))


def mm_nt_act(a: torch.Tensor, w: torch.Tensor, bias: torch.Tensor | None, seed: int, p: float,
              rmax: torch.Tensor | None = None):
    return kernels.gemm_nt_h_act(a, _weight_split(w, False), w.shape[0], bias, seed, p, rmax=rmax)


_ln_fused = os.environ.get("RECBLR_LN_EPI", "1") != "0"
if os.environ.get("RECBLR_LN_EPI", "1") not in ("0", "1"):
    raise ValueError("RECBLR_LN_EPI must be 0 or 1")


def set_ln_fused(on: bool) -> bool:
    global _ln_fused
    prev, _ln_fused = _ln_fused, bool(on)
    return prev


def mm_nt_ln_ok(a: torch.Tensor, w: torch.Tensor) -> bool:
    N, K = w.shape
    if not (_ln_fused and _half and a.dtype == w.dtype and a.shape[0] >= ACT_MIN_ROWS
            and _split_ok(a, N, K)):
        return False
    _apply_nt_ws()
    return kernels.gemm_nt_h_ln_ok(a, N)


def mm_nt_ln(a: torch.Tensor, w: torch.Tensor, bias: torch.Tensor | None, resid: torch.Tensor,
             gamma: torch.Tensor, beta: torch.Tensor, eps: float, seed: int, p: float,
             rmax: torch.Tensor | None = None):
    return kernels.gemm_nt_h_ln(a, _weight_split(w, False), w.shape[0], bias, resid, gamma, beta,
                                eps, seed, p, rmax=rmax)


def mm_nn_dact_ok(dy: torch.Tensor, w: torch.Tensor) -> bool:
    N, K = w.shape
    return (_act_fused and _half and dy.dtype == w.dtype and K <= 512
            and dy.shape[0] >= ACT_MIN_ROWS and _split_ok(dy, K, N)
            and kernels.gemm_nt_h_act_ok(dy, K))


def mm_nn_dact(dy: torch.Tensor, w: torch.Tensor, pre: torch.Tensor, seed: int, p: float,
               rmax: torch.Tensor | None = None):
    return kernels.gemm_nt_h_dact(dy, _weight_split(w, True), w.shape[1], pre, seed, p,
                                  rmax=rmax)


def mm_nn(dy: torch.Tensor, w: torch.Tensor, out: torch.Tensor | None = None,
          rmax: torch.Tensor | None = None) -> torch.Tensor:
    if dy.dtype != w.dtype and out is None and _bf16_ok(dy, w, w.shape[1], w.shape[0]):
        return kernels.gemm_nt_bf16(dy, _bf16_image(w, True), w.shape[1])
    if dy.dtype != w.dtype:
        wb = w.to(dy.dtype)
        return out.addmm_(dy, wb) if out is not None else dy @ wb
    N, K = w.shape
    if _split_ok(dy, K, N):
        r = kernels.gemm_nt_h(dy, _weight_split(w, True), K, rmax=rmax)
        return r if out is None else out.add_(r)
    if out is not None:
        return out.addmm_(dy, w)
    return torch.mm(dy, w)


SPLIT_K = 64
MIN_ROWS_FOR_SPLIT = 16384
TN_FEW_MIN_ROWS = 2048
_tn_few = os.environ.get("RECBLR_TN_FEW", "1") != "0"


_ncus = {}


def _tn_splits(dev, nt: int) -> int:
    n = _ncus.get(dev)
    if n is None:
        n = _ncus[dev] = torch.cuda.get_device_properties(dev).multi_processor_count
    return max(8, (2 * n // nt) // 8 * 8)


def wgrad(dy2: torch.Tensor, x2: torch.Tensor, splits: int = SPLIT_K,
          ymax: torch.Tensor | None = None, xmax: torch.Tensor | None = None) -> torch.Tensor:
    M = dy2.shape[0]
    N, K = dy2.shape[1], x2.shape[1]
    if (ymax is not None and xmax is not None
            and (M >= MIN_ROWS_FOR_SPLIT or (_tn_few and M >= TN_FEW_MIN_ROWS))
            and N % 128 == 0
            and K % 128 == 0 and dy2.stride(1) == 1 and x2.stride(1) == 1
            and dy2.stride(0) % 4 == 0 and x2.stride(0) % 4 == 0
            and dy2.data_ptr() % 16 == 0 and x2.data_ptr() % 16 == 0):
        S = _tn_splits(dy2.device, (N // 128) * (K // 128))
        if M < MIN_ROWS_FOR_SPLIT:
            S = max(8, min(S, M // 32 // 8 * 8))
        parts = kernels.gemm_tn_h(dy2, x2, ymax, xmax, S)
        return kernels.colsum(parts.view(S, -1)).view(N, K)
    if (_small_tn and _half and _split_on and _tn_on and M < MIN_ROWS_FOR_SPLIT and N % 32 == 0
            and K % 32 == 0 and dy2.dtype == torch.float32 and x2.dtype == torch.float32
            and dy2.is_cuda and dy2.stride(1) == 1 and x2.stride(1) == 1):
        return kernels.gemm_tn_hs(dy2, x2)
    if M < MIN_ROWS_FOR_SPLIT or splits <= 1:
        return (dy2.t() @ x2).float()
    mk = M // splits
    main = mk * splits
    a = dy2[:main].unflatten(0, (splits, mk)).transpose(1, 2)
    b = x2[:main].unflatten(0, (splits, mk))
    parts = torch.empty((splits + (main < M), N, K), device=dy2.device, dtype=dy2.dtype)
    torch.bmm(a, b, out=parts[:splits])
    if main < M:
        torch.mm(dy2[main:].t(), x2[main:], out=parts[splits])
    if parts.dtype != torch.float32:
        parts = parts.float()
    return kernels.colsum(parts.view(parts.shape[0], -1)).view(N, K)


def _label(fn, args) -> str:
    name = getattr(fn, "__name__", "gemm")
    if name in ("mm_nt", "mm_nn", "mm_nt_act", "mm_nn_dact") and len(args) >= 2:
        a, w = args[0], args[1]
        n_out = w.shape[1] if name.startswith("mm_nn") else w.shape[0]
        return f"{name}[{a.shape[0]}x{a.shape[1]}->{n_out}]"
    if name == "wgrad" and len(args) >= 2:
        return f"wgrad[{args[0].shape[0]}:{args[0].shape[1]}x{args[1].shape[1]}]"
    return name


def _timed(kind, flops, fn, *args, **kw):
    t = kernels._timer
    if t is None or t.only is not None:
        return fn(*args, **kw)
    e0 = torch.cuda.Event(enable_timing=True)
    e1 = torch.cuda.Event(enable_timing=True)
    e0.record()
    out = fn(*args, **kw)
    e1.record()
    t.records.append((kind, flops, e0, e1))
    t.detail.append((_label(fn, args), flops, e0, e1))
    return out


class LinearFn(torch.autograd.Function):
    @staticmethod
    def forward(ctx, x, weight, bias, slot=None):
        x2 = x.reshape(-1, x.shape[-1])
        flops = 2 * x2.shape[0] * x2.shape[1] * weight.shape[0]
        rx = rmax_buffer(x2, weight.shape[0], weight.shape[1]) if ctx.needs_input_grad[1] else None
        y = _timed("gemm", flops, mm_nt, x2, weight, bias, rmax=rx)
        ctx.rx = rx
        ctx.save_for_backward(x2, weight)
        ctx.has_bias = bias is not None
        ctx.slot = slot
        return y.view(*x.shape[:-1], weight.shape[0])

    @staticmethod
    def backward(ctx, dy):
        x2, weight = ctx.saved_tensors
        dy2 = dy.reshape(-1, dy.shape[-1])
        flops = 2 * x2.shape[0] * x2.shape[1] * weight.shape[0]
        dx = dw = db = None
        ry = None
        if ctx.needs_input_grad[0]:
            slot = ctx.slot
            ry = rmax_buffer(dy2, weight.shape[1], weight.shape[0]) if ctx.rx is not None else None
            dx = _timed("gemm", flops, mm_nn, dy2, weight, rmax=ry)
            if slot is not None and slot.ds is not None:
                if slot.rows is not None:
                    dx.index_add_(0, slot.rows, slot.ds.view(-1, weight.shape[1]))
                    slot.ds = None
                elif not slot.taken:
                    dx.add_(slot.ds.view(-1, weight.shape[1]))
                    slot.ds = None
            dx = dx.view(*dy.shape[:-1], weight.shape[1])
        if ctx.needs_input_grad[1]:
            dw = _timed("gemm", flops, wgrad, dy2, x2, ymax=ry, xmax=ctx.rx)
        if ctx.has_bias and ctx.needs_input_grad[2]:
            db = (kernels.colsum(dy2.contiguous()) if dy2.dtype == torch.float32
                  else dy2.sum(0, dtype=torch.float32))
        return dx, dw, db, None


def has_hooks(module: torch.nn.Module) -> bool:
    g = torch.nn.modules.module
    return bool(module._forward_hooks or module._forward_pre_hooks
                or g._global_forward_hooks or g._global_forward_pre_hooks)


def fire_hooks(module: torch.nn.Module, args: tuple, output) -> None:
    g = torch.nn.modules.module
    for hook in (*g._global_forward_pre_hooks.values(), *module._forward_pre_hooks.values()):
        if hook(module, args) is not None:
            raise NotImplementedError(
                "a forward pre-hook that modifies the input of a Linear fused into a RecBLR "
                "HIP kernel is not supported")
    for hook in (*g._global_forward_hooks.values(), *module._forward_hooks.values()):
        if hook(module, args, output) is not None:
            raise NotImplementedError(
                "a forward hook that replaces the output of a Linear fused into a RecBLR "
                "HIP kernel is not supported")


class HipLinearForward:

    def __init__(self, module: torch.nn.Linear):
        self.module = module

    def __call__(self, x: torch.Tensor) -> torch.Tensor:
        m = self.module
        slot = m.__dict__.get("_recblr_slot")
        m.__dict__["_recblr_slot"] = None
        return linear(x, m, slot)


def linear(x: torch.Tensor, module: torch.nn.Linear, slot=None) -> torch.Tensor:
    if _tuned is None and x.is_cuda:
        _load_tuned()
    return LinearFn.apply(x, module.weight, module.bias, slot)


_tuned = None


def _load_tuned():
    global _tuned
    _tuned = gemm_tuning.use_tuned_gemms()
```

include/recblr_hip.h:

```cpp
#ifndef RECBLR_HIP_H
#define RECBLR_HIP_H

#include <stddef.h>
#include <stdint.h>

#ifdef __cplusplus
extern "C" {
#endif

#define RB_EINVAL (-1)

typedef uint16_t rb_bf16;

#define RB_TILE 16

#define RB_ABI_VERSION 49
int rb_version(void);

const char* rb_last_error_string(void);

int rb_num_kernels(void);

int rb_scan_fwd(const float* gates, const float* tokens, float* states,
                int64_t B, int64_t C, int64_t T, void* stream);

int rb_scan_bwd(const float* gates, const float* states, const float* grad,
                float* d_gates, float* d_tokens,
                int64_t B, int64_t C, int64_t T, void* stream);

int rb_conv_silu_fwd(const float* x, int64_t x_rs, const float* w,
                     const float* bias, float* xc, int64_t xc_rs,
                     int64_t B, int64_t L, int64_t H, int64_t K, const int64_t* seq_offsets, void* stream);

int rb_conv_silu_fwd_rows(const float* x, int64_t x_rs, const float* w, const float* bias,
                          float* xc, int64_t xc_rs, int64_t ntok, int64_t H, int64_t K,
                          const int64_t* row_pos, void* stream);

int rb_conv_silu_bwd(const float* x, int64_t x_rs, const float* w,
                     const float* bias, const float* g1, const float* g2,
                     float* dx, int64_t dx_rs, float* dw_part, float* db_part,
                     int64_t B, int64_t L, int64_t H, int64_t K, const int64_t* seq_offsets, void* stream);

int rb_gate_scan_fwd(const float* rg, int64_t rg_rs, const float* xc,
                     int64_t xc_rs, const float* z, int64_t z_rs,
                     const float* lam, const float* gate_b, const float* h0,
                     int64_t h0_bs, float* y, int64_t y_rs, float* carries,
                     int64_t B, int64_t L, int64_t H, const int64_t* seq_offsets, void* stream);

int rb_gate_scan_bwd(const float* rg, int64_t rg_rs, const float* xc,
                     int64_t xc_rs, const float* z, int64_t z_rs,
                     const float* lam, const float* gate_b, const float* carries,
                     const float* dy,
                     float* drg, int64_t drg_rs, float* dxc, int64_t dxc_rs,
                     float* dz, int64_t dz_rs, float* part, float* dh0_part,
                     int64_t B, int64_t L, int64_t H, const int64_t* seq_offsets, void* stream);

int rb_gate_scan_fwd_last(const float* rg, int64_t rg_rs, const float* xc, int64_t xc_rs,
                          const float* z, int64_t z_rs, const float* lam, const float* gate_b,
                          const float* h0, int64_t h0_bs, float* y_last, float* carries,
                          int64_t B, int64_t L, int64_t H, const int64_t* seq_offsets,
                          const int64_t* batch_row, void* stream);
int rb_gate_scan_bwd_last(const float* rg, int64_t rg_rs, const float* xc, int64_t xc_rs,
                          const float* z, int64_t z_rs, const float* lam, const float* gate_b,
                          const float* carries, const float* dy_last, float* drg,
                          int64_t drg_rs, float* dxc, int64_t dxc_rs, float* dz, int64_t dz_rs,
                          float* part, float* dh0_part, int64_t B, int64_t L, int64_t H,
                          const int64_t* seq_offsets, const int64_t* batch_row, void* stream);

int rb_pad_prefix_fwd(const float* conv_b, const float* gate_w, const float* gate_b,
                      const float* lam, const int64_t* pad, int64_t pad_len, int64_t n_rows,
                      int64_t H, float* h0, float* workspace, void* stream);

int rb_pad_prefix_bwd(const float* conv_b, const float* gate_w, const float* gate_b,
                      const float* lam, const int64_t* pad, int64_t pad_len, int64_t n_rows,
                      int64_t H, const float* dh0, float* dconv_b, float* dgate_w,
                      float* dgate_b, float* dlam, float* workspace, int accumulate,
                      void* stream);



int rb_add_ln_fwd(const float* a, const int64_t* idx, int64_t n_idx_rows,
                  const uint8_t* mask, uint64_t seed, float p, const float* r,
                  const float* gamma, const float* beta, float eps, float* y,
                  float* s_out, float* mean, float* rstd, int64_t rows,
                  int64_t d, void* stream);

int64_t rb_row_num_parts(int64_t rows, int64_t width);

int rb_add_ln_bwd(const float* dy, const float* s, const float* gamma,
                  const float* mean, const float* rstd, const uint8_t* mask,
                  uint64_t seed, float p, float* ds, float* da,
                  float* dgamma_part, float* dbeta_part, float* dbias_part,
                  int64_t n_parts, int64_t rows, int64_t d, void* stream);
int rb_add_ln_bwd2(const float* dy, const float* dy2, const float* s, const float* gamma,
                   const float* mean, const float* rstd, const uint8_t* mask,
                   uint64_t seed, float p, float* ds, float* da,
                   float* dgamma_part, float* dbeta_part, float* dbias_part,
                   int64_t n_parts, int64_t rows, int64_t d, void* stream);

int rb_silu_dropout_fwd(const float* a, const float* bias, const uint8_t* mask,
                        uint64_t seed, float p, float* u, int64_t rows,
                        int64_t cols, void* stream);
int rb_silu_dropout_bwd(const float* a, const float* bias, const uint8_t* mask,
                        uint64_t seed, float p, const float* du, float* da,
                        float* dbias_part, int64_t n_parts, int64_t rows,
                        int64_t cols, void* stream);

int rb_dropout_mask(uint64_t seed, float p, uint8_t* out, int64_t n,
                    void* stream);

int64_t rb_embedding_bwd_workspace(int64_t M, int64_t V, int64_t d);
int rb_embedding_bwd(const int64_t* idx, const float* grad, int64_t M, int64_t d,
                     int64_t V, int64_t padding_idx, float* dweight,
                     void* workspace, int64_t workspace_bytes, void* stream);

int rb_embedding_bwd_plan(const int64_t* idx, int64_t M, int64_t d, int64_t V,
                          void* workspace, int64_t workspace_bytes, void* stream);
int rb_embedding_bwd_apply(const float* grad, int64_t M, int64_t d, int64_t V,
                           int64_t padding_idx, float* dweight, void* workspace,
                           int64_t workspace_bytes, void* stream);

int rb_colsum(const float* in, int64_t M, int64_t P, int64_t C, int64_t rs, int64_t ms,
              float* out, void* stream);

int rb_colsum_chunked(const float* in, int64_t M, int64_t P, int64_t C, int64_t rs,
                      int64_t chunk_rows, float* part, uint32_t* counters, int64_t n_counters,
                      float* out, void* stream);


int64_t rb_item_ce_workspace(int64_t B, int64_t V, int64_t d);

int rb_item_ce_fwd(const float* seq, const float* items, const int64_t* target, int64_t B,
                   int64_t V, int64_t d, float* lse, float* loss, void* workspace,
                   int64_t workspace_bytes, void* stream);

int rb_item_ce_bwd(const float* seq, const float* items, const int64_t* target, const float* lse,
                   const float* dloss, int64_t B, int64_t V, int64_t d, float* dseq,
                   float* ditems, void* workspace, int64_t workspace_bytes, void* stream);

int rb_item_ce_probs(const float* seq, const float* items, const int64_t* target,
                     const float* lse, const float* dloss, int64_t B, int64_t V, int64_t d,
                     int64_t item_offset, float* probs, int64_t ld, void* stream);

int rb_item_split_h(const float* x, int64_t n, int64_t d, void* image, int* exps,
                    float* group_max, void* stream);

int rb_item_ce_fwd_h(const void* seq_img, const int* seq_exp, const void* item_img,
                     const int* item_exp, const int64_t* target, int64_t B, int64_t V, int64_t d,
                     float* lse, float* loss, void* workspace, int64_t workspace_bytes,
                     void* stream);

int rb_item_ce_probs_h(const void* seq_img, const int* seq_exp, const void* item_img,
                       const int* item_exp, const int64_t* target, const float* lse,
                       const float* dloss, int64_t B, int64_t V, int64_t d, int64_t item_offset,
                       float* probs, int64_t ld, void* stream);

int rb_item_ce_probs_h_t(const void* seq_img, const int* seq_exp, const void* item_img,
                         const int* item_exp, const int64_t* target, const float* lse,
                         const float* dloss, int64_t B, int64_t V, int64_t d, int64_t item_offset,
                         float* probs_t, int64_t ldt, float* group_max, void* stream);

int rb_item_ce_probs_h_both(const void* seq_img, const int* seq_exp, const void* item_img,
                            const int* item_exp, const int64_t* target, const float* lse,
                            const float* dloss, int64_t B, int64_t V, int64_t d,
                            int64_t item_offset, float* probs, int64_t ld, float* probs_t,
                            int64_t ldt, float* row_group_max, float* item_group_max,
                            void* stream);

int rb_group_absmax(const float* x, int64_t n, int64_t c, int64_t ld, float* out, void* stream);
// ... 109 lines not shown
```

Before: 393,600.

## Emit per-32-row column maxima in forward/dgrad GEMMs to pre-settle wgrad column scales

```diff
diff --git a/datamining_recblr_amd/_lib.py b/datamining_recblr_amd/_lib.py
--- a/datamining_recblr_amd/_lib.py
+++ b/datamining_recblr_amd/_lib.py
@@ -75,6 +75,8 @@
                                                   "recblr_pairs.h")))
 CANDIDATE_SIGNATURES = parse_header(_read(os.path.join(os.path.dirname(HEADER_PATH),
                                                        "recblr_candidates.h")))
+COLSCALE_SIGNATURES = parse_header(_read(os.path.join(os.path.dirname(HEADER_PATH),
+                                                      "recblr_colscale.h")))
 EXP_SIGNATURES = parse_header(_read(os.path.join(_HERE, "experimental", "recblr_exp.h")))
 PROBE_SIGNATURES = parse_header(_read(os.path.join(_HERE, "probes", "recblr_probe.h")))
 SESSION_SIGNATURES = parse_header(_read(os.path.join(_HERE, "session", "recblr_session.h")))
@@ -108,7 +110,8 @@
 
 def load(path: str | None = None) -> ctypes.CDLL:
     return _load(path or LIB_PATH,
-                 {**SIGNATURES, **DENSE_SIGNATURES, **PAIR_SIGNATURES, **CANDIDATE_SIGNATURES},
+                 {**SIGNATURES, **DENSE_SIGNATURES, **PAIR_SIGNATURES, **CANDIDATE_SIGNATURES,
+                  **COLSCALE_SIGNATURES},
                  "HIP extension not built",
                  "rb_version",
                  "ABI mismatch: library {} vs binding {}; rebuild", cache=path is None,
diff --git a/datamining_recblr_amd/build.py b/datamining_recblr_amd/build.py
--- a/datamining_recblr_amd/build.py
+++ b/datamining_recblr_amd/build.py
@@ -13,7 +13,8 @@
     os.path.join(ROOT, "include", "recblr_hip.h"),
     os.path.join(ROOT, "include", "recblr_dense.h"),
     os.path.join(ROOT, "include", "recblr_pairs.h"),
-    os.path.join(ROOT, "include", "recblr_candidates.h")]
+    os.path.join(ROOT, "include", "recblr_candidates.h"),
+    os.path.join(ROOT, "include", "recblr_colscale.h")]
 OUT = os.path.join(_HERE, "lib", "libdmrecblr.so")
 PROBE_SOURCES = sorted(glob.glob(os.path.join(_HERE, "probes", "*.hip")))
 PROBE_HEADERS = HEADERS + sorted(glob.glob(os.path.join(_HERE, "probes", "*.h")))
diff --git a/datamining_recblr_amd/csrc/capi.hip b/datamining_recblr_amd/csrc/capi.hip
--- a/datamining_recblr_amd/csrc/capi.hip
+++ b/datamining_recblr_amd/csrc/capi.hip
@@ -889,20 +889,43 @@
   return launch_split_weights_h(jobs, (int)n, reinterpret_cast<hipStream_t>(stream));
 }
 
+static int nt_h_args(const char* who, const float* A, int64_t lda, int64_t M, int64_t R,
+                     const void* Wf, int64_t C, const float* out, int64_t ldo, int accumulate) {
+  if (!A || !Wf || !out) return fail(who, "null pointer");
+  if (M <= 0 || R <= 0 || C <= 0) return fail(who, "empty shape");
+  if (accumulate) return fail(who, "accumulate is not supported (add the residual in its consumer)");
+  if (R % 32 || C % 32 || R > (1 << 16) || C > 1024)
+    return fail(who, "R and C must be multiples of 32 (C <= 1024)");
+  if (lda < R || lda % 4 || ldo < C || ldo % 2) return fail(who, "bad row strides");
+  if (!aligned16(A) || !aligned16(Wf) || (reinterpret_cast<uintptr_t>(out) & 7))
+    return fail(who, "A and Wf must be 16-byte aligned, out 8-byte aligned");
+  if ((M + 31) / 32 > 0x7fffffffLL) return fail(who, "grid too large");
+  return 0;
+}
+
 int rb_gemm_nt_h(const float* A, int64_t lda, int64_t M, int64_t R, const void* Wf, int64_t C,
                  const float* bias, float* out, int64_t ldo, int accumulate, float* rmax,
                  void* stream) {
-  if (!A || !Wf || !out) return fail("rb_gemm_nt_h: null pointer");
-  if (M <= 0 || R <= 0 || C <= 0) return fail("rb_gemm_nt_h: empty shape");
-  if (accumulate) return fail("rb_gemm_nt_h: accumulate is not supported (add the residual in its consumer)");
-  if (R % 32 || C % 32 || R > (1 << 16) || C > 1024)
-    return fail("rb_gemm_nt_h: R and C must be multiples of 32 (C <= 1024)");
-  if (lda < R || lda % 4 || ldo < C || ldo % 2) return fail("rb_gemm_nt_h: bad row strides");
-  if (!aligned16(A) || !aligned16(Wf) || (reinterpret_cast<uintptr_t>(out) & 7))
-    return fail("rb_gemm_nt_h: A and Wf must be 16-byte aligned, out 8-byte aligned");
-  if ((M + 31) / 32 > 0x7fffffffLL) return fail("rb_gemm_nt_h: grid too large");
+  if (const int rc = nt_h_args("rb_gemm_nt_h", A, lda, M, R, Wf, C, out, ldo, accumulate)) return rc;
   return launch_gemm_nt_h(A, lda, M, (int)R, Wf, (int)C, bias, out, ldo, accumulate, rmax,
                           reinterpret_cast<hipStream_t>(stream));
+}
+
+int rb_gemm_nt_h_cmax_ok(const float* A, int64_t lda, int64_t M, int64_t R, int64_t C,
+                         const float* out, int64_t ldo) {
+  return R > 0 && R <= 512 && C > 0 && C <= 1024 && gemm_nt_h_cmax_ok(A, lda, M, (int)R, (int)C, out, ldo);
+}
+
+int rb_gemm_nt_h_cmax(const float* A, int64_t lda, int64_t M, int64_t R, const void* Wf, int64_t C,
+                      const float* bias, float* out, int64_t ldo, float* rmax, float* cmax,
+                      void* stream) {
+  if (const int rc = nt_h_args("rb_gemm_nt_h_cmax", A, lda, M, R, Wf, C, out, ldo, 0)) return rc;
+  if (!cmax || !aligned16(cmax)) return fail("rb_gemm_nt_h_cmax: cmax must be a 16-byte aligned buffer");
+  if (!rb_gemm_nt_h_cmax_ok(A, lda, M, R, C, out, ldo))
+    return fail("rb_gemm_nt_h_cmax: this call would not run on the weight-stationary kernel, "
+                "the only one that writes cmax (rb_gemm_nt_h_cmax_ok)");
+  return launch_gemm_nt_h(A, lda, M, (int)R, Wf, (int)C, bias, out, ldo, 0, rmax,
+                          reinterpret_cast<hipStream_t>(stream), cmax);
 }
 
 int rb_gemm_nt_h_act(const float* A, int64_t lda, int64_t M, int64_t R, const void* Wf, int64_t C,
@@ -960,22 +983,42 @@
                                reinterpret_cast<hipStream_t>(stream));
 }
 
+static int tn_h_args(const char* who, const float* dY, int64_t ldy, const float* X, int64_t ldx,
+                     int64_t M, int64_t N, int64_t K, const float* ymax, const float* xmax,
+                     const float* parts, int64_t splits) {
+  if (!dY || !X || !ymax || !xmax || !parts) return fail(who, "null pointer");
+  if (M <= 0 || N <= 0 || K <= 0) return fail(who, "empty shape");
+  if (N % 128 || K % 128 || N > 65536 || K > 65536)
+    return fail(who, "N and K must be multiples of 128 (<= 65536)");
+  if (splits < 1 || splits > 65536) return fail(who, "splits must be in [1, 65536]");
+  if (ldy < N || ldx < K || ldy % 4 || ldx % 4) return fail(who, "bad row strides");
+  if (!aligned16(dY) || !aligned16(X)) return fail(who, "dY and X must be 16-byte aligned");
+  if ((N / 128) * (K / 128) * splits > 0x7fffffffLL) return fail(who, "grid too large");
+  const int64_t mk = ((M + splits - 1) / splits + 31) / 32 * 32;
+  if (mk * (ldy > ldx ? ldy : ldx) * 4 >= 0x7fffffffLL)
+    return fail(who, "a row chunk spans 2 GiB or more (use more splits)");
+  return 0;
+}
+
 int rb_gemm_tn_h(const float* dY, int64_t ldy, const float* X, int64_t ldx, int64_t M, int64_t N,
                  int64_t K, const float* ymax, const float* xmax, float* parts, int64_t splits,
                  void* stream) {
-  if (!dY || !X || !ymax || !xmax || !parts) return fail("rb_gemm_tn_h: null pointer");
-  if (M <= 0 || N <= 0 || K <= 0) return fail("rb_gemm_tn_h: empty shape");
-  if (N % 128 || K % 128 || N > 65536 || K > 65536)
-    return fail("rb_gemm_tn_h: N and K must be multiples of 128 (<= 65536)");
-  if (splits < 1 || splits > 65536) return fail("rb_gemm_tn_h: splits must be in [1, 65536]");
-  if (ldy < N || ldx < K || ldy % 4 || ldx % 4) return fail("rb_gemm_tn_h: bad row strides");
-  if (!aligned16(dY) || !aligned16(X)) return fail("rb_gemm_tn_h: dY and X must be 16-byte aligned");
-  if ((N / 128) * (K / 128) * splits > 0x7fffffffLL) return fail("rb_gemm_tn_h: grid too large");
-  const int64_t mk = ((M + splits - 1) / splits + 31) / 32 * 32;
-  if (mk * (ldy > ldx ? ldy : ldx) * 4 >= 0x7fffffffLL)
-    return fail("rb_gemm_tn_h: a row chunk spans 2 GiB or more (use more splits)");
+  if (const int rc = tn_h_args("rb_gemm_tn_h", dY, ldy, X, ldx, M, N, K, ymax, xmax, parts, splits))
+    return rc;
   return launch_gemm_tn_h(dY, ldy, X, ldx, M, (int)N, (int)K, ymax, xmax, parts, (int)splits,
                           reinterpret_cast<hipStream_t>(stream));
+}
+
+int rb_gemm_tn_h_cmax(const float* dY, int64_t ldy, const float* X, int64_t ldx, int64_t M,
+                      int64_t N, int64_t K, const float* ymax, const float* xmax,
+                      const float* ycmax, const float* xcmax, float* parts, int64_t splits,
+                      void* stream) {
+  if (const int rc = tn_h_args("rb_gemm_tn_h_cmax", dY, ldy, X, ldx, M, N, K, ymax, xmax, parts, splits))
+    return rc;
+  if (!ycmax || !xcmax || !aligned16(ycmax) || !aligned16(xcmax))
+    return fail("rb_gemm_tn_h_cmax: ycmax and xcmax must be 16-byte aligned buffers");
+  return launch_gemm_tn_h(dY, ldy, X, ldx, M, (int)N, (int)K, ymax, xmax, parts, (int)splits,
+                          reinterpret_cast<hipStream_t>(stream), ycmax, xcmax);
 }
 
 int rb_gemm_bf16_weight_image(const float* W, int64_t ldw, int64_t C, int64_t R, int transpose,
diff --git a/datamining_recblr_amd/csrc/common.h b/datamining_recblr_amd/csrc/common.h
--- a/datamining_recblr_amd/csrc/common.h
+++ b/datamining_recblr_amd/csrc/common.h
@@ -11,6 +11,7 @@
 #include "../../include/recblr_dense.h"
 #include "../../include/recblr_pairs.h"
 #include "../../include/recblr_candidates.h"
+#include "../../include/recblr_colscale.h"
 
 namespace rb {
 
@@ -349,7 +350,7 @@
                         const float* bias, void* out, int64_t ldo, hipStream_t st);
 int launch_gemm_tn_h(const float* Y, int64_t ldy, const float* X, int64_t ldx, int64_t M, int N,
                      int K, const float* ymax, const float* xmax, float* parts, int S,
-                     hipStream_t st);
+                     hipStream_t st, const float* ycmax = nullptr, const float* xcmax = nullptr);
 constexpr int kWeightScale = 14;
 template <class S>
 struct WeightSlot {
@@ -381,8 +382,11 @@
 int nt_dact_zero_rest(float* dpart, int64_t used, int64_t n_parts, int C, hipStream_t st);
 bool nt_ws_ok(int64_t M, int K, int C, const float* A, int64_t lda, const float* out, int64_t ldo);
 int launch_gemm_nt_ws(const float* A, int64_t lda, int64_t M, int K, const void* Wf, int C,
-                      const float* bias, float* out, int64_t ldo, float* rmax, hipStream_t st);
+                      const float* bias, float* out, int64_t ldo, float* rmax, float* cmax,
+                      hipStream_t st);
 int gemm_nt_h_mode(int mode);
+bool gemm_nt_h_cmax_ok(const float* A, int64_t lda, int64_t M, int R, int C, const float* out,
+                       int64_t ldo);
 bool nt_ws_act_ok(int64_t M, int K, int C, const float* A, int64_t lda, const float* out,
                   const float* other, int64_t ldo);
 int launch_gemm_nt_ws_act(const float* A, int64_t lda, int64_t M, int K, const void* Wf, int C,
@@ -399,7 +403,7 @@
                          float* rstd, int64_t ldo, float* rmax, hipStream_t st);
 int launch_gemm_nt_h(const float* A, int64_t lda, int64_t M, int R, const void* Wf, int C,
                      const float* bias, float* out, int64_t ldo, int accumulate, float* rmax,
-                     hipStream_t st);
+                     hipStream_t st, float* cmax = nullptr);
 int launch_gemm_nt_h_act(const float* A, int64_t lda, int64_t M, int R, const void* Wf, int C,
                          const float* bias, float* out, int64_t ldo, float* rmax, float* act,
                          DropSpec drop, hipStream_t st);
diff --git a/datamining_recblr_amd/csrc/gemm_half.hip b/datamining_recblr_amd/csrc/gemm_half.hip
--- a/datamining_recblr_amd/csrc/gemm_half.hip
+++ b/datamining_recblr_amd/csrc/gemm_half.hip
@@ -728,7 +728,9 @@
                                         int64_t ldx, int64_t M, int N, int K,
                                         const float* __restrict__ ymax,
                                         const float* __restrict__ xmax, float* __restrict__ parts,
-                                        int S, int64_t mk, int nt_k) {
+                                        int S, int64_t mk, int nt_k,
+                                        const float* __restrict__ ycmax = nullptr,
+                                        const float* __restrict__ xcmax = nullptr) {
   using CF = TnCfg<NBN, NBK>;
   const int tid = threadIdx.x;
   const int lane = tid & 63;
@@ -769,6 +771,50 @@
   const int ey = exp_of(my), ex = exp_of(mx);
   __syncthreads();
 
+  bool settled = false;
+  if constexpr (!PERCOL) {
+    if (ycmax != nullptr && xcmax != nullptr && (r_begin & 31) == 0) {
+      settled = true;
+      constexpr int NCOL = CF::YC + CF::XC, NCG = NCOL / 4, NPH = CF::THREADS / NCG;
+      static_assert(NPH >= 1 && (NPH * NCOL + 1) * 4 <= CF::STAGE, "column maxima fit one stage");
+      float* s_cm = reinterpret_cast<float*>(smem + CF::STAGE);
+      int* s_redo = reinterpret_cast<int*>(smem + CF::STAGE) + NPH * NCOL;
+      if (tid == 0) *s_redo = 0;
+      const int ph = tid / NCG, c4 = 4 * (tid % NCG);
+      if (ph < NPH) {
+        const bool isy = c4 < CF::YC;
+        const int64_t ldc = isy ? N : K;
+        const float* p = (isy ? ycmax + n0 + c4 : xcmax + k0 + (c4 - CF::YC)) + (r_begin / 32) * ldc;
+        f32x4 m{0.0f, 0.0f, 0.0f, 0.0f};
+#pragma unroll 4
+        for (int g = ph; g < T; g += NPH) {
+          const f32x4 v = *reinterpret_cast<const f32x4*>(p + g * ldc);
+#pragma unroll
+          for (int i = 0; i < 4; ++i) m[i] = fmaxf(m[i], v[i]);
+        }
+        *reinterpret_cast<f32x4*>(s_cm + ph * NCOL + c4) = m;
+      }
+      __syncthreads();
+      for (int col = tid; col < NCOL; col += CF::THREADS) {
+        float m = s_cm[col];
+#pragma unroll
+        for (int q = 1; q < NPH; ++q) m = fmaxf(m, s_cm[q * NCOL + col]);
+        const int ec = col < CF::YC ? ey : ex;
+        if (m > 0.0f && m < __builtin_amdgcn_ldexpf(1.0f, ec - 16)) *s_redo = 1;
+        const int e = exp_of(m);
+        const int slot = col < CF::YC ? col * T_PITCH : 2 * CF::YPLANE + (col - CF::YC) * T_PITCH;
+        *reinterpret_cast<int*>(smem + slot + 64) = e;
+      }
+      __syncthreads();
+      const int redo = *s_redo;
+      __syncthreads();
+      if (redo != 0) {
+        tn_percol<NBN, NBK>(smem, Y, ldy, X, ldx, M, N, K, ymax, xmax, parts, S, mk, nt_k);
+        return;
+      }
+    }
+  }
+
   const bool loader = tid < CF::LOADERS;
   const int op = tid < CF::YC ? 0 : 1;
   const int lt = op == 0 ? tid : tid - CF::YC;
@@ -918,7 +964,7 @@
 
   constexpr int NCOL = CF::YC + CF::XC;
   constexpr int pass = PERCOL ? 1 : 0;
-  if constexpr (!PERCOL) {
+  if constexpr (!PERCOL) if (!settled) {
     __syncthreads();
     float* s_cm = reinterpret_cast<float*>(smem + CF::STAGE);
     int* s_redo = reinterpret_cast<int*>(smem + CF::STAGE) + 4 * NCOL;
@@ -989,9 +1035,10 @@
 k_gemm_tn_h(const float* __restrict__ Y, int64_t ldy, const float* __restrict__ X, int64_t ldx,
             int64_t M, int N, int K, const float* __restrict__ ymax,
             const float* __restrict__ xmax, float* __restrict__ parts, int S, int64_t mk,
-            int nt_k) {
+            int nt_k, const float* __restrict__ ycmax, const float* __restrict__ xcmax) {
   extern __shared__ __attribute__((aligned(16))) char smem[];
-  tn_body<NBN, NBK, false>(smem, Y, ldy, X, ldx, M, N, K, ymax, xmax, parts, S, mk, nt_k);
+  tn_body<NBN, NBK, false>(smem, Y, ldy, X, ldx, M, N, K, ymax, xmax, parts, S, mk, nt_k, ycmax,
+                           xcmax);
 }
 
 
@@ -1125,15 +1172,21 @@
   return prev;
 }
 
+bool gemm_nt_h_cmax_ok(const float* A, int64_t lda, int64_t M, int R, int C, const float* out,
+                       int64_t ldo) {
+  return g_nt_mode == 1 && M >= NT_WS_MIN_ROWS && nt_ws_ok(M, R, C, A, lda, out, ldo);
+}
+
 static_assert(NT_WAVES == N_WAVES && NT_BM == N_BM && NT_MAXC == N_MAXC &&
               NT_DACT_MAXC == N_DACT_MAXC, "nt_plan.h sizes the kernels' tiles");
 
 int launch_gemm_nt_h(const float* A, int64_t lda, int64_t M, int R, const void* Wf, int C,
                      const float* bias, float* out, int64_t ldo, int accumulate, float* rmax,
-                     hipStream_t st) {
+                     hipStream_t st, float* cmax) {
   (void)accumulate;
   if (g_nt_mode == 1 && M >= NT_WS_MIN_ROWS && nt_ws_ok(M, R, C, A, lda, out, ldo))
-    return launch_gemm_nt_ws(A, lda, M, R, Wf, C, bias, out, ldo, rmax, st);
+    return launch_gemm_nt_ws(A, lda, M, R, Wf, C, bias, out, ldo, rmax, cmax, st);
+  if (cmax != nullptr) return fail("rb_gemm_nt_h_cmax: not a weight-stationary call");
   const bool wide = aligned16(out) && ldo % 4 == 0;
   const NtPlan p = nt_plan(NtKind::plain, M, R, C, wide, bias != nullptr, num_cus());
   const NtArgs a{A, lda, M, R, Wf, C, bias, out, ldo, rmax, nullptr, nullptr, nullptr, DropSpec{}, st};
@@ -1185,7 +1238,7 @@
 
 int launch_gemm_tn_h(const float* Y, int64_t ldy, const float* X, int64_t ldx, int64_t M, int N,
                      int K, const float* ymax, const float* xmax, float* parts, int S,
-                     hipStream_t st) {
+                     hipStream_t st, const float* ycmax, const float* xcmax) {
   const int64_t mk = ((M + S - 1) / S + 31) / 32 * 32;
   auto run = [&](auto nbn_c, auto nbk_c) {
     constexpr int NBN = decltype(nbn_c)::value, NBK = decltype(nbk_c)::value;
@@ -1199,7 +1252,7 @@
     const int nt_k = K / CF::XC;
     const int nt = (N / CF::YC) * nt_k;
     k_gemm_tn_h<NBN, NBK><<<(unsigned)((nt * S + 7) / 8 * 8), CF::THREADS, CF::LDS, st>>>(
-        Y, ldy, X, ldx, M, N, K, ymax, xmax, parts, S, mk, nt_k);
+        Y, ldy, X, ldx, M, N, K, ymax, xmax, parts, S, mk, nt_k, ycmax, xcmax);
   };
   switch (tn_tile_shape(N, K)) {
     case 2: run(std::integral_constant<int, 2>{}, std::integral_constant<int, 1>{}); break;
diff --git a/datamining_recblr_amd/csrc/gemm_ws.hip b/datamining_recblr_amd/csrc/gemm_ws.hip
--- a/datamining_recblr_amd/csrc/gemm_ws.hip
+++ b/datamining_recblr_amd/csrc/gemm_ws.hip
@@ -46,20 +46,24 @@
   float* rstd = nullptr;
 };
 
-template <int K, int NCB, int D, bool BIAS, bool DEFER, int ABL, int EPI = 0>
+template <int K>
+constexpr int CMQ = K / 4 + 16;
+
+template <int K, int NCB, int D, bool BIAS, bool DEFER, int ABL, int EPI = 0, bool CMAX = false>
 __global__ void __launch_bounds__(THREADS, 1)
 k_gemm_nt_ws(const float* __restrict__ A, int64_t lda, int64_t M, const f16x8* __restrict__ Wi,
              const int* __restrict__ ew, int C, const float* __restrict__ bias,
              float* __restrict__ out, int64_t ldo, float* __restrict__ rmax,
              float* __restrict__ act, DropSpec drop, const float* __restrict__ pre,
-             float* __restrict__ dpart, LnSpec ln) {
+             float* __restrict__ dpart, LnSpec ln, float* __restrict__ cmax) {
   using CF = Cfg<K, NCB, D>;
+  static_assert(CF::LDS + (CMAX ? 2 * CMQ<K> * 16 : 0) <= 160 * 1024, "LDS");
   constexpr int KS = CF::KS, WC = CF::WC, NT = CF::NT, NLD = CF::NLD, NST = CF::NST;
   constexpr bool TWO = EPI == 1 || EPI == 3;
   constexpr bool PRE = EPI == 2 || EPI == 3;
   constexpr int NSTT = TWO ? 2 * NST : NST;
   constexpr int NPRE = PRE ? 2 * NCB : 0;
-  constexpr int NSO = NSTT + 1 + (EPI == 3 ? 2 : 0);
+  constexpr int NSO = NSTT + 1 + (EPI == 3 ? 2 : 0) + (CMAX ? 1 : 0);
   static_assert(EPI != 3 || (NCB == 1 && DEFER), "LN epilogue: whole 128-column rows, deferred stores");
   constexpr bool EARLY1 = D == 1 && (ABL & 32) == 0;
   extern __shared__ __attribute__((aligned(16))) char smem[];
@@ -88,6 +92,13 @@
     asm volatile("ds_write_b32 %0, %1" ::"v"(s_cols + c * 4), "v"(e) : "memory");
     asm volatile("ds_write_b32 %0, %1" ::"v"(s_cols + (NT + c) * 4), "v"(bv) : "memory");
   }
+  const uint32_t s_cmax = sbase + CF::LDS;
+  if constexpr (CMAX) {
+    for (int c = tid; c < 2 * 4 * CMQ<K>; c += THREADS)
+      asm volatile("ds_write_b32 %0, %1" ::"v"(s_cmax + c * 4), "v"(0) : "memory");
+    asm volatile("s_waitcnt lgkmcnt(0)" ::: "memory");
+    __builtin_amdgcn_s_barrier();
+  }
 
   const int col0 = ct * NT + wave * WC;
   f16x8 bw[NCB][KS][2];
@@ -159,6 +170,25 @@
     const int e = exp_of(mx);
     const float sc = __builtin_amdgcn_ldexpf(1.0f, kTR - e);
     const uint32_t img = sbase + ib * CF::IMG;
+    if constexpr (CMAX) {
+      const int lg = lane >> 4;
+#pragma unroll
+      for (int j = 0; j < NLD; ++j) {
+        float m4[4];
+#pragma unroll
+        for (int i = 0; i < 4; ++i) {
+          const float f = src[j][i];
+          const uint32_t a = __float_as_uint(f);
+          const auto h = __builtin_amdgcn_permlane32_swap(a, a, false, false);
+          const uint32_t m2 = __float_as_uint(max3abs(0.0f, __uint_as_float(h[0]), __uint_as_float(h[1])));
+          const auto q = __builtin_amdgcn_permlane16_swap(m2, m2, false, false);
+          m4[i] = fmaxf(__uint_as_float(q[0]), __uint_as_float(q[1]));
+        }
+        const float mv = lg == 0 ? m4[0] : lg == 1 ? m4[1] : lg == 2 ? m4[2] : m4[3];
+        asm volatile("ds_max_u32 %0, %1" ::"v"(s_cmax + (uint32_t)((ib * 4 * CMQ<K> + lg * CMQ<K> + 16 * j + (lane & 15)) * 4)),
+                     "v"(__float_as_uint(mv)) : "memory");
+      }
+    }
 #pragma unroll
     for (int j = 0; j < NLD; ++j) {
       const f32x4 v = src[j] * sc;
@@ -436,6 +466,22 @@
                         ((uint64_t)(uint32_t)__builtin_amdgcn_readfirstlane((uint32_t)(u >> 32)) << 32);
     const auto rr = __builtin_amdgcn_make_buffer_rsrc(reinterpret_cast<void*>(ub), 0, mine ? 4 : 0, 0x00020000);
     __builtin_amdgcn_raw_buffer_store_b32(__float_as_uint(x), rr, 0, 0, 0);
+  };
+  auto cmax_store = [&](int b, int ib) __attribute__((always_inline)) {
+    const int64_t r0 = blk_r0(b);
+    const int c = wave * (K / 8) + lane;
+    uint32_t x = 0;
+    if (lane < K / 8) {
+      const uint32_t a = s_cmax + (uint32_t)((ib * 4 * CMQ<K> + (c & 3) * CMQ<K> + (c >> 2)) * 4);
+      asm volatile("ds_read_b32 %0, %1\n\ts_waitcnt lgkmcnt(0)" : "=v"(x) : "v"(a) : "memory");
+      asm volatile("ds_write_b32 %0, %1" ::"v"(a), "v"(0) : "memory");
+    }
+    const bool mine = ct == 0 && r0 < M;
+    const uint64_t u = reinterpret_cast<uint64_t>(cmax) + (mine ? (uint64_t)(r0 / RB) * (K * 4) : 0);
+    const uint64_t ub = (uint64_t)(uint32_t)__builtin_amdgcn_readfirstlane((uint32_t)u) |
+                        ((uint64_t)(uint32_t)__builtin_amdgcn_readfirstlane((uint32_t)(u >> 32)) << 32);
+    const auto rr = __builtin_amdgcn_make_buffer_rsrc(reinterpret_cast<void*>(ub), 0, mine ? K * 4 : 0, 0x00020000);
+    __builtin_amdgcn_raw_buffer_store_b32(x, rr, lane < K / 8 ? (uint32_t)c * 4 : 0x40000000u, 0, 2);
   };
 
   [&]<int... P>(std::integer_sequence<int, P...>) __attribute__((always_inline)) {
@@ -481,6 +527,7 @@
           if constexpr (u % STEP == 0 && u / STEP < NSTT) flush(u / STEP);
         });
         rmax_store(b, ib);
+        if constexpr (CMAX) cmax_store(b, ib);
         if constexpr (EPI == 3) ln_store(b - 1);
         finish(b, ib);
       } else {
@@ -489,6 +536,7 @@
 #pragma unroll
         for (int i = 0; i < NSTT; ++i) flush(i);
         rmax_store(b, ib);
+        if constexpr (CMAX) cmax_store(b, ib);
       }
       if constexpr (LATE) do_split();
       asm volatile("s_waitcnt lgkmcnt(0)" ::: "memory");
@@ -527,20 +575,21 @@
   }
 }
 
-template <int K, int NCB, int D, bool BIAS, bool DEFER, int ABL, int EPI = 0>
+template <int K, int NCB, int D, bool BIAS, bool DEFER, int ABL, int EPI = 0, bool CMAX = false>
 void run(const float* A, int64_t lda, int64_t M, const void* Wi, const int* ew, int C,
          const float* bias, float* out, int64_t ldo, float* rmax, int grid, hipStream_t st,
          float* act = nullptr, DropSpec drop = DropSpec{}, const float* pre = nullptr,
-         float* dpart = nullptr, LnSpec ln = LnSpec{}) {
+         float* dpart = nullptr, LnSpec ln = LnSpec{}, float* cmax = nullptr) {
   using CF = Cfg<K, NCB, D>;
+  constexpr int lds = CF::LDS + (CMAX ? 2 * CMQ<K> * 16 : 0);
   static bool done = false;
   if (!done) {
-    (void)hipFuncSetAttribute((const void*)k_gemm_nt_ws<K, NCB, D, BIAS, DEFER, ABL, EPI>,
-                              hipFuncAttributeMaxDynamicSharedMemorySize, CF::LDS);
+    (void)hipFuncSetAttribute((const void*)k_gemm_nt_ws<K, NCB, D, BIAS, DEFER, ABL, EPI, CMAX>,
+                              hipFuncAttributeMaxDynamicSharedMemorySize, lds);
     done = true;
   }
-  k_gemm_nt_ws<K, NCB, D, BIAS, DEFER, ABL, EPI><<<grid, THREADS, CF::LDS, st>>>(
-      A, lda, M, (const f16x8*)Wi, ew, C, bias, out, ldo, rmax, act, drop, pre, dpart, ln);
+  k_gemm_nt_ws<K, NCB, D, BIAS, DEFER, ABL, EPI, CMAX><<<grid, THREADS, lds, st>>>(
+      A, lda, M, (const f16x8*)Wi, ew, C, bias, out, ldo, rmax, act, drop, pre, dpart, ln, cmax);
 }
 
 template <int K>
@@ -570,7 +619,8 @@
 }
 
 int launch_gemm_nt_ws(const float* A, int64_t lda, int64_t M, int K, const void* Wf, int C,
-                      const float* bias, float* out, int64_t ldo, float* rmax, hipStream_t st) {
+                      const float* bias, float* out, int64_t ldo, float* rmax, float* cmax,
+                      hipStream_t st) {
   if (!nt_ws_ok(M, K, C, A, lda, out, ldo)) return fail("rb_gemm_nt_h: no weight-stationary launch for this shape");
   const WeightImage w = weight_image(Wf, C, K);
   const int ncb = ws::ncb_for(K, C);
@@ -579,9 +629,15 @@
     dispatch_int<1, 2, 4>(ncb, [&](auto nc) {
       dispatch_bool(bias != nullptr, [&](auto bias_c) {
         constexpr int KK = decltype(kc)::value, NC = decltype(nc)::value;
-        if constexpr (NC <= 16 / (KK / 32))
-          ws::run<KK, NC, ws::depth<KK>(), decltype(bias_c)::value, true, 0>(
-              A, lda, M, w.wi, w.ew, C, bias, out, ldo, rmax, grid, st);
+        if constexpr (NC <= 16 / (KK / 32)) {
+          if (cmax != nullptr)
+            ws::run<KK, NC, ws::depth<KK>(), decltype(bias_c)::value, true, 0, 0, true>(
+                A, lda, M, w.wi, w.ew, C, bias, out, ldo, rmax, grid, st, nullptr, DropSpec{}, nullptr,
+                nullptr, ws::LnSpec{}, cmax);
+          else
+            ws::run<KK, NC, ws::depth<KK>(), decltype(bias_c)::value, true, 0>(
+                A, lda, M, w.wi, w.ew, C, bias, out, ldo, rmax, grid, st);
+        }
       });
     });
   });
diff --git a/datamining_recblr_amd/kernels.py b/datamining_recblr_amd/kernels.py
--- a/datamining_recblr_amd/kernels.py
+++ b/datamining_recblr_amd/kernels.py
@@ -1304,7 +1304,8 @@
 
 
 def gemm_nt_h(a: torch.Tensor, wf: torch.Tensor, C: int, bias: torch.Tensor | None = None,
-              out: torch.Tensor | None = None, rmax: torch.Tensor | None = None) -> torch.Tensor:
+              out: torch.Tensor | None = None, rmax: torch.Tensor | None = None,
+              cmax: torch.Tensor | None = None) -> torch.Tensor:
     _check(a, "a")
     if a.dim() != 2 or a.stride(1) != 1:
         raise ValueError("a must be a 2-D tensor with unit inner stride")
@@ -1319,6 +1320,14 @@
         _check(rmax, "rmax")
         if rmax.numel() < (M + 31) // 32:
             raise ValueError("rmax needs ceil(M/32) entries")
+    if cmax is not None:
+        _check(cmax, "cmax")
+        if cmax.shape != ((M + 31) // 32, R) or not cmax.is_contiguous():
+            raise ValueError("cmax must be a contiguous [ceil(M/32), R] tensor")
+        _lib.call("rb_gemm_nt_h_cmax", a.data_ptr(), a.stride(0), M, R, wf.data_ptr(), C,
+                  0 if bias is None else bias.data_ptr(), out.data_ptr(), out.stride(0),
+                  0 if rmax is None else rmax.data_ptr(), cmax.data_ptr(), _stream(a))
+        return out
     _lib.call("rb_gemm_nt_h", a.data_ptr(), a.stride(0), M, R, wf.data_ptr(), C,
               0 if bias is None else bias.data_ptr(), out.data_ptr(), out.stride(0), 0,
               0 if rmax is None else rmax.data_ptr(), _stream(a))
@@ -1437,7 +1446,8 @@
 
 
 def gemm_tn_h(dy: torch.Tensor, x: torch.Tensor, ymax: torch.Tensor, xmax: torch.Tensor,
-              splits: int) -> torch.Tensor:
+              splits: int, ycmax: torch.Tensor | None = None,
+              xcmax: torch.Tensor | None = None) -> torch.Tensor:
     for t, n in ((dy, "dy"), (x, "x"), (ymax, "ymax"), (xmax, "xmax")):
         _check(t, n)
     if dy.dim() != 2 or x.dim() != 2 or dy.stride(1) != 1 or x.stride(1) != 1:
@@ -1449,6 +1459,16 @@
     if ymax.numel() < (M + 31) // 32 or xmax.numel() < (M + 31) // 32:
         raise ValueError("ymax / xmax need ceil(M/32) entries")
     parts = torch.empty((splits, N, K), device=dy.device, dtype=torch.float32)
+    if ycmax is not None and xcmax is not None:
+        nb = (M + 31) // 32
+        for t, n, w in ((ycmax, "ycmax", N), (xcmax, "xcmax", K)):
+            _check(t, n)
+            if t.shape != (nb, w) or not t.is_contiguous():
+                raise ValueError(f"{n} must be a contiguous [ceil(M/32), {w}] tensor")
+        _lib.call("rb_gemm_tn_h_cmax", dy.data_ptr(), dy.stride(0), x.data_ptr(), x.stride(0), M,
+                  N, K, ymax.data_ptr(), xmax.data_ptr(), ycmax.data_ptr(), xcmax.data_ptr(),
+                  parts.data_ptr(), splits, _stream(dy))
+        return parts
     _lib.call("rb_gemm_tn_h", dy.data_ptr(), dy.stride(0), x.data_ptr(), x.stride(0), M, N, K,
               ymax.data_ptr(), xmax.data_ptr(), parts.data_ptr(), splits, _stream(dy))
     return parts
diff --git a/datamining_recblr_amd/linear.py b/datamining_recblr_amd/linear.py
--- a/datamining_recblr_amd/linear.py
+++ b/datamining_recblr_amd/linear.py
@@ -132,6 +132,23 @@
     return None
 
 
+_tn_cmax = os.environ.get("RECBLR_TN_CMAX", "1") != "0"
+NT_WS_MIN_ROWS = 16384
+
+
+def set_tn_cmax(on: bool) -> bool:
+    global _tn_cmax
+    prev, _tn_cmax = _tn_cmax, bool(on)
+    return prev
+
+
+def cmax_buffer(a: torch.Tensor, C: int, R: int) -> torch.Tensor | None:
+    if (_tn_cmax and _half and _tn_on and _NT_WS == "1" and _split_ok(a, C, R)
+            and a.shape[0] >= NT_WS_MIN_ROWS and R in (128, 256, 512) and C % 128 == 0):
+        return torch.empty(((a.shape[0] + 31) // 32, R), device=a.device, dtype=torch.float32)
+    return None
+
+
 BF16_NT_MAX_R = 512
 BF16_NT_MIN_ROWS = 65536
 _BF16_MODES = ("auto", "1", "0")
@@ -173,7 +190,7 @@
 
 
 def mm_nt(a: torch.Tensor, w: torch.Tensor, bias: torch.Tensor | None = None,
-          rmax: torch.Tensor | None = None) -> torch.Tensor:
+          rmax: torch.Tensor | None = None, cmax: torch.Tensor | None = None) -> torch.Tensor:
     if a.dtype != w.dtype and _bf16_ok(a, w, w.shape[0], w.shape[1]):
         b = None if bias is None else bias.contiguous()
         return kernels.gemm_nt_bf16(a, _bf16_image(w, False), w.shape[0], bias=b)
@@ -182,7 +199,7 @@
         return torch.addmm(bias.to(a.dtype), a, wb.t()) if bias is not None else a @ wb.t()
     N, K = w.shape
     if _split_ok(a, N, K):
-        return kernels.gemm_nt_h(a, _weight_split(w, False), N, bias=bias, rmax=rmax)
+        return kernels.gemm_nt_h(a, _weight_split(w, False), N, bias=bias, rmax=rmax, cmax=cmax)
     return torch.addmm(bias, a, w.t()) if bias is not None else torch.mm(a, w.t())
 
 
@@ -248,7 +265,7 @@
 
 
 def mm_nn(dy: torch.Tensor, w: torch.Tensor, out: torch.Tensor | None = None,
-          rmax: torch.Tensor | None = None) -> torch.Tensor:
+          rmax: torch.Tensor | None = None, cmax: torch.Tensor | None = None) -> torch.Tensor:
     if dy.dtype != w.dtype and out is None and _bf16_ok(dy, w, w.shape[1], w.shape[0]):
         return kernels.gemm_nt_bf16(dy, _bf16_image(w, True), w.shape[1])
     if dy.dtype != w.dtype:
@@ -256,7 +273,7 @@
         return out.addmm_(dy, wb) if out is not None else dy @ wb
     N, K = w.shape
     if _split_ok(dy, K, N):
-        r = kernels.gemm_nt_h(dy, _weight_split(w, True), K, rmax=rmax)
+        r = kernels.gemm_nt_h(dy, _weight_split(w, True), K, rmax=rmax, cmax=cmax)
         return r if out is None else out.add_(r)
     if out is not None:
         return out.addmm_(dy, w)
@@ -280,7 +297,8 @@
 
 
 def wgrad(dy2: torch.Tensor, x2: torch.Tensor, splits: int = SPLIT_K,
-          ymax: torch.Tensor | None = None, xmax: torch.Tensor | None = None) -> torch.Tensor:
+          ymax: torch.Tensor | None = None, xmax: torch.Tensor | None = None,
+          ycmax: torch.Tensor | None = None, xcmax: torch.Tensor | None = None) -> torch.Tensor:
     M = dy2.shape[0]
     N, K = dy2.shape[1], x2.shape[1]
     if (ymax is not None and xmax is not None
@@ -292,7 +310,9 @@
         S = _tn_splits(dy2.device, (N // 128) * (K // 128))
         if M < MIN_ROWS_FOR_SPLIT:
             S = max(8, min(S, M // 32 // 8 * 8))
-        parts = kernels.gemm_tn_h(dy2, x2, ymax, xmax, S)
+        if ycmax is None or xcmax is None or M < MIN_ROWS_FOR_SPLIT:
+            ycmax = xcmax = None
+        parts = kernels.gemm_tn_h(dy2, x2, ymax, xmax, S, ycmax=ycmax, xcmax=xcmax)
         return kernels.colsum(parts.view(S, -1)).view(N, K)
     if (_small_tn and _half and _split_on and _tn_on and M < MIN_ROWS_FOR_SPLIT and N % 32 == 0
             and K % 32 == 0 and dy2.dtype == torch.float32 and x2.dtype == torch.float32
@@ -344,8 +364,10 @@
         x2 = x.reshape(-1, x.shape[-1])
         flops = 2 * x2.shape[0] * x2.shape[1] * weight.shape[0]
         rx = rmax_buffer(x2, weight.shape[0], weight.shape[1]) if ctx.needs_input_grad[1] else None
-        y = _timed("gemm", flops, mm_nt, x2, weight, bias, rmax=rx)
+        cx = cmax_buffer(x2, weight.shape[0], weight.shape[1]) if rx is not None else None
+        y = _timed("gemm", flops, mm_nt, x2, weight, bias, rmax=rx, cmax=cx)
         ctx.rx = rx
+        ctx.cx = cx
         ctx.save_for_backward(x2, weight)
         ctx.has_bias = bias is not None
         ctx.slot = slot
@@ -357,11 +379,13 @@
         dy2 = dy.reshape(-1, dy.shape[-1])
         flops = 2 * x2.shape[0] * x2.shape[1] * weight.shape[0]
         dx = dw = db = None
-        ry = None
+        ry = cy = None
         if ctx.needs_input_grad[0]:
             slot = ctx.slot
             ry = rmax_buffer(dy2, weight.shape[1], weight.shape[0]) if ctx.rx is not None else None
-            dx = _timed("gemm", flops, mm_nn, dy2, weight, rmax=ry)
+            cy = (cmax_buffer(dy2, weight.shape[1], weight.shape[0])
+                  if ry is not None and ctx.cx is not None else None)
+            dx = _timed("gemm", flops, mm_nn, dy2, weight, rmax=ry, cmax=cy)
             if slot is not None and slot.ds is not None:
                 if slot.rows is not None:
                     dx.index_add_(0, slot.rows, slot.ds.view(-1, weight.shape[1]))
@@ -371,7 +395,8 @@
                     slot.ds = None
             dx = dx.view(*dy.shape[:-1], weight.shape[1])
         if ctx.needs_input_grad[1]:
-            dw = _timed("gemm", flops, wgrad, dy2, x2, ymax=ry, xmax=ctx.rx)
+            dw = _timed("gemm", flops, wgrad, dy2, x2, ymax=ry, xmax=ctx.rx, ycmax=cy,
+                        xcmax=ctx.cx)
         if ctx.has_bias and ctx.needs_input_grad[2]:
             db = (kernels.colsum(dy2.contiguous()) if dy2.dtype == torch.float32
                   else dy2.sum(0, dtype=torch.float32))
diff --git a/include/recblr_colscale.h b/include/recblr_colscale.h
--- /dev/null
+++ b/include/recblr_colscale.h
@@ -0,0 +1,25 @@
+#ifndef RECBLR_COLSCALE_H
+#define RECBLR_COLSCALE_H
+
+#include <stdint.h>
+
+#ifdef __cplusplus
+extern "C" {
+#endif
+
+int rb_gemm_nt_h_cmax_ok(const float* A, int64_t lda, int64_t M, int64_t R, int64_t C,
+                         const float* out, int64_t ldo);
+int rb_gemm_nt_h_cmax(const float* A, int64_t lda, int64_t M, int64_t R, const void* Wf, int64_t C,
+                      const float* bias, float* out, int64_t ldo, float* rmax, float* cmax,
+                      void* stream);
+
+int rb_gemm_tn_h_cmax(const float* dY, int64_t ldy, const float* X, int64_t ldx, int64_t M,
+                      int64_t N, int64_t K, const float* ymax, const float* xmax,
+                      const float* ycmax, const float* xcmax, float* parts, int64_t splits,
+                      void* stream);
+
+#ifdef __cplusplus
+}
+#endif
+
+#endif
diff --git a/include/recblr_hip.h b/include/recblr_hip.h
--- a/include/recblr_hip.h
+++ b/include/recblr_hip.h
@@ -14,7 +14,7 @@
 
 #define RB_TILE 16
 
-#define RB_ABI_VERSION 49
+#define RB_ABI_VERSION 50
 int rb_version(void);
 
 const char* rb_last_error_string(void);
```

After: 385,700. -2.0%, worse.
